# kiranbond/cilium

Hardware: AMD Instinct MI355X
Metric: policy verdicts/sec (whole node) + request GB/s, 10K-rule L7 HTTP set (higher is better)
Workload: dtype u8

## Files before the change

cilium_amd/_native.py:

```python
from __future__ import annotations

import ctypes as C
import os
from pathlib import Path

LIB_PATH = Path(os.environ.get("CILIUM_AMD_LIB") or Path(__file__).resolve().parent / "libciliumgpu.so")

CG_OK = 0
CG_POLICY_DROP = 1
CG_PARSER_ERROR = 2
CG_UNKNOWN_PARSER = 3
CG_UNKNOWN_CONNECTION = 4
CG_INVALID_ADDRESS = 5
CG_INVALID_INSTANCE = 6
CG_UNKNOWN_ERROR = 7
CG_INVALID_ARGUMENT = 16
CG_NO_DEVICE = 17
CG_DEVICE_ERROR = 18
CG_POLICY_REJECTED = 19
CG_REVISION_MISMATCH = 20
CG_MAP_FULL = 21
CG_NOT_FOUND = 22
CG_NO_MAP = 23
CG_UNSUPPORTED = 24

CG_REGEX_ECMA, CG_REGEX_GO = 0, 1

CG_L4_F_INGRESS = 0x01
CG_L4_F_FRAGMENT = 0x02
CG_L4_F_CB_POLICY = 0x04
CG_L4_CAN_ACCESS, CG_L4_INGRESS, CG_L4_EGRESS, CG_L4_IGNORE_DROP = 0, 1, 2, 0x100
CG_DROP_POLICY = -133
CG_DROP_FRAG_NOSUPPORT = -157
CG_DROP_MISSED_TAIL_CALL = -140
CG_POLICY_ARRAY_SLOTS = 65536
CG_DROP_INVALID, CG_DROP_CT_INVALID_HDR, CG_DROP_CT_UNKNOWN_PROTO, CG_DROP_UNKNOWN_L3 = -134, -135, -137, -139
CG_DROP_INVALID_EXTHDR = -156
CG_FRAME_NOT_LOCAL, CG_FRAME_TO_HOST = -1, -2
CG_ENDPOINT_F_HOST = 1

CG_PF_DYN4, CG_PF_DYN6, CG_PF_FIX4, CG_PF_FIX6 = 1, 2, 4, 8
CG_XDP_DROP, CG_XDP_PASS = 1, 2
CG_WORLD_ID = 2

CG_CTR_HTTP_PROGRAMS, CG_CTR_KAFKA, CG_CTR_PREFILTER, CG_CTR_HTTP_RULES, CG_CTR_HTTP_ALLREDUCE = 0, 1, 2, 3, 4
CG_HTTP_RULE_NO_HTTP, CG_HTTP_RULE_SCOPE_ALLOW = 0xFFFFFFFF, 0xFFFFFFFE

CG_HTTP_TILE = 64
CG_HTTP_UNITS = 9

CG_KAFKA_MAX_TOPICS = 12
CG_KAFKA_K_NIL, CG_KAFKA_K_TYPED, CG_KAFKA_K_CONSUMER_METADATA = 0, 1, 2
CG_KAFKA_UNKNOWN_STR = 0xFFFFFFFF
CG_KAFKA_TOPICS_IN_ARENA = 255
CG_KAFKA_DECODE_OK, CG_KAFKA_DECODE_ERROR = 0, 1
CG_KAFKA_V_DENY, CG_KAFKA_V_ALLOW, CG_KAFKA_V_CLOSE = 0, 1, 2

CG_SEL_MATCH_LABEL, CG_SEL_IN, CG_SEL_NOT_IN, CG_SEL_EXISTS, CG_SEL_DOES_NOT_EXIST = 0, 1, 2, 3, 4
CG_EXP_ALL = 0x1


class CiliumGPUError(RuntimeError):
    def __init__(self, code: int, msg: str):
        super().__init__(f"[{code}] {msg}")
        self.code = code
        self.msg = msg


class KV(C.Structure):
    _fields_ = [("key", C.c_char_p), ("value", C.c_char_p)]


class PolicyKeyC(C.Structure):
    _pack_ = 1
    _fields_ = [("sec_label", C.c_uint32), ("dport", C.c_uint16), ("protocol", C.c_uint8), ("egress", C.c_uint8)]


class PolicyEntryC(C.Structure):
    _fields_ = [("proxy_port", C.c_uint16), ("pad", C.c_uint16 * 3), ("packets", C.c_uint64),
                ("bytes", C.c_uint64)]


class CidrC(C.Structure):
    _fields_ = [("family", C.c_uint8), ("prefixlen", C.c_uint8), ("pad", C.c_uint8 * 2), ("addr", C.c_uint8 * 16)]


class SelectorTableC(C.Structure):
    _fields_ = [("n_selectors", C.c_size_t), ("req_off", C.c_void_p), ("ops", C.c_void_p),
                ("key_blob", C.c_void_p), ("key_off", C.c_void_p), ("val_off", C.c_void_p),
                ("val_blob", C.c_void_p), ("val_str_off", C.c_void_p)]


class SelcacheRulesC(C.Structure):
    _fields_ = [("n_rules", C.c_size_t), ("subject", C.c_void_p), ("dir_flags", C.c_void_p),
                ("req_off", C.c_void_p * 2), ("req_idx", C.c_void_p * 2),
                ("allow_off", C.c_void_p * 2), ("allow_idx", C.c_void_p * 2)]


class ExpandTableC(C.Structure):
    _fields_ = [("n_rows", C.c_size_t), ("rows", C.c_void_p), ("src_off", C.c_void_p), ("src_idx", C.c_void_p)]


_u64, _u32, _sz, _p, _i64 = C.c_uint64, C.c_uint32, C.c_size_t, C.c_void_p, C.c_int64
SIGNATURES = {
    "cg_open": (_u64, [C.POINTER(KV), _sz, C.c_uint8]),
    "cg_close": (None, [_u64]),
    "cg_last_error": (C.c_char_p, []),
    "cg_version": (C.c_char_p, []),
    "cg_sync": (C.c_int, [_u64]),
    "cg_policymap_create": (C.c_int, [_u64, _u32, C.POINTER(_u32)]),
    "cg_policymap_destroy": (C.c_int, [_u64, _u32]),
    "cg_policymap_allow": (C.c_int, [_u64, _u32, _p, _p, _sz]),
    "cg_policymap_delete": (C.c_int, [_u64, _u32, _p, _sz]),
    "cg_policymap_lookup": (C.c_int, [_u64, _u32, _p, _p]),
    "cg_policymap_dump": (C.c_int, [_u64, _u32, _p, _p, _sz, C.POINTER(_sz)]),
    "cg_policymap_flush": (C.c_int, [_u64, _u32]),
    "cg_l4_verdicts_dev": (C.c_int, [_u64, _u32, _p, _sz, _p, _p]),
    "cg_l4_verdicts_host": (C.c_int, [_u64, _u32, _p, _sz, _p]),
    "cg_l4_policy_verdicts_dev": (C.c_int, [_u64, _u32, _u32, _p, _sz, _p, _p]),
    "cg_l4_policy_verdicts_host": (C.c_int, [_u64, _u32, _u32, _p, _sz, _p]),
    "cg_prefilter_create": (C.c_int, [_u64, _u32, _u32, _u32, C.POINTER(_u32)]),
    "cg_prefilter_destroy": (C.c_int, [_u64, _u32]),
    "cg_prefilter_insert": (C.c_int, [_u64, _u32, _i64, _p, _sz, C.POINTER(_i64)]),
    "cg_prefilter_delete": (C.c_int, [_u64, _u32, _i64, _p, _sz, C.POINTER(_i64)]),
    "cg_prefilter_dump": (C.c_int, [_u64, _u32, _p, _sz, C.POINTER(_sz), C.POINTER(_i64)]),
    "cg_prefilter_set_endpoints": (C.c_int, [_u64, _u32, _p, _sz, _p, _sz]),
    "cg_prefilter_verdicts_dev": (C.c_int, [_u64, _u32, _p, _sz, _p, _p, _sz, _p, _p]),
    "cg_prefilter_verdicts_host": (C.c_int, [_u64, _u32, _p, _sz, _p, _p, _sz, _p]),
    "cg_ipcache_create": (C.c_int, [_u64, _u32, C.POINTER(_u32)]),
    "cg_ipcache_destroy": (C.c_int, [_u64, _u32]),
    "cg_ipcache_update": (C.c_int, [_u64, _u32, _p, _p, _sz]),
    "cg_ipcache_delete": (C.c_int, [_u64, _u32, _p, _sz]),
    "cg_ipcache_lookup": (C.c_int, [_u64, _u32, _p, _p]),
    "cg_ipcache_dump": (C.c_int, [_u64, _u32, _p, _p, _sz, C.POINTER(_sz)]),
    "cg_ipcache_resolve_dev": (C.c_int, [_u64, _u32, _p, _sz, _p, _p, _sz, _p, _p]),
    "cg_ipcache_resolve_host": (C.c_int, [_u64, _u32, _p, _sz, _p, _p, _sz, _p]),
    "cg_proxylib_stats": (C.c_int, [_u64, C.POINTER(C.c_uint64), C.POINTER(C.c_uint64)]),
    "cg_kafka_decode_stats": (C.c_int, [_u64, C.POINTER(C.c_uint64), C.POINTER(C.c_uint64)]),
    "cg_kafka_inflate_stats": (C.c_int, [_u64, C.POINTER(C.c_uint64)]),
    "cg_proxylib_set_batching": (C.c_int, [_u64, _u32, _u32]),
    "cg_proxylib_policy_update": (C.c_int, [_u64, C.c_char_p, _sz]),
    "cg_proxylib_policy_update_npds": (C.c_int, [_u64, C.c_char_p, _sz]),
    "cg_l4_verdicts_ipcache_dev": (C.c_int, [_u64, _u32, _u32, _p, _p, _sz, _p, _p]),
    "cg_l4_verdicts_ipcache_host": (C.c_int, [_u64, _u32, _u32, _p, _p, _sz, _p]),
    "cg_l4_verdicts_ipcache6_dev": (C.c_int, [_u64, _u32, _u32, _p, _p, _sz, _p, _p]),
    "cg_l4_verdicts_ipcache6_host": (C.c_int, [_u64, _u32, _u32, _p, _p, _sz, _p]),
    "cg_http_policy_update": (C.c_int, [_u64, C.c_char_p, _sz]),
    "cg_http_policy_update_npds": (C.c_int, [_u64, C.c_char_p, _sz]),
    "cg_http_pack_threads": (_u32, []),
    "cg_http_policy_export": (C.c_int, [_u64, C.c_void_p, _sz, C.POINTER(_sz)]),
    "cg_http_policy_import": (C.c_int, [_u64, C.c_char_p, _sz]),
    "cg_http_policy_index": (C.c_int, [_u64, C.c_char_p, C.POINTER(_u32)]),
    "cg_http_policy_stats": (C.c_int, [_u64, C.POINTER(_u64), _sz]),
    "cg_http_rule_info_get": (C.c_int, [_u64, _p, _sz, C.POINTER(_sz)]),
    "cg_http_batch_bytes": (_sz, [_u64, _sz]),
    "cg_http_batch_slots": (_sz, [_u64, _sz]),
    "cg_http_pack": (C.c_int, [_u64, _sz, _p, _p, _p, _p, _p, _p, _p, _sz, _p, C.POINTER(_sz), _p, _sz,
                               C.POINTER(_sz)]),
    "cg_http_parse_heads": (C.c_int, [_p, _p, _sz, _p, _sz, _p, C.POINTER(_sz), _p]),
    "cg_http_verdicts_dev": (C.c_int, [_u64, _p, _sz, _p, _p, _p]),
    "cg_http_verdicts_host": (C.c_int, [_u64, _p, _sz, _p, _sz, _p, _sz, _p]),
    "cg_http_verdicts_rules_host": (C.c_int, [_u64, _p, _sz, _p, _sz, _p, _sz, _p, _p]),
    "cg_http_verdicts_rules_dev": (C.c_int, [_u64, _p, _sz, _p, _p, _p, _p]),
    "cg_http_verdicts_raw_dev": (C.c_int, [_u64, _p, _p, _sz, _p, _p, _p, _p, _p, _p]),
    "cg_http_verdicts_raw_host": (C.c_int, [_u64, _p, _p, _sz, _p, _p, _p, _p, _p]),
    "cg_http_verdicts_fields_dev": (C.c_int, [_u64, _p, _p, _sz, _p, _p, _p, _p, _p, _p]),
    "cg_http_verdicts_fields_host": (C.c_int, [_u64, _p, _p, _sz, _p, _p, _p, _p, _p]),
    "cg_http_ring_open": (C.c_int, [_u64, C.c_uint32, C.c_uint32]),
    "cg_http_ring_verdicts": (C.c_int, [_u64, _p, _p, _sz, _p, _p, _p, _p, _p]),
    "cg_http_ring_stats": (C.c_int, [_u64, C.POINTER(C.c_uint64), C.POINTER(C.c_uint64)]),
    "cg_http_ring_close": (C.c_int, [_u64]),
    "cg_kafka_policy_update": (C.c_int, [_u64, C.c_char_p, _sz]),
    "cg_kafka_policy_index": (C.c_int, [_u64, C.c_char_p, C.POINTER(_u32)]),
    "cg_kafka_intern": (C.c_int, [_u64, _u32, C.c_char_p, _sz, C.POINTER(_u32)]),
    "cg_kafka_verdicts_dev": (C.c_int, [_u64, _p, _sz, _p, _p, _p]),
    "cg_kafka_verdicts_split_dev": (C.c_int, [_u64, _p, _p, _sz, _p, _p, _p]),
    "cg_kafka_verdicts_host": (C.c_int, [_u64, _p, _sz, _p, _sz, _p]),
    "cg_kafka_decode_host": (C.c_int, [_u64, _p, _p, _sz, _p, _p, _p, _p, _sz, C.POINTER(_sz), _p]),
    "cg_kafka_decode_dev": (C.c_int, [_u64, _p, _p, _sz, _p, _p, _p, _p, _sz, C.POINTER(_sz), _p, _p]),
    "cg_kafka_verdicts_raw_host": (C.c_int, [_u64, _p, _p, _sz, _p, _p, _p]),
    "cg_diag_kafka_decode_host": (C.c_int, [_u64, _p, _p, _sz, _p, _p, _p, _p, _sz, C.POINTER(_sz), _p]),
    "cg_read_counters": (C.c_int, [_u64, _u32, _u32, _p, _sz, C.POINTER(_sz)]),
    "cg_counters_device_ptr": (C.c_int, [_u64, _u32, _u32, C.POINTER(_p), C.POINTER(_sz)]),
    "cg_counters_copy_dev": (C.c_int, [_u64, _u32, _u32, _p, _sz, _p]),
    "cg_reset_counters": (C.c_int, [_u64]),
    "cg_diag_regex_match": (C.c_int, [C.c_char_p, _sz, _p, _sz, _u32, C.POINTER(C.c_uint8)]),
    "cg_regex_validate": (C.c_int, [C.c_char_p, _sz, _u32]),
    "cg_diag_http_eval_host": (C.c_int, [_u64, _p, _sz, _p, _sz, _p, _sz, _p]),
    "cg_diag_http_rules_host": (C.c_int, [_u64, _p, _sz, _p, _sz, _p, _sz, _p]),
    "cg_diag_kafka_eval_host": (C.c_int, [_u64, _p, _sz, _p, _sz, _p]),
    "cg_diag_l4_eval_host": (C.c_int, [_u64, _u32, _p, _sz, _p]),
    "cg_diag_ipcache_eval_host": (C.c_int, [_u64, _u32, _p, _sz, _p, _p, _sz, _p]),
    "cg_diag_prefilter_eval_host": (C.c_int, [_u64, _u32, _p, _sz, _p, _p, _sz, _p]),
    "cg_selcache_create": (C.c_int, [_u64, C.POINTER(_u32)]),
    "cg_selcache_destroy": (C.c_int, [_u64, _u32]),
    "cg_selcache_set_identities": (C.c_int, [_u64, _u32, _p, _sz, _p, _p, _p, _p, _p]),
    "cg_selcache_set_cidr_identities": (C.c_int, [_u64, _u32, _p, _p, _sz]),
    "cg_selcache_set_rules": (C.c_int, [_u64, _u32, C.POINTER(SelectorTableC), C.POINTER(SelcacheRulesC)]),
    "cg_selcache_info": (C.c_int, [_u64, _u32, C.POINTER(_sz), C.POINTER(_sz), C.POINTER(_sz), C.POINTER(_sz)]),
    "cg_selcache_match_dev": (C.c_int, [_u64, _u32, C.POINTER(SelectorTableC), _p, _sz, _p]),
    "cg_selcache_match_host": (C.c_int, [_u64, _u32, C.POINTER(SelectorTableC), _p, _sz]),
    "cg_selcache_reach_dev": (C.c_int, [_u64, _u32, _p, _sz, _p, _p, _p, _p]),
    "cg_selcache_reach_host": (C.c_int, [_u64, _u32, _p, _sz, _p, _p, _p]),
    "cg_diag_selcache_match_host": (C.c_int, [_u64, _u32, C.POINTER(SelectorTableC), _p, _sz, _u32]),
    "cg_diag_selcache_reach_host": (C.c_int, [_u64, _u32, _p, _sz, _p, _p, _p, _u32]),
    "cg_selcache_expand_dev": (C.c_int, [_u64, _u32, C.POINTER(ExpandTableC), _p, _sz, _p, _p, _p, _sz, _p, _p]),
    "cg_selcache_expand_host": (C.c_int, [_u64, _u32, C.POINTER(ExpandTableC), _p, _sz, _p, _p, _p, _sz, _p]),
    "cg_selcache_entries_host": (C.c_int, [_u64, _u32, C.POINTER(SelectorTableC), _p, _sz, C.POINTER(ExpandTableC),
                                           _p, _p, _p, _sz, _p, _p]),
    "cg_diag_selcache_expand_host": (C.c_int, [_u64, _u32, C.POINTER(ExpandTableC), _p, _sz, _p, _p, _p, _sz, _p,
                                               _u32]),
    "cg_diag_selcache_entries_host": (C.c_int, [_u64, _u32, C.POINTER(SelectorTableC), _p, _sz,
                                                C.POINTER(ExpandTableC), _p, _p, _p, _sz, _p, _p, _u32]),
    "cg_policymap_sync": (C.c_int, [_u64, _u32, _p, _p, _sz, C.POINTER(_sz), C.POINTER(_sz)]),
    "cg_policy_array_create": (C.c_int, [_u64, C.POINTER(_u32)]),
    "cg_policy_array_destroy": (C.c_int, [_u64, _u32]),
    "cg_policy_array_set": (C.c_int, [_u64, _u32, _p, _p, _sz]),
    "cg_policy_array_clear": (C.c_int, [_u64, _u32, _p, _sz]),
    "cg_policy_array_get": (C.c_int, [_u64, _u32, C.c_uint16, C.POINTER(_u32)]),
    "cg_l4_array_verdicts_dev": (C.c_int, [_u64, _u32, _u32, _p, _p, _sz, _p, _p]),
    "cg_l4_array_verdicts_host": (C.c_int, [_u64, _u32, _u32, _p, _p, _sz, _p]),
    "cg_l4_array_verdicts_ipcache_dev": (C.c_int, [_u64, _u32, _u32, _u32, C.c_int, _p, _p, _p, _sz, _p, _p]),
    "cg_l4_array_verdicts_ipcache_host": (C.c_int, [_u64, _u32, _u32, _u32, C.c_int, _p, _p, _p, _sz, _p]),
    "cg_diag_l4_array_eval_host": (C.c_int, [_u64, _u32, _u32, _p, _p, _sz, _p]),
    "cg_endpoint_map_create": (C.c_int, [_u64, _u32, C.POINTER(_u32)]),
    "cg_endpoint_map_destroy": (C.c_int, [_u64, _u32]),
    "cg_endpoint_map_update": (C.c_int, [_u64, _u32, _p, _p, _sz]),
    "cg_endpoint_map_delete": (C.c_int, [_u64, _u32, _p, _sz]),
    "cg_endpoint_map_lookup": (C.c_int, [_u64, _u32, _p, _p]),
    "cg_endpoint_map_dump": (C.c_int, [_u64, _u32, _p, _p, _sz, C.POINTER(_sz)]),
    "cg_l4_frames_verdicts_dev": (C.c_int, [_u64, _u32, _u32, _p, _p, _sz, _p, _u32, _p, _u32, _p, _p, _p, _p]),
    "cg_l4_frames_verdicts_host": (C.c_int, [_u64, _u32, _u32, _p, _p, _sz, _p, _u32, _p, _u32, _p, _p, _p]),
    "cg_diag_l4_frames_eval_host": (C.c_int, [_u64, _u32, _u32, _p, _p, _sz, _p, _u32, _p, _u32, _p, _p, _p, _p]),
}


def _load() -> C.CDLL:
    if not LIB_PATH.exists():
        raise ImportError(f"{LIB_PATH} is missing: build it with `python -m cilium_amd.build` "
                          "(there is no CPU fallback for the verdict paths)")
    lib = C.CDLL(str(LIB_PATH), mode=os.RTLD_NOW | getattr(os, "RTLD_GLOBAL", 0))
    for name, (res, args) in SIGNATURES.items():
        fn = getattr(lib, name)
        fn.restype = res
        fn.argtypes = args
    return lib


lib = _load()


def check(rc: int) -> None:
    if rc != CG_OK:
        raise CiliumGPUError(rc, lib.cg_last_error().decode(errors="replace"))


def regex_validate(pattern, flavour: int = CG_REGEX_GO) -> None:
    b = pattern.encode("utf-8", "surrogateescape") if isinstance(pattern, str) else bytes(pattern)
    check(lib.cg_regex_validate(b, len(b), flavour))


def ptr(a) -> int | None:
    if a is None:
        return None
    if hasattr(a, "data_ptr"):
        return a.data_ptr()
    return a.ctypes.data
```

cilium_amd/classifier.py:

```python
from __future__ import annotations

import ctypes as C
import ipaddress
import json
from typing import Iterable, Optional, Sequence

import numpy as np

from . import _native as N
from .policy import PolicyEntry, PolicyKey, PortRuleKafka, htons

L4_TUPLE_DTYPE = np.dtype([("identity", "<u4"), ("dport", "<u2"), ("proto", "u1"), ("flags", "u1"),
                           ("len", "<u4")])
POLICY_KEY_DTYPE = np.dtype([("sec_label", "<u4"), ("dport", "<u2"), ("protocol", "u1"), ("egress", "u1")])
CIDR_DTYPE = np.dtype([("family", "u1"), ("prefixlen", "u1"), ("pad", "u1", (2,)), ("addr", "u1", (16,))])
KAFKA_REQ_DTYPE = np.dtype([("api_key", "<i2"), ("api_version", "<i2"), ("kind", "u1"), ("n_topics", "u1"),
                            ("policy", "<u2"), ("remote", "<u4"), ("client_id", "<u4"),
                            ("topic_ids", "<u4", (N.CG_KAFKA_MAX_TOPICS,))])
ENDPOINT_KEY_DTYPE = np.dtype([("family", "u1"), ("pad", "u1", (3,)), ("addr", "u1", (16,))])
ENDPOINT_INFO_DTYPE = np.dtype([("lxc_id", "<u2"), ("pad", "<u2"), ("flags", "<u4")])
FRAME_INFO_DTYPE = np.dtype([("t", L4_TUPLE_DTYPE), ("lxc_id", "<u2"), ("family", "u1"), ("pad", "u1")])
assert ENDPOINT_KEY_DTYPE.itemsize == 20 and ENDPOINT_INFO_DTYPE.itemsize == 8 and FRAME_INFO_DTYPE.itemsize == 16
assert L4_TUPLE_DTYPE.itemsize == 12 and KAFKA_REQ_DTYPE.itemsize == 64 and CIDR_DTYPE.itemsize == 20


def _p(a):
    return N.ptr(a)


class HttpBatch:

    def __init__(self, batch: np.ndarray, arena: np.ndarray, order: np.ndarray, nslots: int, n: int):
        self.batch, self.arena, self.order, self.nslots, self.n = batch, arena, order, nslots, n

    def used_bytes(self) -> int:
        return int(self.batch[:64].view(np.uint64)[5])


class Classifier:

    def __init__(self, device: int = 0, debug: bool = False):
        kv = (N.KV * 1)(N.KV(b"device", str(device).encode()))
        self.h = N.lib.cg_open(kv, 1, 1 if debug else 0)
        if not self.h:
            raise N.CiliumGPUError(N.CG_NO_DEVICE, N.lib.cg_last_error().decode())
        self.device = device

    def close(self) -> None:
        if self.h:
            N.lib.cg_close(self.h)
            self.h = 0

    def __enter__(self):
        return self

    def __exit__(self, *a):
        self.close()

    def __del__(self):
        try:
            self.close()
        except Exception:
            pass

    def sync(self) -> None:
        N.check(N.lib.cg_sync(self.h))

    def policy_map(self, max_entries: int = 0) -> "PolicyMap":
        return PolicyMap(self, max_entries)

    def policy_array(self) -> "PolicyArray":
        return PolicyArray(self)

    def endpoint_map(self, max_entries: int = 0) -> "EndpointMap":
        return EndpointMap(self, max_entries)

    def prefilter(self, dyn4: bool = False, dyn6: bool = False, fix4: bool = True, fix6: bool = True,
                  max_lpm: int = 0, max_hash: int = 0) -> "PreFilter":
        return PreFilter(self, dyn4, dyn6, fix4, fix6, max_lpm, max_hash)

    def ipcache(self, max_entries: int = 0) -> "IPCache":
        return IPCache(self, max_entries)

    def selector_cache(self) -> "SelectorCache":
        from .selcache import SelectorCache
        return SelectorCache(self)

    def update_http_policy(self, policies: list[dict] | bytes | str) -> None:
        blob = policies if isinstance(policies, (bytes, str)) else json.dumps(policies, separators=(",", ":"))
        if isinstance(blob, str):
            blob = blob.encode()
        N.check(N.lib.cg_http_policy_update(self.h, blob, len(blob)))

    def update_http_policy_npds(self, discovery_response: bytes) -> None:
        N.check(N.lib.cg_http_policy_update_npds(self.h, discovery_response, len(discovery_response)))

    def export_http_policy(self) -> bytes:
        n = C.c_size_t()
        N.check(N.lib.cg_http_policy_export(self.h, None, 0, C.byref(n)))
        buf = C.create_string_buffer(n.value)
        N.check(N.lib.cg_http_policy_export(self.h, buf, n.value, C.byref(n)))
        return buf.raw[:n.value]

    def import_http_policy(self, image: bytes) -> None:
        N.check(N.lib.cg_http_policy_import(self.h, image, len(image)))

    def http_policy_index(self, name: str) -> int:
        v = C.c_uint32()
        rc = N.lib.cg_http_policy_index(self.h, name.encode(), C.byref(v))
        if rc == N.CG_NOT_FOUND:
            return 0xFFFFFFFF
        N.check(rc)
        return v.value

    def http_policy_stats(self) -> dict:
        out = (C.c_uint64 * 12)()
        N.check(N.lib.cg_http_policy_stats(self.h, out, 12))
        keys = ["programs", "parts", "states", "table_bytes", "fields", "rules", "policies", "remote_slots",
                "exceptions", "cells", "max_program_cells", "lds_programs"]
        return dict(zip(keys, list(out)))

    def pack_http(self, policy: np.ndarray, ingress: np.ndarray, port: np.ndarray, remote: np.ndarray,
                  hdr_blob: np.ndarray, hdr_off: np.ndarray):
        n = len(policy)
        policy = np.ascontiguousarray(policy, dtype=np.uint32)
        ingress = np.ascontiguousarray(ingress, dtype=np.uint8)
        port = np.ascontiguousarray(port, dtype=np.uint16)
        remote = np.ascontiguousarray(remote, dtype=np.uint32)
        hdr_blob = np.ascontiguousarray(hdr_blob, dtype=np.uint8)
        hdr_off = np.ascontiguousarray(hdr_off, dtype=np.uint64)
        if len(hdr_blob) == 0:
            hdr_blob = np.zeros(1, np.uint8)
        used = C.c_size_t()
        nslots = C.c_size_t()
        stats = (C.c_uint64 * 12)()
        N.check(N.lib.cg_http_policy_stats(self.h, stats, 12))
        cap = (int(hdr_off[n]) - int(hdr_off[0]) if n else 0) + n * (int(stats[4]) + 24) + 16
        arena = np.empty(cap, np.uint8)
        batch = np.empty(N.lib.cg_http_batch_bytes(self.h, n), np.uint8)
        order = np.empty(max(N.lib.cg_http_batch_slots(self.h, n), 1), np.uint32)
        N.check(N.lib.cg_http_pack(self.h, n, _p(policy), _p(ingress), _p(port), _p(remote), _p(hdr_blob),
                                   _p(hdr_off), _p(batch), batch.nbytes, _p(order), C.byref(nslots), _p(arena),
                                   arena.nbytes, C.byref(used)))
        arena = arena[:max(used.value, 16)].copy()
        return HttpBatch(batch, arena, order[:nslots.value], nslots.value, n)

    @staticmethod
    def parse_http_heads(raw_blob: np.ndarray, raw_off: np.ndarray):
        raw_blob = np.ascontiguousarray(raw_blob, np.uint8)
        raw_off = np.ascontiguousarray(raw_off, np.uint64)
        n = len(raw_off) - 1
        if len(raw_blob) == 0:
            raw_blob = np.zeros(1, np.uint8)
        used = C.c_size_t()
        N.check(N.lib.cg_http_parse_heads(_p(raw_blob), _p(raw_off), n, None, 0, None, C.byref(used), None))
        blob = np.zeros(max(used.value, 1), np.uint8)
        off = np.zeros(n + 1, np.uint64)
        ok = np.zeros(max(n, 1), np.uint8)
        N.check(N.lib.cg_http_parse_heads(_p(raw_blob), _p(raw_off), n, _p(blob), blob.nbytes, _p(off),
                                          C.byref(used), _p(ok)))
        return blob, off, ok[:n]

    def pack_http_raw(self, policy, ingress, port, remote, raw_blob: np.ndarray, raw_off: np.ndarray):
        blob, off, ok = self.parse_http_heads(raw_blob, raw_off)
        pol = np.where(ok.astype(bool), np.asarray(policy, np.uint32), np.uint32(0xFFFFFFFF)).astype(np.uint32)
        return self.pack_http(pol, ingress, port, remote, blob, off)

    def http_verdicts_raw(self, policy, ingress, port, remote, raw_blob: np.ndarray, raw_off: np.ndarray) -> np.ndarray:
        return self._verdicts_from_host(N.lib.cg_http_verdicts_raw_host, policy, ingress, port, remote, raw_blob,
                                        raw_off)

    def http_verdicts_fields(self, policy, ingress, port, remote, hdr_blob: np.ndarray,
                             hdr_off: np.ndarray) -> np.ndarray:
        return self._verdicts_from_host(N.lib.cg_http_verdicts_fields_host, policy, ingress, port, remote, hdr_blob,
                                        hdr_off)

    def http_ring_open(self, workgroups: int = 16, slots: int = 32) -> None:
        N.check(N.lib.cg_http_ring_open(self.h, workgroups, slots))

    def http_ring_verdicts(self, policy, ingress, port, remote, hdr_blob: np.ndarray,
                           hdr_off: np.ndarray) -> np.ndarray:
        return self._verdicts_from_host(N.lib.cg_http_ring_verdicts, policy, ingress, port, remote, hdr_blob,
                                        hdr_off)

    def http_ring_stats(self) -> dict:
        served, launches = C.c_uint64(), C.c_uint64()
        N.check(N.lib.cg_http_ring_stats(self.h, C.byref(served), C.byref(launches)))
        return {"served": served.value, "launches": launches.value}

    def http_ring_close(self) -> None:
        N.check(N.lib.cg_http_ring_close(self.h))

    def _verdicts_from_host(self, fn, policy, ingress, port, remote, raw_blob, raw_off) -> np.ndarray:
        raw_blob = np.ascontiguousarray(raw_blob, np.uint8)
        raw_off = np.ascontiguousarray(raw_off, np.uint64)
        n = len(raw_off) - 1
        if len(raw_blob) == 0:
            raw_blob = np.zeros(1, np.uint8)
        pol = np.ascontiguousarray(policy, np.uint32)
        ing = np.ascontiguousarray(ingress, np.uint8)
        prt = np.ascontiguousarray(port, np.uint16)
        rem = np.ascontiguousarray(remote, np.uint32)
        out = np.zeros(max(n, 1), np.uint8)
        N.check(fn(self.h, _p(raw_blob), _p(raw_off), n, _p(pol), _p(ing), _p(prt), _p(rem), _p(out)))
        return out[:n]

    def http_verdicts_raw_dev(self, d_raw, d_off, n: int, d_policy, d_ingress, d_port, d_remote, d_out,
                              stream=None) -> None:
        N.check(N.lib.cg_http_verdicts_raw_dev(self.h, _p(d_raw), _p(d_off), n, _p(d_policy), _p(d_ingress),
                                               _p(d_port), _p(d_remote), _p(d_out), stream))

    def http_verdicts_fields_dev(self, d_blob, d_off, n: int, d_policy, d_ingress, d_port, d_remote, d_out,
                                 stream=None) -> None:
        N.check(N.lib.cg_http_verdicts_fields_dev(self.h, _p(d_blob), _p(d_off), n, _p(d_policy), _p(d_ingress),
                                                  _p(d_port), _p(d_remote), _p(d_out), stream))

    def http_verdicts(self, b: "HttpBatch") -> np.ndarray:
        out = np.zeros(max(b.n, 1), np.uint8)
        N.check(N.lib.cg_http_verdicts_host(self.h, _p(b.batch), b.nslots, _p(b.order), b.n, _p(b.arena),
                                            b.arena.nbytes, _p(out)))
        return out[:b.n]

    def http_verdicts_dev(self, d_batch, nslots: int, d_arena, d_out, stream=None) -> None:
        N.check(N.lib.cg_http_verdicts_dev(self.h, _p(d_batch), nslots, _p(d_arena), _p(d_out), stream))

    def http_verdicts_rules(self, b: "HttpBatch") -> tuple[np.ndarray, np.ndarray]:
        out = np.zeros(max(b.n, 1), np.uint8)
        rule = np.zeros(max(b.n, 1), np.uint32)
        N.check(N.lib.cg_http_verdicts_rules_host(self.h, _p(b.batch), b.nslots, _p(b.order), b.n, _p(b.arena),
                                                  b.arena.nbytes, _p(out), _p(rule)))
        return out[:b.n], rule[:b.n]

    def http_verdicts_rules_dev(self, d_batch, nslots: int, d_arena, d_out, d_rule, stream=None) -> None:
        N.check(N.lib.cg_http_verdicts_rules_dev(self.h, _p(d_batch), nslots, _p(d_arena), _p(d_out), _p(d_rule),
                                                 stream))

    HTTP_RULE_INFO_DTYPE = np.dtype([("policy", "<u4"), ("ingress", "<u4"), ("port", "<u4"), ("scope", "<u4"),
                                     ("rule", "<u4"), ("http_rule", "<u4")])

    def http_rule_info(self) -> np.ndarray:
        n = C.c_size_t()
        N.check(N.lib.cg_http_rule_info_get(self.h, None, 0, C.byref(n)))
        out = np.zeros(max(n.value, 1), self.HTTP_RULE_INFO_DTYPE)
        N.check(N.lib.cg_http_rule_info_get(self.h, _p(out), n.value, C.byref(n)))
        return out[:n.value]

    def http_rule_hits(self) -> np.ndarray:
        return self.read_counters(N.CG_CTR_HTTP_RULES)

    def allreduce_counter_count(self) -> int:
        return self.counters_device_ptr(N.CG_CTR_HTTP_ALLREDUCE)[1]

    def counters_copy_dev(self, d_dst, n: int, stream=None, what: int = N.CG_CTR_HTTP_ALLREDUCE) -> None:
        N.check(N.lib.cg_counters_copy_dev(self.h, what, 0, _p(d_dst), n, stream))

    def http_rules_host_diag(self, b: "HttpBatch") -> np.ndarray:
        out = np.zeros(max(b.n, 1), np.uint32)
        N.check(N.lib.cg_diag_http_rules_host(self.h, _p(b.batch), b.nslots, _p(b.order), b.n, _p(b.arena),
                                              b.arena.nbytes, _p(out)))
        return out[:b.n]

    def http_eval_host_diag_slots(self, b: "HttpBatch") -> np.ndarray:
        v = self.http_eval_host_diag(b)
        out = np.zeros(b.nslots, np.uint8)
        order = b.order[:b.nslots]
        real = order < b.n
        out[real] = v[order[real]]
        return out

    def http_eval_host_diag(self, b: "HttpBatch") -> np.ndarray:
        out = np.zeros(max(b.n, 1), np.uint8)
        N.check(N.lib.cg_diag_http_eval_host(self.h, _p(b.batch), b.nslots, _p(b.order), b.n, _p(b.arena),
                                             b.arena.nbytes, _p(out)))
        return out[:b.n]

    def update_kafka_policy(self, redirects: list[dict]) -> None:
        def conv(r):
            return r.to_json() if isinstance(r, PortRuleKafka) else r
        doc = [{"name": rd["name"], "selectors": [
            {"identities": s.get("identities"), "rules": [conv(r) for r in s.get("rules", [])]}
            for s in rd.get("selectors", [])]} for rd in redirects]
        blob = json.dumps(doc).encode()
        N.check(N.lib.cg_kafka_policy_update(self.h, blob, len(blob)))

    def kafka_redirect_index(self, name: str) -> int:
        v = C.c_uint32()
        rc = N.lib.cg_kafka_policy_index(self.h, name.encode(), C.byref(v))
        if rc == N.CG_NOT_FOUND:
            return 0xFFFF
        N.check(rc)
        return v.value

    def kafka_intern(self, what: str, s: bytes) -> int:
        v = C.c_uint32()
        N.check(N.lib.cg_kafka_intern(self.h, 0 if what == "topic" else 1, s, len(s), C.byref(v)))
        return v.value

    def pack_kafka(self, redirect: Sequence[int], remote: Sequence[int], api_key: Sequence[int],
                   api_version: Sequence[int], kind: Sequence[int], client_id: Sequence[bytes],
                   topics: Sequence[Sequence[bytes]]):
        n = len(redirect)
        reqs = np.zeros(n, KAFKA_REQ_DTYPE)
        reqs["policy"] = np.asarray(redirect, np.uint16)
        reqs["remote"] = np.asarray(remote, np.uint32)
        reqs["api_key"] = np.asarray(api_key, np.int16)
        reqs["api_version"] = np.asarray(api_version, np.int16)
        reqs["kind"] = np.asarray(kind, np.uint8)
        cache_t: dict = {}
        cache_c: dict = {}
        arena: list[int] = []
        for i in range(n):
            c = client_id[i]
            if c not in cache_c:
                cache_c[c] = self.kafka_intern("client", c)
            reqs["client_id"][i] = cache_c[c]
            ts = topics[i]
            ids = []
            for t in ts:
                if t not in cache_t:
                    cache_t[t] = self.kafka_intern("topic", t)
                ids.append(cache_t[t])
            reqs["n_topics"][i] = min(len(ids), N.CG_KAFKA_TOPICS_IN_ARENA)
            if len(ids) <= N.CG_KAFKA_MAX_TOPICS:
                reqs["topic_ids"][i, :len(ids)] = ids
            else:
                reqs["topic_ids"][i, 0] = len(arena)
                if len(ids) >= N.CG_KAFKA_TOPICS_IN_ARENA:
                    reqs["topic_ids"][i, 1] = len(ids)
                arena.extend(ids)
        return reqs, np.asarray(arena if arena else [0], np.uint32)

    def kafka_decode(self, raw, raw_off, redirect, remote, diag_cpu: bool = False):
        raw = np.ascontiguousarray(raw, np.uint8)
        off = np.ascontiguousarray(raw_off, np.uint64)
        n = len(off) - 1
        red = np.ascontiguousarray(redirect, np.uint16)
        rem = np.ascontiguousarray(remote, np.uint32)
        if len(red) != n or len(rem) != n:
            raise ValueError("redirect/remote must have one entry per request")
        reqs = np.zeros(max(n, 1), KAFKA_REQ_DTYPE)
        status = np.zeros(max(n, 1), np.uint8)
        fn = N.lib.cg_diag_kafka_decode_host if diag_cpu else N.lib.cg_kafka_decode_host
        cap = 64
        while True:
            arena = np.zeros(cap, np.uint32)
            used = C.c_size_t()
            rc = fn(self.h, _p(raw), _p(off), n, _p(red), _p(rem), _p(reqs), _p(arena), cap, C.byref(used),
                    _p(status))
            if rc == N.CG_MAP_FULL and used.value > cap:
                cap = used.value
                continue
            N.check(rc)
            return reqs[:n], arena[:max(used.value, 1)], status[:n]

    def kafka_decode_dev(self, d_raw, d_off, n: int, d_redirect, d_remote, d_reqs, d_arena, arena_cap: int,
                         d_status, stream=None) -> int:
        used = C.c_size_t()
        N.check(N.lib.cg_kafka_decode_dev(self.h, _p(d_raw), _p(d_off), n, _p(d_redirect), _p(d_remote),
                                          _p(d_reqs), _p(d_arena), arena_cap, C.byref(used), _p(d_status), stream))
        return used.value

    def kafka_verdicts_raw(self, raw, raw_off, redirect, remote) -> np.ndarray:
        raw = np.ascontiguousarray(raw, np.uint8)
        off = np.ascontiguousarray(raw_off, np.uint64)
        n = len(off) - 1
        red = np.ascontiguousarray(redirect, np.uint16)
        rem = np.ascontiguousarray(remote, np.uint32)
        if len(red) != n or len(rem) != n:
            raise ValueError("redirect/remote must have one entry per request")
        out = np.zeros(max(n, 1), np.uint8)
        N.check(N.lib.cg_kafka_verdicts_raw_host(self.h, _p(raw), _p(off), n, _p(red), _p(rem), _p(out)))
        return out[:n]

    def kafka_verdicts(self, reqs: np.ndarray, arena: Optional[np.ndarray] = None) -> np.ndarray:
        n = len(reqs)
        out = np.zeros(max(n, 1), np.uint8)
        N.check(N.lib.cg_kafka_verdicts_host(self.h, _p(reqs), n, _p(arena), 0 if arena is None else len(arena),
                                             _p(out)))
        return out[:n]

    def kafka_verdicts_dev(self, d_reqs, n: int, d_arena, d_out, stream=None) -> None:
        N.check(N.lib.cg_kafka_verdicts_dev(self.h, _p(d_reqs), n, _p(d_arena), _p(d_out), stream))

    def kafka_verdicts_split_dev(self, d_heads, d_topics, n: int, d_arena, d_out, stream=None) -> None:
        N.check(N.lib.cg_kafka_verdicts_split_dev(self.h, _p(d_heads), _p(d_topics), n, _p(d_arena), _p(d_out),
                                                  stream))

    def kafka_eval_host_diag(self, reqs: np.ndarray, arena: Optional[np.ndarray] = None) -> np.ndarray:
        n = len(reqs)
        out = np.zeros(max(n, 1), np.uint8)
        N.check(N.lib.cg_diag_kafka_eval_host(self.h, _p(reqs), n, _p(arena), 0 if arena is None else len(arena),
                                              _p(out)))
        return out[:n]

    def read_counters(self, what: int, ident: int = 0) -> np.ndarray:
        n = C.c_size_t()
        N.check(N.lib.cg_read_counters(self.h, what, ident, None, 0, C.byref(n)))
        out = np.zeros(max(n.value, 1), np.uint64)
        N.check(N.lib.cg_read_counters(self.h, what, ident, _p(out), n.value, C.byref(n)))
        return out[:n.value]

    def counters_device_ptr(self, what: int, ident: int = 0) -> tuple[int, int]:
        p = C.c_void_p()
        n = C.c_size_t()
        N.check(N.lib.cg_counters_device_ptr(self.h, what, ident, C.byref(p), C.byref(n)))
        return p.value or 0, n.value

    def reset_counters(self) -> None:
        N.check(N.lib.cg_reset_counters(self.h))


class PolicyEntriesDump(list):

    def less(self, i: int, j: int) -> bool:
        a, b = self[i][0], self[j][0]
        if a.TrafficDirection < b.TrafficDirection:
            return True
        return a.TrafficDirection <= b.TrafficDirection and a.Identity < b.Identity

    def sorted(self) -> "PolicyEntriesDump":
        return PolicyEntriesDump(sorted(self, key=lambda ke: (ke[0].TrafficDirection, ke[0].Identity)))


class PolicyMap:

    def __init__(self, cl: Classifier, max_entries: int = 0):
        self.cl = cl
        v = C.c_uint32()
        N.check(N.lib.cg_policymap_create(cl.h, max_entries, C.byref(v)))
        self.id = v.value

    @classmethod
    def attach(cls, cl: Classifier, map_id: int) -> "PolicyMap":
        pm = cls.__new__(cls)
        pm.cl, pm.id = cl, int(map_id)
        return pm

    @staticmethod
    def _keys(keys: Iterable[PolicyKey]) -> np.ndarray:
        ks = list(keys)
        a = np.zeros(len(ks), POLICY_KEY_DTYPE)
        for i, k in enumerate(ks):
            a[i] = (k.Identity, k.DestPort, k.Nexthdr, k.TrafficDirection)
        return a

    def allow_key(self, k: PolicyKey, proxy_port: int) -> None:
        self.allow(k.Identity, k.DestPort, k.Nexthdr, k.TrafficDirection, proxy_port)

    def allow(self, identity: int, dport: int, proto: int, direction: int, proxy_port: int) -> None:
        self.allow_keys(self._keys([PolicyKey(identity, htons(dport), proto, int(direction))]),
                        np.asarray([htons(proxy_port)], np.uint16))

    def allow_keys(self, keys: np.ndarray, ports_be: np.ndarray) -> None:
        keys = np.ascontiguousarray(keys, POLICY_KEY_DTYPE)
        ports_be = np.ascontiguousarray(ports_be, np.uint16)
        N.check(N.lib.cg_policymap_allow(self.cl.h, self.id, _p(keys), _p(ports_be), len(keys)))

    def sync(self, keys: np.ndarray, ports_be: np.ndarray) -> tuple[int, int]:
        keys = np.ascontiguousarray(keys, POLICY_KEY_DTYPE)
        ports_be = np.ascontiguousarray(ports_be, np.uint16)
        if len(keys) != len(ports_be):
            raise ValueError("keys and ports_be differ in length")
        added, deleted = C.c_size_t(), C.c_size_t()
        N.check(N.lib.cg_policymap_sync(self.cl.h, self.id, _p(keys) if len(keys) else None,
                                        _p(ports_be) if len(keys) else None, len(keys),
                                        C.byref(added), C.byref(deleted)))
        return added.value, deleted.value

    def exists(self, identity: int, dport: int, proto: int, direction: int) -> bool:
        return self.lookup(PolicyKey(identity, htons(dport), proto, int(direction))) is not None

    def lookup(self, k: PolicyKey) -> Optional[PolicyEntry]:
        key = self._keys([k])
        e = N.PolicyEntryC()
        rc = N.lib.cg_policymap_lookup(self.cl.h, self.id, _p(key), C.byref(e))
        if rc == N.CG_NOT_FOUND:
            return None
        N.check(rc)
        return PolicyEntry(e.proxy_port, e.packets, e.bytes)

    def delete_key(self, k: PolicyKey) -> None:
        self.delete(k.Identity, k.DestPort, k.Nexthdr, k.TrafficDirection)

    def delete(self, identity: int, dport: int, proto: int, direction: int) -> None:
        key = self._keys([PolicyKey(identity, htons(dport), proto, int(direction))])
        N.check(N.lib.cg_policymap_delete(self.cl.h, self.id, _p(key), 1))

    def dump_to_slice(self) -> PolicyEntriesDump:
        n = C.c_size_t()
        N.check(N.lib.cg_policymap_dump(self.cl.h, self.id, None, None, 0, C.byref(n)))
        keys = np.zeros(max(n.value, 1), POLICY_KEY_DTYPE)
        ents = (N.PolicyEntryC * max(n.value, 1))()
        N.check(N.lib.cg_policymap_dump(self.cl.h, self.id, _p(keys), C.addressof(ents), n.value, C.byref(n)))
        return PolicyEntriesDump(
            (PolicyKey(int(k["sec_label"]), int(k["dport"]), int(k["protocol"]), int(k["egress"])),
             PolicyEntry(e.proxy_port, e.packets, e.bytes)) for k, e in zip(keys[:n.value], ents[:n.value]))

    def destroy(self) -> None:
        N.check(N.lib.cg_policymap_destroy(self.cl.h, self.id))

    def flush(self) -> None:
        N.check(N.lib.cg_policymap_flush(self.cl.h, self.id))

    def verdicts(self, tuples: np.ndarray, mode: int = N.CG_L4_CAN_ACCESS) -> np.ndarray:
        tuples = np.ascontiguousarray(tuples, L4_TUPLE_DTYPE)
        out = np.zeros(max(len(tuples), 1), np.int32)
        if mode == N.CG_L4_CAN_ACCESS:
            N.check(N.lib.cg_l4_verdicts_host(self.cl.h, self.id, _p(tuples), len(tuples), _p(out)))
        else:
            N.check(N.lib.cg_l4_policy_verdicts_host(self.cl.h, self.id, mode, _p(tuples), len(tuples), _p(out)))
        return out[:len(tuples)]

    def policy_can_access_ingress(self, tuples: np.ndarray) -> np.ndarray:
        return self.verdicts(tuples, N.CG_L4_INGRESS)

    def policy_can_egress(self, tuples: np.ndarray) -> np.ndarray:
        return self.verdicts(tuples, N.CG_L4_EGRESS)

    def verdicts_via_ipcache(self, ipc: "IPCache", remote: np.ndarray, tuples: np.ndarray) -> np.ndarray:
        tuples = np.ascontiguousarray(tuples, L4_TUPLE_DTYPE)
        out = np.zeros(max(len(tuples), 1), np.int32)
        if remote.dtype == np.uint8:
            remote = np.ascontiguousarray(remote, np.uint8).reshape(-1, 16)
            N.check(N.lib.cg_l4_verdicts_ipcache6_host(self.cl.h, self.id, ipc.id, _p(remote), _p(tuples),
                                                       len(tuples), _p(out)))
        else:
            remote = np.ascontiguousarray(remote, np.uint32)
            N.check(N.lib.cg_l4_verdicts_ipcache_host(self.cl.h, self.id, ipc.id, _p(remote), _p(tuples),
                                                      len(tuples), _p(out)))
        return out[:len(tuples)]

    def verdicts_dev(self, d_tuples, n: int, d_out, stream=None, mode: int = N.CG_L4_CAN_ACCESS) -> None:
        if mode == N.CG_L4_CAN_ACCESS:
            N.check(N.lib.cg_l4_verdicts_dev(self.cl.h, self.id, _p(d_tuples), n, _p(d_out), stream))
        else:
            N.check(N.lib.cg_l4_policy_verdicts_dev(self.cl.h, self.id, mode, _p(d_tuples), n, _p(d_out), stream))

    def eval_host_diag(self, tuples: np.ndarray) -> np.ndarray:
        tuples = np.ascontiguousarray(tuples, L4_TUPLE_DTYPE)
        out = np.zeros(max(len(tuples), 1), np.int32)
        N.check(N.lib.cg_diag_l4_eval_host(self.cl.h, self.id, _p(tuples), len(tuples), _p(out)))
        return out[:len(tuples)]


class PolicyArray:

    def __init__(self, cl: Classifier):
        self.cl = cl
        v = C.c_uint32()
        N.check(N.lib.cg_policy_array_create(cl.h, C.byref(v)))
        self.id = v.value

    @staticmethod
    def _lxc(lxc_ids) -> np.ndarray:
        a = np.asarray(lxc_ids)
        if a.size and (a.min() < 0 or a.max() >= N.CG_POLICY_ARRAY_SLOTS):
            raise N.CiliumGPUError(N.CG_INVALID_ARGUMENT, "lxc_id outside the policy array")
        return np.ascontiguousarray(a, np.uint16).reshape(-1)

    def set(self, lxc_id: int, policy_map: "PolicyMap") -> None:
        self.set_many([lxc_id], [policy_map])

    def set_many(self, lxc_ids, maps: Sequence) -> None:
# ... 332 lines not shown
```

cilium_amd/csrc/capi.cc:

```cpp
#include <hip/hip_runtime_api.h>

#include <algorithm>
#include <exception>
#include <chrono>
#include <cstring>
#include <map>
#include <memory>
#include <mutex>
#include <thread>
#include <string>
#include <vector>

#include "endpoint_map.h"
#include "engine.h"
#include "frame_walk.h"
#include "http.h"
#include "kafka.h"
#include "kafka_wire.h"
#include "kernels.h"
#include "l4.h"
#include "l4_array.h"
#include "l4_walk.h"
#include "ipcache.h"
#include "lpm.h"
// ... 1396 lines not shown

int cg_diag_selcache_match_host(uint64_t h, uint32_t sc_id, const cg_selector_table* sels, uint64_t* bits,
                                size_t cap_words, uint32_t threads) {
  return guarded([&] {
    auto e = get(h);
    const auto p = sc_pub(*e, sc_id);
    ScSelTab own;
    const ScSelTab& t = sc_table_of(*p, sels, &own);
    sc_check_cap(*p, t, bits, cap_words);
    sc_match_host(p->host_idents(), t.view(), bits, threads);
  });
}

static void sc_ensure_host_m(Engine& e, ScPublished& p, uint32_t threads) {
  std::lock_guard<std::mutex> lk(e.mu);
  const size_t need = p.seltab.sels.size() * (size_t)p.words;
  if (p.host_m.size() != need || !need) {
    p.host_m.assign(std::max<size_t>(need, 1), 0);
    sc_match_host(p.host_idents(), p.seltab.view(), p.host_m.data(), threads);
    if (!need) p.host_m.resize(1);
  }
}

int cg_diag_selcache_reach_host(uint64_t h, uint32_t sc_id, const uint32_t* endpoints, size_t n, uint64_t* ing,
                                uint64_t* eg, uint8_t* flags, uint32_t threads) {
  return guarded([&] {
    auto e = get(h);
    const auto p = sc_pub(*e, sc_id);
    sc_check_endpoints(*p, endpoints, n, ing, eg, flags);
    sc_ensure_host_m(*e, *p, threads);
    sc_reach_host(p->host_rules(), p->n, p->words, endpoints, n, ing, eg, flags, threads);
  });
}

static void sc_check_expand_out(const cg_expand_table* table, const void* row_off, const void* keys,
                                const void* proxy, size_t cap) {
  if (!table) fail(CG_INVALID_ARGUMENT, "selcache expand: NULL table");
  if (!row_off) fail(CG_INVALID_ARGUMENT, "selcache expand: NULL row_off");
  if (cap && (!keys || !proxy)) fail(CG_INVALID_ARGUMENT, "selcache expand: NULL keys/proxy");
  if (cap > (1ull << 40)) fail(CG_INVALID_ARGUMENT, "selcache expand: cap_entries out of range");
}

static ScExpDev sc_exp_view(const ScPublished& p, const ScExpRow* rows, const uint32_t* src_idx, size_t n_rows,
                            const uint32_t* ids, const uint64_t* src) {
  ScExpDev X{};
  X.rows = rows;
  X.src_idx = src_idx;
  X.ids = ids;
  X.src = reinterpret_cast<const unsigned long long*>(src);
  X.n_rows = (uint32_t)n_rows;
  X.n_ids = p.n;
  X.words = p.words;
  return X;
}

int cg_selcache_expand_dev(uint64_t h, uint32_t sc_id, const cg_expand_table* table, const uint64_t* d_src,
                           size_t src_rows, uint64_t* d_row_off, cg_policy_key* d_keys, uint16_t* d_proxy,
                           size_t cap_entries, uint64_t* d_total, void* stream) {
  return guarded([&] {
    auto e = get(h);
    e->require_gpu();
    sc_check_expand_out(table, d_row_off, d_keys, d_proxy, cap_entries);
    if ((uintptr_t)d_keys & 7u) fail(CG_INVALID_ARGUMENT, "selcache expand: d_keys is not 8-byte aligned");
    const auto p = sc_pub(*e, sc_id);
    const ScExpTab t = sc_compile_expand(*table, src_rows);
    if (!t.src_idx.empty() && p->words && !d_src) fail(CG_INVALID_ARGUMENT, "selcache expand: NULL source matrix");
    e->set_device();
    void* st = stream_of(*e, stream);
    auto tmp = std::make_shared<DevTables>();
    const ScExpDev X = sc_exp_view(*p, tmp->add(t.rows), tmp->add(t.src_idx), t.rows.size(), p->d_ids, d_src);
    check_launch(launch_selcache_expand(X, (unsigned long long*)d_row_off, d_keys, d_proxy, cap_entries,
                                        (unsigned long long*)d_total, st, e->cus),
                 "selcache expand kernel launch");
    fence(p->tab, st);
    fence(tmp, st);
  });
}

static void sc_expand_copy_back(Engine& e, size_t n_rows, const DevMem& d_off, const DevMem& d_keys,
                                const DevMem& d_proxy, uint64_t* row_off, cg_policy_key* keys, uint16_t* proxy,
                                size_t cap, uint64_t* total) {
  hipStream_t st = (hipStream_t)e.stream;
  hip_check(hipMemcpyAsync(row_off, d_off.get(), (n_rows + 1) * sizeof(uint64_t), hipMemcpyDeviceToHost, st),
            "hipMemcpy D2H");
  dev_sync(e, nullptr);
  const uint64_t n = row_off[n_rows];
  if (total) *total = n;
  if (n && n <= cap) {
    hip_check(hipMemcpyAsync(keys, d_keys.get(), n * sizeof(cg_policy_key), hipMemcpyDeviceToHost, st), "hipMemcpy D2H");
    hip_check(hipMemcpyAsync(proxy, d_proxy.get(), n * sizeof(uint16_t), hipMemcpyDeviceToHost, st), "hipMemcpy D2H");
    dev_sync(e, nullptr);
  }
}

int cg_selcache_expand_host(uint64_t h, uint32_t sc_id, const cg_expand_table* table, const uint64_t* src,
                            size_t src_rows, uint64_t* row_off, cg_policy_key* keys, uint16_t* proxy,
                            size_t cap_entries, uint64_t* total) {
  return guarded([&] {
    auto e = get(h);
    e->require_gpu();
    sc_check_expand_out(table, row_off, keys, proxy, cap_entries);
    const auto p = sc_pub(*e, sc_id);
    const ScExpTab t = sc_compile_expand(*table, src_rows);
    const size_t src_bytes = src_rows * (size_t)p->words * sizeof(uint64_t);
    if (src_bytes && !src) fail(CG_INVALID_ARGUMENT, "selcache expand: NULL source matrix");
    e->set_device();
    DevTables tmp;
    DevMem d_src, d_off, d_keys, d_proxy;
    d_src.upload(src, src_bytes);
    d_off.alloc((t.rows.size() + 1) * sizeof(uint64_t));
    d_keys.alloc(cap_entries * sizeof(cg_policy_key));
    d_proxy.alloc(cap_entries * sizeof(uint16_t));
    const ScExpDev X = sc_exp_view(*p, tmp.add(t.rows), tmp.add(t.src_idx), t.rows.size(), p->d_ids, d_src.as<uint64_t>());
    check_launch(launch_selcache_expand(X, d_off.as<unsigned long long>(), d_keys.get(), d_proxy.as<uint16_t>(),
                                        cap_entries, nullptr, e->stream, e->cus),
                 "selcache expand kernel launch");
    fence(p->tab, e->stream);
    sc_expand_copy_back(*e, t.rows.size(), d_off, d_keys, d_proxy, row_off, keys, proxy, cap_entries, total);
  });
}

static void sc_check_entries_args(const ScPublished& p, const uint32_t* eps, size_t n, const void* flags) {
  if (n && (!eps || !flags)) fail(CG_INVALID_ARGUMENT, "selcache entries: NULL endpoints/flags");
  if (n > 0x3FFFFFFFu) fail(CG_MAP_FULL, "selcache entries: too many endpoints");
  for (size_t i = 0; i < n; ++i)
    if (eps[i] >= p.n) fail(CG_INVALID_ARGUMENT, "selcache entries: endpoint index outside the identity table");
}

int cg_selcache_entries_host(uint64_t h, uint32_t sc_id, const cg_selector_table* sels, const uint32_t* endpoints,
                             size_t n_endpoints, const cg_expand_table* table, uint64_t* row_off,
                             cg_policy_key* keys, uint16_t* proxy, size_t cap_entries, uint64_t* total,
                             uint8_t* flags) {
  return guarded([&] {
    auto e = get(h);
    e->require_gpu();
    sc_check_expand_out(table, row_off, keys, proxy, cap_entries);
    const auto p = sc_pub(*e, sc_id);
    sc_check_entries_args(*p, endpoints, n_endpoints, flags);
    ScSelTab own;
    if (sels) own = sc_compile_selectors(*p->idents, sc_parse_selectors(*sels));
    const size_t S = own.sels.size(), E = n_endpoints, W = p->words;
    const ScExpTab t = sc_compile_expand(*table, S + 2 * E);
    e->set_device();
    DevTables tmp;
    DevMem d_src, d_ep, d_fl, d_off, d_keys, d_proxy;
    d_src.alloc((S + 2 * E) * W * sizeof(uint64_t));
    d_off.alloc((t.rows.size() + 1) * sizeof(uint64_t));
    d_keys.alloc(cap_entries * sizeof(cg_policy_key));
    d_proxy.alloc(cap_entries * sizeof(uint16_t));
    unsigned long long* src = d_src.as<unsigned long long>();
    if (S)
      check_launch(launch_selcache_match(p->dI, sc_upload_table(own, tmp), src, e->stream, e->cus),
                   "selcache match kernel launch");
    if (E) {
      d_ep.upload(endpoints, E * sizeof(uint32_t));
      d_fl.alloc(E);
      check_launch(launch_selcache_reach(p->dR, p->n, p->words, d_ep.as<uint32_t>(), E, src + S * W,
                                         src + (S + E) * W, d_fl.as<uint8_t>(), e->stream),
                   "selcache reach kernel launch");
      hip_check(hipMemcpyAsync(flags, d_fl.get(), E, hipMemcpyDeviceToHost, (hipStream_t)e->stream), "hipMemcpy D2H");
    }
    const ScExpDev X = sc_exp_view(*p, tmp.add(t.rows), tmp.add(t.src_idx), t.rows.size(), p->d_ids, d_src.as<uint64_t>());
    check_launch(launch_selcache_expand(X, d_off.as<unsigned long long>(), d_keys.get(), d_proxy.as<uint16_t>(),
                                        cap_entries, nullptr, e->stream, e->cus),
                 "selcache expand kernel launch");
    fence(p->tab, e->stream);
    sc_expand_copy_back(*e, t.rows.size(), d_off, d_keys, d_proxy, row_off, keys, proxy, cap_entries, total);
  });
}

int cg_diag_selcache_expand_host(uint64_t h, uint32_t sc_id, const cg_expand_table* table, const uint64_t* src,
                                 size_t src_rows, uint64_t* row_off, cg_policy_key* keys, uint16_t* proxy,
                                 size_t cap_entries, uint64_t* total, uint32_t threads) {
  return guarded([&] {
    auto e = get(h);
    sc_check_expand_out(table, row_off, keys, proxy, cap_entries);
    const auto p = sc_pub(*e, sc_id);
    const ScExpTab t = sc_compile_expand(*table, src_rows);
    if (src_rows * (size_t)p->words && !src) fail(CG_INVALID_ARGUMENT, "selcache expand: NULL source matrix");
    uint64_t n = 0;
    sc_expand_host(sc_exp_view(*p, t.rows.data(), t.src_idx.data(), t.rows.size(), p->ids.data(), src),
                   row_off, keys, proxy, cap_entries, &n, threads);
    if (total) *total = n;
  });
}

int cg_diag_selcache_entries_host(uint64_t h, uint32_t sc_id, const cg_selector_table* sels,
                                  const uint32_t* endpoints, size_t n_endpoints, const cg_expand_table* table,
                                  uint64_t* row_off, cg_policy_key* keys, uint16_t* proxy, size_t cap_entries,
                                  uint64_t* total, uint8_t* flags, uint32_t threads) {
  return guarded([&] {
    auto e = get(h);
    sc_check_expand_out(table, row_off, keys, proxy, cap_entries);
    const auto p = sc_pub(*e, sc_id);
    sc_check_entries_args(*p, endpoints, n_endpoints, flags);
    ScSelTab own;
    if (sels) own = sc_compile_selectors(*p->idents, sc_parse_selectors(*sels));
    const size_t S = own.sels.size(), E = n_endpoints, W = p->words;
    const ScExpTab t = sc_compile_expand(*table, S + 2 * E);
    std::vector<uint64_t> src(std::max<size_t>((S + 2 * E) * W, 1), 0);
    if (S) sc_match_host(p->host_idents(), own.view(), src.data(), threads);
    if (E) {
      sc_ensure_host_m(*e, *p, threads);
      sc_reach_host(p->host_rules(), p->n, p->words, endpoints, E, src.data() + S * W,
                    src.data() + (S + E) * W, flags, threads);
    }
    uint64_t n = 0;
    sc_expand_host(sc_exp_view(*p, t.rows.data(), t.src_idx.data(), t.rows.size(), p->ids.data(), src.data()),
                   row_off, keys, proxy, cap_entries, &n, threads);
    if (total) *total = n;
  });
}

int cg_http_policy_update(uint64_t h, const char* json, size_t len) {
  return guarded([&] {
    auto e = get(h);
    if (!json) fail(CG_INVALID_ARGUMENT, "NULL policy");
    std::shared_ptr<HttpSnapshot> snap = http_compile(json, len);
    if (e->has_gpu()) {
      e->set_device();
      snap->upload(*e);
    }
    {
      std::lock_guard<std::mutex> lk(e->mu);
      e->http = snap;
    }
    bump_epoch();
  });
}

int cg_http_policy_update_npds(uint64_t h, const uint8_t* resp, size_t len) {
  std::string json;
  const int rc = guarded([&] {
    if (!resp && len) fail(CG_INVALID_ARGUMENT, "NULL DiscoveryResponse");
    json = npds_pb_to_json(resp, len, true);
  });
  if (rc != CG_OK) return rc;
  return cg_http_policy_update(h, json.data(), json.size());
}

static std::shared_ptr<HttpSnapshot> http_snap(Engine& e);

int cg_http_policy_export(uint64_t h, void* buf, size_t cap, size_t* len) {
  return guarded([&] {
    auto e = get(h);
    const std::vector<uint8_t> img = http_image_export(*http_snap(*e));
    if (len) *len = img.size();
    if (buf && cap >= img.size()) memcpy(buf, img.data(), img.size());
    else if (buf) fail(CG_INVALID_ARGUMENT, "policy image buffer too small");
  });
}

int cg_http_policy_import(uint64_t h, const void* buf, size_t len) {
  return guarded([&] {
    auto e = get(h);
    std::shared_ptr<HttpSnapshot> snap = http_image_import(static_cast<const uint8_t*>(buf), len);
    if (e->has_gpu()) {
      e->set_device();
      snap->upload(*e);
    }
    {
      std::lock_guard<std::mutex> lk(e->mu);
      e->http = snap;
    }
    bump_epoch();
  });
}

static std::shared_ptr<HttpSnapshot> http_snap(Engine& e) {
  std::lock_guard<std::mutex> lk(e.mu);
  if (!e.http) fail(CG_NOT_FOUND, "no HTTP policy installed");
  return e.http;
}

int cg_http_policy_index(uint64_t h, const char* name, uint32_t* index) {
  return guarded([&] {
    auto e = get(h);
    auto s = http_snap(*e);
    auto it = s->policy_index.find(name ? name : "");
    if (it == s->policy_index.end()) fail(CG_NOT_FOUND, "no policy named " + std::string(name ? name : ""));
    *index = it->second;
  });
}

int cg_http_rule_info_get(uint64_t h, cg_http_rule_info* out, size_t cap, size_t* n) {
  return guarded([&] {
    auto e = get(h);
    auto s = http_snap(*e);
    if (n) *n = s->rule_info.size();
    if (out) memcpy(out, s->rule_info.data(), std::min(cap, s->rule_info.size()) * sizeof(cg_http_rule_info));
  });
}

int cg_http_policy_stats(uint64_t h, uint64_t* out, size_t n) {
  return guarded([&] {
    auto e = get(h);
    auto s = http_snap(*e);
    uint64_t max_prog_cells = 0, lds_progs = 0;
    for (const auto& pg : s->progs) {
      if (pg.flags & kProgAllowAll) continue;
      max_prog_cells = std::max<uint64_t>(max_prog_cells, pg.cell_count);
      lds_progs += (pg.flags & kProgRebased) && pg.cell_count <= kMaxLdsCells;
    }
    uint64_t v[12] = {s->progs.size(),
                     s->parts.size(),
                     s->total_states,
                     s->cells.size() * 4,
                     s->fields.size(),
                     s->total_rules,
                     s->npolicies,
                     s->total_remote_slots,
                     s->total_exceptions,
                     s->cells.size(),
                     max_prog_cells,
                     lds_progs};
    for (size_t i = 0; i < n && i < 12; ++i) out[i] = v[i];
  });
}

size_t cg_http_batch_bytes(uint64_t h, size_t n) {
  size_t v = 0;
  guarded([&] {
    auto e = get(h);
    v = http_batch_bytes(*http_snap(*e), n);
  });
  return v;
}

size_t cg_http_batch_slots(uint64_t h, size_t n) {
  size_t v = 0;
  guarded([&] {
    auto e = get(h);
    v = http_batch_slots(*http_snap(*e), n);
  });
  return v;
}

int cg_http_pack(uint64_t h, size_t n, const uint32_t* policy, const uint8_t* ingress, const uint16_t* port,
                 const uint32_t* remote, const uint8_t* hdr_blob, const uint64_t* hdr_off, void* batch,
                 size_t batch_cap, uint32_t* order, size_t* nslots, uint8_t* arena, size_t arena_cap,
                 size_t* arena_used) {
  return guarded([&] {
    auto e = get(h);
    auto s = http_snap(*e);
    http_pack(*s, n, policy, ingress, port, remote, hdr_blob, hdr_off, batch, batch_cap, order, nslots, arena,
              arena_cap, arena_used);
  });
}

static size_t batch_used_bytes(const void* batch) {
  HttpBatchHeader hdr;
  memcpy(&hdr, batch, sizeof(hdr));
  if (hdr.magic != kBatchMagic) fail(CG_INVALID_ARGUMENT, "not a packed HTTP batch");
  return hdr.total_bytes;
}

int cg_http_verdicts_dev(uint64_t h, const void* d_batch, size_t nslots, const uint8_t* d_arena, uint8_t* d_out,
                         void* stream) {
  return guarded([&] {
    auto e = get(h);
    e->require_gpu();
    auto s = http_snap(*e);
    e->set_device();
    check_launch(launch_http(s->dev, d_batch, nslots, d_arena, d_out, stream_of(*e, stream), e->cus),
                 "http kernel launch");
    s->fence.record(stream_of(*e, stream));
  });
}

int cg_http_verdicts_rules_dev(uint64_t h, const void* d_batch, size_t nslots, const uint8_t* d_arena, uint8_t* d_out,
                               uint32_t* d_rule, void* stream) {
  return guarded([&] {
    auto e = get(h);
    e->require_gpu();
    auto s = http_snap(*e);
    if (nslots && !d_rule) fail(CG_INVALID_ARGUMENT, "NULL rule array");
    e->set_device();
    check_launch(launch_http(s->dev, d_batch, nslots, d_arena, d_out, stream_of(*e, stream), e->cus, nullptr, d_rule),
                 "http kernel launch");
    s->fence.record(stream_of(*e, stream));
  });
}

int cg_http_verdicts_raw_dev(uint64_t h, const uint8_t* d_raw, const uint64_t* d_raw_off, size_t n,
                             const uint32_t* d_policy, const uint8_t* d_ingress, const uint16_t* d_port,
                             const uint32_t* d_remote, uint8_t* d_out, void* stream) {
  return guarded([&] {
    auto e = get(h);
    e->require_gpu();
    auto s = http_snap(*e);
    if (n && (!d_raw_off || !d_policy || !d_ingress || !d_port || !d_remote || !d_out))
      fail(CG_INVALID_ARGUMENT, "NULL device array");
    e->set_device();
    auto lease = e->staging.acquire(e->device);
    http_verdicts_raw_on(*s, *lease, e->cus, RawInput::Heads, d_raw, d_raw_off, n, d_policy, d_ingress, d_port,
                         d_remote, d_out, stream_of(*e, stream));
    s->fence.record(stream_of(*e, stream));
    if (!stream) hip_check(hipStreamSynchronize((hipStream_t)stream_of(*e, stream)), "hipStreamSynchronize");
  });
}

int cg_http_verdicts_fields_dev(uint64_t h, const uint8_t* d_hdr_blob, const uint64_t* d_hdr_off, size_t n,
                                const uint32_t* d_policy, const uint8_t* d_ingress, const uint16_t* d_port,
                                const uint32_t* d_remote, uint8_t* d_out, void* stream) {
  return guarded([&] {
    auto e = get(h);
    e->require_gpu();
    auto s = http_snap(*e);
    if (n && (!d_hdr_off || !d_policy || !d_ingress || !d_port || !d_remote || !d_out))
      fail(CG_INVALID_ARGUMENT, "NULL device array");
    e->set_device();
    auto lease = e->staging.acquire(e->device);
    http_verdicts_raw_on(*s, *lease, e->cus, RawInput::Lists, d_hdr_blob, d_hdr_off, n, d_policy, d_ingress, d_port,
                         d_remote, d_out, stream_of(*e, stream));
    s->fence.record(stream_of(*e, stream));
    if (!stream) hip_check(hipStreamSynchronize((hipStream_t)stream_of(*e, stream)), "hipStreamSynchronize");
  });
}

static void* stage_in(StagingSlot& sl, int i, const void* src, size_t bytes) {
  void* d = sl.dev_buf(i, bytes);
  if (!bytes) return d;
  void* hb = sl.host_buf(i, bytes);
  memcpy(hb, src, bytes);
  hip_check(hipMemcpyAsync(d, hb, bytes, hipMemcpyHostToDevice, (hipStream_t)sl.stream), "H2D");
  return d;
}

static void http_verdicts_host_impl(uint64_t h, const void* batch, size_t nslots, const uint32_t* order,
                                    size_t n, const uint8_t* arena, size_t arena_len, uint8_t* out, uint32_t* rule);

int cg_http_verdicts_host(uint64_t h, const void* batch, size_t nslots, const uint32_t* order, size_t n,
                          const uint8_t* arena, size_t arena_len, uint8_t* out) {
  return guarded([&] { http_verdicts_host_impl(h, batch, nslots, order, n, arena, arena_len, out, nullptr); });
}

int cg_http_verdicts_rules_host(uint64_t h, const void* batch, size_t nslots, const uint32_t* order, size_t n,
                                const uint8_t* arena, size_t arena_len, uint8_t* out, uint32_t* rule) {
  return guarded([&] {
    if (n && !rule) fail(CG_INVALID_ARGUMENT, "NULL rule array");
    http_verdicts_host_impl(h, batch, nslots, order, n, arena, arena_len, out, rule);
  });
}

static void http_verdicts_host_impl(uint64_t h, const void* batch, size_t nslots, const uint32_t* order,
                                    size_t n, const uint8_t* arena, size_t arena_len, uint8_t* out, uint32_t* rule) {
  {
    auto e = get(h);
    e->require_gpu();
    auto s = http_snap(*e);
    if (!batch || (n && (!order || !out))) fail(CG_INVALID_ARGUMENT, "NULL batch/order/out");
    HttpBatchHeader hdr;
    memcpy(&hdr, batch, sizeof(hdr));
    if (hdr.magic != kBatchMagic || hdr.epoch != s->epoch)
      fail(CG_INVALID_ARGUMENT, "batch was packed against another policy snapshot");
    if (hdr.nslots != nslots) fail(CG_INVALID_ARGUMENT, "nslots differs from the packed batch");
    if (hdr.arena_bytes && (!arena || arena_len < hdr.arena_bytes))
      fail(CG_INVALID_ARGUMENT, "overflow arena shorter than the packed batch needs");
    e->set_device();
    auto lease = e->staging.acquire(e->device);
    void* dr = stage_in(*lease, 0, batch, batch_used_bytes(batch));
    void* da = stage_in(*lease, 1, arena, hdr.arena_bytes);
    void* dout = lease->dev_buf(2, nslots + 1);
    uint32_t* drule = rule ? (uint32_t*)lease->dev_buf(3, (nslots + 1) * 4) : nullptr;
    check_launch(launch_http(s->dev, dr, nslots, (const uint8_t*)da, (uint8_t*)dout, lease->stream, e->cus, nullptr,
                             drule),
                 "http kernel launch");
    uint8_t* slots = (uint8_t*)lease->host_buf(2, nslots + 1);
    uint32_t* rslots = rule ? (uint32_t*)lease->host_buf(3, (nslots + 1) * 4) : nullptr;
    if (nslots)
      hip_check(hipMemcpyAsync(slots, dout, nslots, hipMemcpyDeviceToHost, (hipStream_t)lease->stream), "D2H");
    if (nslots && rule)
      hip_check(hipMemcpyAsync(rslots, drule, nslots * 4, hipMemcpyDeviceToHost, (hipStream_t)lease->stream), "D2H");
    hip_check(hipStreamSynchronize((hipStream_t)lease->stream), "hipStreamSynchronize");
    for (size_t i = 0; i < nslots; ++i)
      if (order[i] < n) {
        out[order[i]] = slots[i];
        if (rule) rule[order[i]] = rslots[i];
      }
  }
}

int cg_kafka_policy_update(uint64_t h, const char* json, size_t len) {
  return guarded([&] {
    auto e = get(h);
    if (!json) fail(CG_INVALID_ARGUMENT, "NULL policy");
    auto snap = kafka_compile(json, len);
    if (e->has_gpu()) {
      e->set_device();
      snap->upload(*e);
    }
    std::lock_guard<std::mutex> lk(e->mu);
    e->kafka = snap;
  });
}

static std::shared_ptr<KafkaSnapshot> kafka_snap(Engine& e) {
  std::lock_guard<std::mutex> lk(e.mu);
  if (!e.kafka) fail(CG_NOT_FOUND, "no Kafka policy installed");
  return e.kafka;
}

int cg_kafka_policy_index(uint64_t h, const char* name, uint32_t* index) {
  return guarded([&] {
    auto e = get(h);
    auto s = kafka_snap(*e);
    auto it = s->redirect_index.find(name ? name : "");
    if (it == s->redirect_index.end()) fail(CG_NOT_FOUND, "no Kafka redirect named " + std::string(name ? name : ""));
    *index = it->second;
  });
}

int cg_kafka_intern(uint64_t h, uint32_t what, const char* str, size_t len, uint32_t* id) {
  return guarded([&] {
    auto e = get(h);
    auto s = kafka_snap(*e);
    const auto& m = what == 0 ? s->topic_ids : s->client_ids;
    auto it = m.find(std::string(str ? str : "", len));
    *id = it == m.end() ? CG_KAFKA_UNKNOWN_STR : it->second;
  });
}

int cg_kafka_verdicts_dev(uint64_t h, const cg_kafka_request* d_reqs, size_t n, const uint32_t* d_arena,
                          uint8_t* d_out, void* stream) {
  return guarded([&] {
    auto e = get(h);
    e->require_gpu();
    auto s = kafka_snap(*e);
    e->set_device();
    check_launch(launch_kafka(s->dev, d_reqs, n, d_arena, d_out, stream_of(*e, stream), e->cus),
                 "kafka kernel launch");
    s->fence.record(stream_of(*e, stream));
  });
}

int cg_kafka_verdicts_split_dev(uint64_t h, const cg_kafka_request_head* d_heads, const uint32_t* d_topics,
                                size_t n, const uint32_t* d_arena, uint8_t* d_out, void* stream) {
  return guarded([&] {
    auto e = get(h);
    e->require_gpu();
    auto s = kafka_snap(*e);
    if (n && (!d_heads || !d_topics || !d_out)) fail(CG_INVALID_ARGUMENT, "NULL heads/topics/out");
    e->set_device();
    check_launch(launch_kafka(s->dev, d_heads, n, d_arena, d_out, stream_of(*e, stream), e->cus, d_topics),
                 "kafka kernel launch");
    s->fence.record(stream_of(*e, stream));
  });
}

int cg_kafka_verdicts_host(uint64_t h, const cg_kafka_request* reqs, size_t n, const uint32_t* arena,
                           size_t arena_len, uint8_t* out) {
  return guarded([&] {
    auto e = get(h);
    e->require_gpu();
    auto s = kafka_snap(*e);
    if (n && (!reqs || !out)) fail(CG_INVALID_ARGUMENT, "NULL requests/out");
    e->set_device();
    auto lease = e->staging.acquire(e->device);
    const uint32_t* da = (const uint32_t*)stage_in(*lease, 0, arena, arena ? arena_len * 4 : 0);
    hip_check(hipStreamSynchronize((hipStream_t)lease->stream), "hipStreamSynchronize");
    host_pipeline(*e, n, {{reqs, sizeof(cg_kafka_request)}}, {{out, 1}},
                  [&](void* const* din, void* const* dout, size_t cnt, void* st) {
                    check_launch(launch_kafka(s->dev, din[0], cnt, da, (uint8_t*)dout[0], st, e->cus),
                                 "kafka kernel launch");
                  });
  });
}

static size_t kafka_decode_on(Engine& e, const KafkaSnapshot& s, StagingSlot& sl, const uint8_t* d_raw,
                              const uint64_t* d_off, size_t n, const uint16_t* d_red, const uint32_t* d_rem,
                              cg_kafka_request* d_reqs, uint32_t* d_arena, size_t arena_cap, uint8_t* d_status,
                              hipStream_t st) {
  auto* ctr = (unsigned long long*)sl.dev_buf(7, 48);
  hip_check(hipMemsetAsync(ctr, 0, 48, st), "hipMemsetAsync");
  auto* dlist = (uint32_t*)sl.dev_buf(28, n * 4);
  uint8_t* zarena = (uint8_t*)sl.dev_buf(27, kKafkaInflateArena);
  check_launch(launch_kafka_decode(s.ddict[0], s.ddict[1], d_raw, d_off, n, d_red, d_rem, d_reqs, d_arena,
                                   arena_cap, ctr, d_status, st, e.cus, dlist, zarena, kKafkaInflateArena),
               "kafka decode kernel launch");
  auto* hc = (unsigned long long*)sl.host_buf(7, 48);
  hip_check(hipMemcpyAsync(hc, ctr, 48, hipMemcpyDeviceToHost, st), "D2H");
  hip_check(hipStreamSynchronize(st), "hipStreamSynchronize");
  size_t used = (size_t)hc[0];
  e.kafka_inflated.fetch_add(hc[3]);
  e.kafka_deferred.fetch_add(hc[4]);
  e.kafka_arena_full.fetch_add(hc[5]);
  if (hc[4] == 0) return used;
  std::vector<uint8_t> status(n);
  std::vector<uint64_t> off(n + 1);
  hip_check(hipMemcpy(status.data(), d_status, n, hipMemcpyDeviceToHost), "D2H");
  hip_check(hipMemcpy(off.data(), d_off, (n + 1) * 8, hipMemcpyDeviceToHost), "D2H");
  std::vector<uint8_t> bytes;
  std::vector<uint32_t> spill;
  for (size_t i = 0; i < n; ++i) {
    if (status[i] != 2) continue;
    const uint64_t len = off[i + 1] > off[i] ? off[i + 1] - off[i] : 0;
    bytes.resize(len);
    if (len) hip_check(hipMemcpy(bytes.data(), d_raw + off[i], len, hipMemcpyDeviceToHost), "D2H");
    cg_kafka_request q;
    hip_check(hipMemcpy(&q, d_reqs + i, sizeof(q), hipMemcpyDeviceToHost), "D2H");
    const size_t base = spill.size();
    const uint8_t rc = kafka_decode_host_one(s, bytes.data(), len, q.policy, q.remote, &q, &spill);
    if (rc == CG_KAFKA_DECODE_OK && q.n_topics > CG_KAFKA_MAX_TOPICS) q.topic_ids[0] = (uint32_t)(used + base);
    hip_check(hipMemcpy(d_reqs + i, &q, sizeof(q), hipMemcpyHostToDevice), "H2D");
    hip_check(hipMemcpy(d_status + i, &rc, 1, hipMemcpyHostToDevice), "H2D");
  }
  if (!spill.empty() && used + spill.size() <= arena_cap)
    hip_check(hipMemcpy(d_arena + used, spill.data(), spill.size() * 4, hipMemcpyHostToDevice), "H2D");
  return used + spill.size();
}

static void check_offsets(const uint64_t* off, size_t n) {
  if (!off) fail(CG_INVALID_ARGUMENT, "NULL raw_off");
  for (size_t i = 0; i < n; ++i)
    if (off[i + 1] < off[i]) fail(CG_INVALID_ARGUMENT, "raw_off must be non-decreasing");
}

int cg_kafka_decode_stats(uint64_t h, uint64_t* device_inflated, uint64_t* host_deferred) {
  return guarded([&] {
// ... 695 lines not shown
```

cilium_amd/csrc/clsdfa.cc:

```cpp
#include "clsdfa.h"

#include <algorithm>
#include <deque>
#include <map>
#include <numeric>
#include <unordered_map>

#include "common.h"

namespace cg {

namespace {

struct Partition {
  std::vector<int> elems, loc, blk, first, end, mid;
  std::vector<int> touched;

  explicit Partition(int n) : elems(n), loc(n), blk(n, 0) {
    std::iota(elems.begin(), elems.end(), 0);
    std::iota(loc.begin(), loc.end(), 0);
  }
  int nblocks() const { return (int)first.size(); }
  void mark(int e) {
    int b = blk[e];
    int i = loc[e], j = mid[b];
    if (i < j) return;
    std::swap(elems[i], elems[j]);
    loc[elems[i]] = i;
    loc[elems[j]] = j;
    if (mid[b]++ == first[b]) touched.push_back(b);
  }
};

}

ClsDfa minimize_cls(const ClsDfa& d) {
  const int n = d.size();
  const int k = d.ncls;
  Partition P(n);
  {
    std::vector<std::pair<uint32_t, int>> v(n);
    for (int s = 0; s < n; ++s) v[s] = {d.label[s], s};
    std::stable_sort(v.begin(), v.end());
    for (int i = 0; i < n; ++i) {
      int s = v[i].second;
      P.elems[i] = s;
      P.loc[s] = i;
      if (i == 0 || v[i].first != v[i - 1].first) {
        P.first.push_back(i);
        if (i > 0) P.end.push_back(i);
      }
      P.blk[s] = (int)P.first.size() - 1;
    }
    P.end.push_back(n);
    P.mid = P.first;
  }
  std::vector<int> inv_off((size_t)k * n + 1, 0);
  std::vector<int> inv((size_t)n * k);
  for (int s = 0; s < n; ++s)
    for (int c = 0; c < k; ++c) inv_off[(size_t)c * n + d.trans[(size_t)s * k + c] + 1]++;
  for (size_t i = 1; i < inv_off.size(); ++i) inv_off[i] += inv_off[i - 1];
  {
    std::vector<int> fill(inv_off.begin(), inv_off.end() - 1);
    for (int s = 0; s < n; ++s)
      for (int c = 0; c < k; ++c) inv[fill[(size_t)c * n + d.trans[(size_t)s * k + c]]++] = s;
  }
  std::vector<uint8_t> in_w(P.nblocks(), 1);
  std::vector<int> W;
  for (int b = 0; b < P.nblocks(); ++b) W.push_back(b);
  std::vector<int> splitter;
  while (!W.empty()) {
    int A = W.back();
    W.pop_back();
    in_w[A] = 0;
    splitter.assign(P.elems.begin() + P.first[A], P.elems.begin() + P.end[A]);
    for (int c = 0; c < k; ++c) {
      for (int t : splitter) {
        size_t o = (size_t)c * n + t;
        for (int i = inv_off[o]; i < inv_off[o + 1]; ++i) P.mark(inv[i]);
      }
      for (int b : P.touched) {
        if (P.mid[b] == P.end[b]) {
          P.mid[b] = P.first[b];
          continue;
        }
        int nb = P.nblocks();
        P.first.push_back(P.first[b]);
        P.end.push_back(P.mid[b]);
        P.mid.push_back(P.first[b]);
        P.first[b] = P.mid[b];
        P.mid[b] = P.first[b];
        for (int i = P.first[nb]; i < P.end[nb]; ++i) P.blk[P.elems[i]] = nb;
        in_w.push_back(0);
        int sz_nb = P.end[nb] - P.first[nb], sz_b = P.end[b] - P.first[b];
        if (in_w[b]) {
          W.push_back(nb);
          in_w[nb] = 1;
        } else if (sz_nb <= sz_b) {
          W.push_back(nb);
          in_w[nb] = 1;
        } else {
          W.push_back(b);
          in_w[b] = 1;
        }
      }
      P.touched.clear();
    }
  }
  const int nb = P.nblocks();
  std::vector<int> rep(nb);
  for (int b = 0; b < nb; ++b) rep[b] = P.elems[P.first[b]];
  std::vector<int> newid(nb, -1);
  std::vector<int> order;
  int dead_b = P.blk[0];
  newid[dead_b] = 0;
  order.push_back(dead_b);
  ClsDfa out;
  int start_b = P.blk[1];
  if (start_b != dead_b) {
    newid[start_b] = 1;
    order.push_back(start_b);
    for (size_t qi = 1; qi < order.size(); ++qi) {
      int s = rep[order[qi]];
      for (int c = 0; c < k; ++c) {
        int t = P.blk[d.trans[(size_t)s * k + c]];
        if (newid[t] < 0) {
          newid[t] = (int)order.size();
          order.push_back(t);
        }
      }
    }
  } else {
    order.push_back(dead_b);
  }
  const int m = (int)order.size();
  std::vector<int> col_id(k);
  std::vector<int> col_rep;
  {
    std::map<std::vector<int>, int> cols;
    std::vector<int> col(m);
    for (int c = 0; c < k; ++c) {
      for (int i = 0; i < m; ++i) {
        int t = (i == 1 && start_b == dead_b) ? 0 : newid[P.blk[d.trans[(size_t)rep[order[i]] * k + c]]];
        col[i] = (i == 0) ? 0 : t;
      }
      auto it = cols.emplace(col, (int)cols.size());
      col_id[c] = it.first->second;
      if (it.second) col_rep.push_back(c);
    }
  }
  out.ncls = (int)col_rep.size();
  for (int b = 0; b < 256; ++b) out.clsmap[b] = (uint8_t)col_id[d.clsmap[b]];
  out.trans.assign((size_t)m * out.ncls, 0);
  out.label.assign(m, 0);
  for (int i = 1; i < m; ++i) {
    if (start_b == dead_b) break;
    int s = rep[order[i]];
    out.label[i] = d.label[s];
    for (int c = 0; c < out.ncls; ++c)
      out.trans[(size_t)i * out.ncls + c] = newid[P.blk[d.trans[(size_t)s * k + col_rep[c]]]];
  }
  return out;
}

}
```

cilium_amd/csrc/clsdfa.h:

```cpp
#pragma once

#include <cstddef>
#include <cstdint>
#include <vector>

namespace cg {

struct ClsDfa {
  int ncls = 1;
  uint8_t clsmap[256] = {0};
  std::vector<int32_t> trans;
  std::vector<uint32_t> label;
  int size() const { return (int)label.size(); }
  int next(int s, uint8_t b) const { return trans[(size_t)s * ncls + clsmap[b]]; }
};

ClsDfa minimize_cls(const ClsDfa& d);

}
```

cilium_amd/csrc/dev_types.h:

```cpp
#pragma once

#include <hip/hip_vector_types.h>

#include <cstddef>
#include <cstdint>
#include <cstring>

#include "../../include/cilium_gpu.h"

#if defined(__HIP__) || defined(__HIPCC__)
#define CG_HD __host__ __device__
#else
#define CG_HD
#endif
#define CG_HDI CG_HD inline __attribute__((always_inline))

namespace cg {

CG_HD inline uint4 load16(const void* p) {
#if defined(__HIP_DEVICE_COMPILE__)
  return *reinterpret_cast<const uint4*>(p);
#else
  uint4 v;
  memcpy(&v, p, sizeof(v));
  return v;
#endif
}

constexpr uint64_t kL4EmptyKey = ~0ULL;
struct L4Slot {
  uint64_t key;
  uint32_t val;
  uint32_t pad;
};
struct L4Dev {
  const L4Slot* slots;
  const uint32_t* fp;
  uint32_t bucket_mask;
  uint32_t max_entries;
  unsigned long long* counters;
};

CG_HD inline uint64_t l4_hash1(uint64_t k) {
  k ^= k >> 33;
  k *= 0xff51afd7ed558ccdULL;
  k ^= k >> 33;
  k *= 0xc4ceb9fe1a85ec53ULL;
  k ^= k >> 33;
  return k;
}
CG_HD inline uint32_t l4_fin(uint32_t x) {
  x ^= x >> 15;
  x *= 0x2C1B3C6Du;
  x ^= x >> 13;
  return x;
}
constexpr uint32_t kL4MulLo = 0x9E3779B1u, kL4MulHi = 0x85EBCA77u;
CG_HD inline uint32_t l4_h(uint64_t key) {
  return l4_fin((uint32_t)key * kL4MulLo + (uint32_t)(key >> 32) * kL4MulHi);
}
CG_HD inline uint32_t l4_alt(uint32_t fp) { return (fp * 0x9E3779u) | 1u; }

CG_HD inline uint64_t l4_hash2(uint64_t k) {
  k += 0x9e3779b97f4a7c15ULL;
  k ^= k >> 30;
  k *= 0xbf58476d1ce4e5b9ULL;
  k ^= k >> 27;
  k *= 0x94d049bb133111ebULL;
  k ^= k >> 31;
  return k;
}

CG_HD inline void l4_place_h(uint32_t h, uint32_t mask, uint32_t* b1, uint32_t* b2, uint32_t* fp) {
  uint32_t f = h >> 24;
  f = f ? f : 1u;
  *fp = f;
  *b1 = h & mask;
  *b2 = *b1 ^ (l4_alt(f) & mask);
}
CG_HD inline void l4_place(uint64_t key, uint32_t mask, uint32_t* b1, uint32_t* b2, uint32_t* fp) {
  l4_place_h(l4_h(key), mask, b1, b2, fp);
}

struct L4ArrDev {
  const uint32_t* slot;
  const L4Dev* recs;
};
static_assert(sizeof(L4Dev) == 32, "the array kernel reads a record as two 16-byte loads");

constexpr uint32_t kLpmPartial = 2;
struct LpmDev {
  const uint32_t* top;
  const uint32_t* top_rank;
  const uint32_t* mid;
  const uint32_t* leaf_base;
  const uint64_t* leaves;
  const uint64_t* v6_code;
  const uint32_t* v6_mix;
  const uint64_t* v6_iv;
  uint32_t v6_bits;
  const uint32_t* ep4_keys;
  uint32_t ep4_mask;
  uint32_t ep4_zero;
  const uint64_t* ep6_keys;
  uint32_t ep6_mask;
  uint32_t ep6_zero;
  unsigned long long* counters;
};

CG_HD inline uint32_t ep_hash32(uint32_t a) { return l4_fin(a * kL4MulLo); }
CG_HD inline uint32_t ep_hash128(uint64_t hi, uint64_t lo) {
  return l4_fin((uint32_t)hi * kL4MulLo + (uint32_t)(hi >> 32) * kL4MulHi + (uint32_t)lo * 0xC2B2AE3Du +
                (uint32_t)(lo >> 32) * 0x27D4EB2Fu);
}
CG_HD inline uint32_t lpm_partials(uint32_t w) { return w & ~(w << 1) & 0xAAAAAAAAu; }
CG_HD inline uint32_t v6_code_of(uint64_t cw, uint32_t tb, uint32_t* m) {
  const uint32_t w = (uint32_t)cw, sh = 2 * (tb & 15);
  *m = (uint32_t)(cw >> 32) + (uint32_t)__builtin_popcount(lpm_partials(w) & ((1u << sh) - 1));
  return (w >> sh) & 3;
}

constexpr uint32_t kProgAllowAll = 1;
constexpr uint32_t kProgHasAlways = 2;
constexpr uint32_t kNoAcc = 0xFFFFFFFFu;
struct HttpProg {
  uint32_t part_begin;
  uint32_t part_count;
  uint32_t flags;
  uint32_t mask_words;
  uint32_t always_off;
  uint32_t default_remote;
  uint32_t cell_begin;
  uint32_t cell_count;
  uint32_t rtab_off;
  uint32_t rtab_nb;
  uint32_t rule_base;
  uint32_t nrules;
  uint32_t rdir_base, rdir_len, rdir_off, pad;
};
constexpr uint32_t kProgRemoteDirect = 16;
constexpr uint32_t kRdirMaxSpan = 8192;
constexpr uint32_t kLdsRuleHits = 512;
constexpr uint32_t kMaxLdsCells = (160 * 1024 - 64 - 4 * kLdsRuleHits - 4 * 64) / 4;
constexpr uint32_t kNoRow = 0xFFFFFFFFu;
constexpr uint32_t kProgRebased = 4;
constexpr uint32_t kProgClass = 8;
struct HttpPart {
  uint32_t cell_off;
  uint32_t ncells;
  uint32_t acc_off;
  uint32_t start;
  uint32_t nstates;
  uint32_t dead;
  uint32_t walk_off;
  uint32_t mode;
};
constexpr uint32_t kPartClass = 1;
constexpr uint32_t kProgAllow = 0xFFFFFFFEu;
constexpr uint32_t kProgDeny = 0xFFFFFFFFu;

constexpr uint32_t kBatchMagic = 0x34484743u;
constexpr uint32_t kChunkTiles = 64;
struct HttpBatchHeader {
  uint32_t magic;
  uint32_t epoch;
  uint32_t nchunks;
  uint32_t ntiles;
  uint64_t tiles_off;
  uint64_t nslots;
  uint64_t ttab_off;
  uint64_t total_bytes;
  uint64_t arena_bytes;
  uint32_t pad[2];
};
struct HttpTile {
  uint32_t at;
  uint32_t units;
};
constexpr uint32_t kTileHalfLast = 0x8000u;
CG_HD inline uint32_t tile_units(const HttpTile& t) { return t.units & 0x7FFFu; }
CG_HD inline uint32_t tile_tail(const HttpTile& t) { return t.units >> 16; }
CG_HD inline bool tile_half(const HttpTile& t) { return (t.units & kTileHalfLast) != 0; }
CG_HD inline uint32_t tile_granules(const HttpTile& t) { return 1 + 2 * tile_units(t) - (tile_half(t) ? 1u : 0u); }
struct HttpChunk {
  uint32_t prog;
  uint32_t first_tile;
  uint32_t ntiles;
  uint32_t pad;
};
struct HttpDev {
  const HttpProg* progs;
  const HttpPart* parts;
  const uint32_t* cells;
  const uint32_t* dflt;
  uint32_t npolicies;
  uint32_t nprogs;
  uint32_t nparts;
  uint32_t epoch;
  uint32_t lds_cells;
  uint32_t n_global_progs;
  unsigned long long* counters;
  unsigned long long* rule_hits;
};

constexpr uint32_t kRawMaxFields = 32;
constexpr uint32_t kRawMaxHead = 61440;
constexpr uint32_t kRawKeys = 10;
constexpr uint32_t kFieldsMaxList = 65535;
struct HttpRawDev {
  const uint32_t* phash_keys;
  const uint32_t* phash_vals;
  uint32_t phash_mask;
  uint32_t npolicies;
  const uint32_t* dflt;
  const HttpProg* progs;
  uint32_t nprogs;
  uint32_t nfields;
  int32_t f_method, f_path, f_authority;
  uint32_t fmask;
  const uint32_t* fslots;
  const uint8_t* fnames;
  const uint8_t* codes;
  const uint32_t* nkeys;
  uint32_t nkmask;
  uint32_t fnames_bytes;
  const uint32_t* walk_bits;
  uint32_t raw_values;
  int32_t f_empty;
};
CG_HD inline uint32_t raw_name_hash(uint32_t nl, uint32_t lo0, uint32_t lo1, uint32_t hi0, uint32_t hi1) {
  uint32_t x = lo0 ^ (lo1 << 7 | lo1 >> 25) ^ (hi0 << 13 | hi0 >> 19) ^ (hi1 << 21 | hi1 >> 11) ^ nl;
  x ^= x >> 16;
  return ((x & 0xFFFFFFu) * 0x9E3779u) ^ (x >> 11);
}
CG_HD inline uint32_t raw_fnv(uint32_t h, uint8_t c) { return (h ^ c) * 16777619u; }
constexpr uint32_t kRawFnvInit = 2166136261u;
struct RawReqs {
  const uint8_t* raw;
  const uint64_t* off;
  const uint32_t* policy;
  const uint8_t* ingress;
  const uint16_t* port;
  const uint32_t* remote;
  size_t n;
  RawReqs at(size_t a, size_t m) const { return {raw, off + a, policy + a, ingress + a, port + a, remote + a, m}; }
};
constexpr uint32_t kRingReqs = 256;
constexpr uint32_t kRingBlob = 32 * 1024;
constexpr size_t kRingOut = 64, kRingData = kRingOut + kRingReqs;
struct RingLayout {
  uint32_t rem, port, ing, off, blob;
};
CG_HD inline RingLayout ring_layout(uint32_t n) {
  RingLayout L;
  L.rem = 4 * n;
  L.port = 8 * n;
  L.ing = L.port + ((2 * n + 3) & ~3u);
  L.off = L.ing + ((n + 3) & ~3u);
  L.blob = (L.off + 4 * (n + 1) + 15) & ~15u;
  return L;
}
constexpr size_t kRingDataMax = ((15 * kRingReqs + 4 + 16) & ~(size_t)15) + kRingBlob;
constexpr size_t kRingSlotBytes = (kRingData + kRingDataMax + 255) & ~(size_t)255;
static_assert(kRingData % 16 == 0, "the data is copied in 16-byte units");
constexpr uint32_t kRingStop = 0, kRingCtlBytes = 256;
constexpr size_t kRingReplyBytes = 512;
static_assert(kRingOut + kRingReqs <= kRingReplyBytes, "reply slot");
struct HttpRingDev {
  uint8_t* slots;
  uint8_t* reply;
  uint32_t reply_stride;
  uint32_t* ctl;
  uint32_t nslots, nwg;
  uint64_t idle_ticks;
  uint64_t life_ticks;
  uint32_t lds_cells;
  uint32_t trace;
  uint32_t echo;
  uint32_t lds_tabs;
};
constexpr uint32_t kRingStampAt = 8, kRingStamps = 7;

struct HttpRawRun {
  uint32_t t0, units, base, prog;
  uint32_t send;
};

constexpr uint32_t kRawUnits = 9;
constexpr uint32_t kRawTileGran = 1 + 2 * 8;
constexpr uint32_t kRawScanThreads = 256;
constexpr uint32_t kRawCntStride = 64;
enum : uint32_t {
  kRawCtlChunks = 0,
  kRawCtlWalk = 1,
  kRawCtlDefer = 2,
  kRawCtlError = 3,
  kRawCtlLate = 4,
  kRawCtlWords = 16
};
struct RawLayoutDev {
  uint32_t* kcnt;
  unsigned long long* dir;
  HttpChunk* chunks;
  HttpTile* ttab;
  uint8_t* tiles;
  uint32_t* order;
  uint32_t* ctl;
  uint32_t* walk;
  uint32_t* dlist;
  unsigned long long* late;
  uint32_t dpk, ext, cshift;
  uint32_t seq, maxchunks, nkeys;
  uint32_t spin;
  uint32_t stripes;
};
CG_HD inline uint32_t raw_vkey(const RawLayoutDev& L, uint32_t k, uint32_t b) { return k * L.stripes + (b & (L.stripes - 1u)); }

CG_HD inline uint32_t hash32(uint32_t x) {
  x ^= x >> 16;
  x *= 0x7feb352dU;
  x ^= x >> 15;
  x *= 0x846ca68bU;
  x ^= x >> 16;
  return x;
}
template <class P>
CG_HDI uint32_t lookup_prog(P phk, P phv, P dflt, uint32_t phash_mask, uint32_t npolicies, uint32_t policy,
                            bool ingress, uint32_t port) {
  if (policy >= npolicies) return kProgDeny;
  const uint32_t key = (policy << 17) | ((uint32_t)ingress << 16) | (port & 0xFFFF);
  uint32_t h = hash32(key) & phash_mask;
  for (uint32_t probe = 0; probe <= phash_mask; ++probe) {
    const uint32_t kk = phk[h];
    if (kk == key) return phv[h];
    if (kk == 0xFFFFFFFFu) break;
    h = (h + 1) & phash_mask;
  }
  return dflt[policy * 2 + (ingress ? 1 : 0)];
}
constexpr uint32_t kRtabBucketCells = 8;
CG_HD inline uint32_t mul24(uint32_t a, uint32_t b) {
#if defined(__HIP_DEVICE_COMPILE__)
  return __umul24(a, b);
#else
  return (a & 0xFFFFFFu) * (b & 0xFFFFFFu);
#endif
}
CG_HD inline uint32_t mulhi24(uint32_t a, uint32_t b) {
  return (uint32_t)(((uint64_t)(a & 0xFFFFFFu) * (b & 0xFFFFFFu)) >> 32);
}
CG_HD inline uint32_t rtab_hash(uint32_t id) {
  const uint32_t a = id ^ (id >> 15);
  return mul24(a, 0x9E3779u) ^ (a >> 17);
}
CG_HD inline uint32_t rtab_b1h(uint32_t h, uint32_t nb) { return mulhi24(h, nb << 8); }
CG_HD inline uint32_t rtab_b2h(uint32_t h, uint32_t nb) {
  return mulhi24(mul24(h ^ (h >> 11), 0x85EBCBu) >> 8, nb << 8);
}
CG_HD inline uint32_t rtab_b1(uint32_t id, uint32_t nb) { return rtab_b1h(rtab_hash(id), nb); }
CG_HD inline uint32_t rtab_b2(uint32_t id, uint32_t nb) { return rtab_b2h(rtab_hash(id), nb); }

CG_HD inline uint32_t hash64to32(uint64_t k) {
  k = l4_hash1(k);
  return (uint32_t)k;
}

struct KafkaRuleDev {
  unsigned long long keys;
  uint32_t flags;
  int32_t version;
  uint32_t client_id;
  uint32_t pad;
};
constexpr uint32_t kKfKeyWild = 1, kKfVerWild = 2, kKfHasClient = 4, kKfHasTopic = 8;
CG_HD inline uint32_t kf_hash(uint64_t k) {
  return l4_fin((uint32_t)k * kL4MulLo + (uint32_t)(k >> 32) * kL4MulHi);
}
constexpr uint32_t kKfBuckets = 65;
constexpr uint32_t kKfSumsPerGroup = 2 * kKfBuckets;
struct KafkaSumDev {
  unsigned long long vm[3];
  uint32_t any;
  uint32_t x_off, x_cnt;
  uint32_t pad;
};
constexpr uint32_t kKfSumHasClients = 8;
struct KafkaClientDev {
  unsigned long long key;
  unsigned long long vm;
  uint32_t any, pad[3];
};
struct KafkaGroupSlot {
  unsigned long long key;
  uint32_t group, pad;
};
struct KafkaTopicDev {
  unsigned long long key;
  uint32_t off, cnt;
};
struct KafkaDev {
  const KafkaSumDev* sums;
  const KafkaRuleDev* rules;
  const KafkaTopicDev* thash;
  uint32_t thash_mask;
  const KafkaClientDev* chash;
  uint32_t chash_mask;
  const KafkaGroupSlot* ghash;
  uint32_t ghash_mask;
  const uint32_t* dflt_group;
  uint32_t nredirects;
  unsigned long long* counters;
};

constexpr uint32_t kKfDictSlotWords = 8;
struct KafkaDictDev {
  const uint32_t* slots;
  const uint8_t* blob;
  uint32_t mask, pad;
};
constexpr uint32_t kKfDictEmpty = 0xFFFFFFFFu;
CG_HD inline uint32_t kf_fnv1a(const uint8_t* p, uint32_t n) {
  uint32_t h = 2166136261u;
  for (uint32_t i = 0; i < n; ++i) h = (h ^ p[i]) * 16777619u;
  return h;
}

constexpr uint32_t kWorldId = 2;
constexpr uint64_t kIpcMiss = kWorldId;
struct alignas(8) IpcVal {
  uint32_t identity;
  uint32_t tunnel;
};
struct IpcacheDev {
  const uint32_t* l16x;
  const uint64_t* chunks;
  const uint64_t* code6;
  const uint32_t* ent6;
  const uint8_t* crowd6;
  const uint64_t* runs6;
  uint32_t v6_bits;
  uint32_t nruns6;
  const uint32_t* ex4;
  const uint64_t* ex6;
  uint32_t ex4_mask, ex6_mask, ex4_probes, ex6_probes;
};
constexpr uint32_t kIpcExact = 1u << 17;
// ... 370 lines not shown
```

cilium_amd/csrc/http.cc:

```cpp
#include "http.h"

#include <algorithm>
#include <array>
#include <cstdio>
#include <cstdlib>
#include <atomic>
#include <cstring>
#include <functional>
#include <map>
#include <random>
#include <set>
#include <unordered_map>

#include "clsdfa.h"
#include "comb.h"
#include "http_walk.h"
#include "json.h"
#include "regex.h"

namespace cg {

namespace {

constexpr uint8_t kSep = 0x00;
// ... 286 lines not shown
    }
  }
  int ncls = 0;
  for (int b = 0; b < 256; ++b) ncls = std::max(ncls, cls[b] + 1);
  std::vector<int> rep(ncls, -1);
  for (int b = 0; b < 256; ++b)
    if (rep[cls[b]] < 0) rep[cls[b]] = b;

  ClsDfa d;
  d.ncls = ncls;
  for (int b = 0; b < 256; ++b) d.clsmap[b] = (uint8_t)cls[b];
  std::unordered_map<std::vector<uint64_t>, int, VecHash64> ids;
  std::vector<std::vector<uint64_t>> states;
  std::map<std::vector<uint64_t>, uint32_t> mask_ids;
  label_masks.clear();

  auto label_of = [&](const std::vector<uint64_t>& st) -> uint32_t {
    if ((int)st[0] != F) return 0;
    std::vector<uint64_t> m(W, 0);
    for (size_t i = 1; i < st.size(); ++i)
      for (uint32_t t : all_rules[(size_t)(st[i] >> 32)].tags) m[t >> 6] |= 1ULL << (t & 63);
    uint32_t kept_group = 0xFFFFFFFFu;
    for (uint32_t b = 0; b < 64 * W; ++b) {
      if (!((m[b >> 6] >> (b & 63)) & 1)) continue;
      if (group[b] == kept_group) m[b >> 6] &= ~(1ULL << (b & 63));
      else kept_group = group[b];
    }
    auto it = mask_ids.emplace(m, (uint32_t)mask_ids.size() + 1);
    if (it.second) label_masks.push_back(m);
    return it.first->second;
  };
  auto intern = [&](std::vector<uint64_t>&& st) -> int {
    if (st.size() == 1) return 0;
    auto it = ids.find(st);
    if (it != ids.end()) return it->second;
    int id = (int)states.size();
    if (id >= kMaxUnionStates) throw TooBig{};
    ids.emplace(st, id);
    d.label.push_back(label_of(st));
    states.push_back(std::move(st));
    d.trans.resize((size_t)(id + 1) * ncls, 0);
    return id;
  };
  states.push_back({(uint64_t)-1});
  d.label.push_back(0);
  d.trans.assign(ncls, 0);
  {
    std::vector<uint64_t> st{0};
    for (int r : rules) {
      if (F == 0) {
        st.push_back((uint64_t)r << 32 | 1);
      } else {
        st.push_back((uint64_t)r << 32 | (uint32_t)fc.dfas[all_rules[r].fd[0]].start);
      }
    }
    if (F == 0) st[0] = 0;
    if (st.size() == 1) {
      states.push_back({(uint64_t)-2});
      d.label.push_back(0);
      d.trans.resize(2 * ncls, 0);
    } else {
      int id = (int)states.size();
      ids.emplace(st, id);
      d.label.push_back(label_of(st));
      states.push_back(st);
      d.trans.resize((size_t)(id + 1) * ncls, 0);
    }
  }
  std::vector<uint64_t> nx;
  for (size_t si = 1; si < states.size(); ++si) {
    if (states[si][0] == (uint64_t)-2) break;
    const int f = (int)states[si][0];
    for (int c = 0; c < ncls; ++c) {
      int b = rep[c];
      int target = 0;
      if (f < F) {
        const std::vector<uint64_t>& cur = states[si];
        nx.clear();
        if (b == kRestAbsent) {
          nx.push_back((uint64_t)F);
          for (size_t i = 1; i < cur.size(); ++i) {
            uint32_t r = (uint32_t)(cur[i] >> 32), q = (uint32_t)cur[i];
            bool ok = true;
            for (int g = f; g < F && ok; ++g) {
              const ByteDfa& fd = fc.dfas[all_rules[r].fd[g]];
              const int s1 = fd.next(g == f ? (int)q : fd.start, kAbsent);
              ok = s1 != 0 && fd.accept[s1];
            }
            if (ok) nx.push_back((uint64_t)r << 32 | 1u);
          }
        } else if (b == kSep) {
          nx.push_back((uint64_t)(f + 1));
          for (size_t i = 1; i < cur.size(); ++i) {
            uint32_t r = (uint32_t)(cur[i] >> 32), q = (uint32_t)cur[i];
            const ByteDfa& fd = fc.dfas[all_rules[r].fd[f]];
            if (!fd.accept[q]) continue;
            uint32_t nq = (f + 1 < F) ? (uint32_t)fc.dfas[all_rules[r].fd[f + 1]].start : 1u;
            nx.push_back((uint64_t)r << 32 | nq);
          }
        } else {
          nx.push_back((uint64_t)f);
          for (size_t i = 1; i < cur.size(); ++i) {
            uint32_t r = (uint32_t)(cur[i] >> 32), q = (uint32_t)cur[i];
            int nq = fc.dfas[all_rules[r].fd[f]].next((int)q, b);
            if (nq) nx.push_back((uint64_t)r << 32 | (uint32_t)nq);
          }
        }
        target = intern(std::vector<uint64_t>(nx));
      }
      d.trans[si * ncls + c] = target;
    }
  }
  return d;
}

struct PartOut {
  ClsDfa dfa;
  CombTable comb;
  std::vector<std::vector<uint64_t>> label_masks;
};

void build_parts(const FieldDfaCache& fc, const std::vector<URule>& all_rules, std::vector<int> rules,
                 int F, uint32_t W, const std::vector<uint32_t>& group, std::vector<PartOut>& out) {
  if (rules.empty()) return;
  PartOut p;
  bool ok = true;
  try {
    ClsDfa raw = build_union(fc, all_rules, rules, F, W, group, p.label_masks);
    p.dfa = minimize_cls(raw);
    std::vector<uint32_t> labels(p.dfa.size(), kCombNoLabel);
    for (int s = 0; s < p.dfa.size(); ++s)
      if (p.dfa.label[s]) labels[s] = p.dfa.label[s] - 1;
    if (p.dfa.size() > kMaxPartStates || p.label_masks.size() >= kCombNoLabel ||
        !build_comb(p.dfa, labels, &p.comb))
      ok = false;
  } catch (const TooBig&) {
    ok = false;
  }
  if (ok) {
    if (getenv("CILIUM_GPU_DEBUG"))
      fprintf(stderr, "[cilium-gpu] http part: %zu rules, %d states, %d byte classes, %zu comb cells\n", rules.size(),
              p.dfa.size(), p.dfa.ncls, p.comb.cells.size());
    out.push_back(std::move(p));
    return;
  }
  if (rules.size() == 1) fail(CG_UNSUPPORTED, "a single HTTP rule exceeds the DFA state budget");
  std::vector<int> a(rules.begin(), rules.begin() + rules.size() / 2);
  std::vector<int> b(rules.begin() + rules.size() / 2, rules.end());
  build_parts(fc, all_rules, a, F, W, group, out);
  build_parts(fc, all_rules, b, F, W, group, out);
}

}

uint32_t http_next_epoch() {
  static std::atomic<uint32_t> g_epoch{0};
  return ++g_epoch;
}

std::shared_ptr<HttpSnapshot> http_compile(const char* json, size_t len) {
  std::vector<PolicySpec> pols = parse_npds(json, len);
  auto snap = std::make_shared<HttpSnapshot>();
  HttpSnapshot& S = *snap;
  S.epoch = http_next_epoch();
  if (pols.size() >= 0x7FFF) fail(CG_POLICY_REJECTED, "too many policies");

  std::set<std::string> names;
  for (const auto& p : pols)
    for (int d = 0; d < 2; ++d)
      for (const auto& [port, sc] : p.dir[d])
        for (const auto& pr : sc.rules)
          for (const auto& hr : pr.http)
            for (const auto& m : hr) names.insert(m.name);
  for (const char* pseudo : {":method", ":path", ":authority"})
    if (names.count(pseudo)) {
      S.fields.push_back(pseudo);
      names.erase(pseudo);
    }
  for (const auto& n : names) S.fields.push_back(n);
  const int F = (int)S.fields.size();
  std::map<std::string, int> field_idx;
  for (int i = 0; i < F; ++i) field_idx[S.fields[i]] = i;

  FieldDfaCache fc;
  {
    size_t nraw = 0;
    for (const auto& p : pols) nraw += p.deny_unlisted;
    if (nraw && nraw != pols.size())
      fail(CG_POLICY_REJECTED, "proxylib and Envoy HTTP policies cannot share one snapshot");
    S.raw_values = fc.raw = nraw != 0;
  }
  S.npolicies = (uint32_t)pols.size();
  S.dflt.assign((size_t)S.npolicies * 2, kProgAllow);
  std::vector<std::pair<uint32_t, uint32_t>> phash;


  auto build_prog = [&](const std::vector<const ScopeSpec*>& scopes, uint32_t key, uint32_t pol_idx,
                        uint32_t ingress, uint32_t port) -> uint32_t {
    HttpProg pg{};
    uint32_t pid = (uint32_t)S.progs.size();
    struct Bit {
      const PnprSpec* pnpr;
      uint32_t scope, pnpr_idx, http_idx;
    };
    std::vector<Bit> bits;
    std::vector<uint32_t> pnpr_first;
    std::vector<const PnprSpec*> pnprs;
    for (uint32_t si = 0; si < scopes.size(); ++si) {
      const ScopeSpec* sc = scopes[si];
      bool have_http = false;
      for (const auto& r : sc->rules) have_http |= r.has_http;
      if (!have_http || sc->rules.empty()) {
        if (si == 0) {
          pg.flags = kProgAllowAll;
          S.progs.push_back(pg);
          S.prog_key.push_back(key);
          return pid;
        }
        bits.push_back({nullptr, si, 0, CG_HTTP_RULE_SCOPE_ALLOW});
        break;
      }
      for (uint32_t ri = 0; ri < sc->rules.size(); ++ri) {
        const PnprSpec& r = sc->rules[ri];
        pnprs.push_back(&r);
        pnpr_first.push_back((uint32_t)bits.size());
        if (r.http.empty()) bits.push_back({&r, si, ri, CG_HTTP_RULE_NO_HTTP});
        for (uint32_t hi = 0; hi < r.http.size(); ++hi) bits.push_back({&r, si, ri, hi});
      }
    }
    const uint32_t R = (uint32_t)bits.size();
    const uint32_t W = (R + 63) / 64;
    pg.mask_words = W;
    pg.rule_base = (uint32_t)S.rule_info.size();
    pg.nrules = R;
    for (const Bit& b : bits) S.rule_info.push_back({pol_idx, ingress, port, b.scope, b.pnpr_idx, b.http_idx});
    std::vector<uint64_t> always(W, 0), open(W, 0);
    std::map<uint32_t, std::vector<uint64_t>> by_remote;
    for (uint32_t j = 0; j < R; ++j) {
      const Bit& b = bits[j];
      if (!b.pnpr || b.pnpr->http.empty()) always[j >> 6] |= 1ULL << (j & 63);
      if (!b.pnpr || !b.pnpr->has_remotes) open[j >> 6] |= 1ULL << (j & 63);
    }
    for (uint32_t j = 0; j < R; ++j) {
      const Bit& b = bits[j];
      if (!b.pnpr || !b.pnpr->has_remotes) continue;
      for (uint64_t rid : b.pnpr->remotes) {
        if (rid > 0xFFFFFFFFULL) continue;
        auto it = by_remote.find((uint32_t)rid);
        if (it == by_remote.end()) it = by_remote.emplace((uint32_t)rid, open).first;
        it->second[j >> 6] |= 1ULL << (j & 63);
      }
    }
    for (uint64_t w : always)
      if (w) pg.flags |= kProgHasAlways;
    std::vector<URule> urules;
    std::map<std::vector<int>, size_t> dedupe;
    for (uint32_t j = 0; j < (uint32_t)pnprs.size(); ++j) {
      uint32_t bit = pnpr_first[j];
      for (const auto& hr : pnprs[j]->http) {
        const uint32_t tag = bit++;
        std::vector<std::vector<const MatcherSpec*>> per_field(F);
        for (const auto& m : hr) per_field[field_idx[m.name]].push_back(&m);
        std::vector<int> fd(F);
        bool empty = false;
        for (int f = 0; f < F; ++f) {
          fd[f] = fc.conj(per_field[f]);
          if (fc.empty_lang(fd[f])) empty = true;
        }
        if (empty) continue;
        auto it = dedupe.find(fd);
        if (it == dedupe.end()) {
          dedupe[fd] = urules.size();
          urules.push_back({fd, {tag}});
        } else {
          urules[it->second].tags.push_back(tag);
        }
      }
    }
    S.total_rules += urules.size();
    std::vector<int> idx(urules.size());
    for (size_t i = 0; i < idx.size(); ++i) idx[i] = (int)i;
    std::vector<PartOut> parts;
    std::vector<uint32_t> group(64 * (size_t)W, 0xFFFFFFFEu);
    for (uint32_t j = 0; j < R; ++j) group[j] = (j && bits[j].pnpr == bits[j - 1].pnpr) ? group[j - 1] : j;
    build_parts(fc, urules, idx, F, W, group, parts);
    std::array<uint8_t, 256> code{};
    if (parts.size() == 1 && parts[0].dfa.ncls <= 64) {
      ClsDfa z = zero_class_first(parts[0].dfa);
      std::vector<uint32_t> labels(z.size(), kCombNoLabel);
      for (int st = 0; st < z.size(); ++st)
        if (z.label[st]) labels[st] = z.label[st] - 1;
      CombTable cc;
      if (build_comb(z, labels, &cc, kCombMaxBase, true) && scale_comb(&cc)) {
        parts[0].dfa = std::move(z);
        parts[0].comb = std::move(cc);
        pg.flags |= kProgClass;
        for (int b = 0; b < 256; ++b) code[b] = (uint8_t)(4 * parts[0].dfa.clsmap[b]);
      }
    }
    if (pg.flags & kProgClass) {
      S.prog_code.resize(pid + 1);
      S.prog_code[pid] = code;
    }
    pg.part_begin = (uint32_t)S.parts.size();
    pg.part_count = (uint32_t)parts.size();
    while (S.cells.size() & 3) S.cells.push_back(kCombEmpty);
    pg.cell_begin = (uint32_t)S.cells.size();
    size_t block = 0;
    for (const auto& po : parts) block += po.comb.cells.size();
    const bool rebase = block <= kCombMaxBase;
    if (rebase) pg.flags |= kProgRebased;
    for (auto& po : parts) {
      HttpPart hp{};
      const ClsDfa& d = po.dfa;
      CombTable& cb = po.comb;
      hp.cell_off = (uint32_t)S.cells.size();
      if (rebase) rebase_comb(&cb, hp.cell_off - pg.cell_begin);
      hp.walk_off = rebase ? pg.cell_begin : hp.cell_off;
      hp.nstates = (uint32_t)d.size();
      hp.start = cb.start;
      hp.dead = cb.dead;
      hp.ncells = (uint32_t)cb.cells.size();
      hp.mode = cb.scaled ? kPartClass : 0;
      S.cells.insert(S.cells.end(), cb.cells.begin(), cb.cells.end());
      S.total_states += d.size();
      S.total_exceptions += cb.exceptions;
      S.parts.push_back(hp);
    }
    auto put_mask = [&](const std::vector<uint64_t>& m) -> uint32_t {
      if (S.cells.size() & 1) S.cells.push_back(0);
      const uint32_t off = (uint32_t)S.cells.size() - pg.cell_begin;
      for (uint64_t w : m) {
        S.cells.push_back((uint32_t)w);
        S.cells.push_back((uint32_t)(w >> 32));
      }
      return off;
    };
    for (size_t i = 0; i < parts.size(); ++i) {
      HttpPart& hp = S.parts[pg.part_begin + i];
      if (S.cells.size() & 1) S.cells.push_back(0);
      hp.acc_off = (uint32_t)S.cells.size() - pg.cell_begin;
      for (size_t l = 0; l < parts[i].label_masks.size(); ++l) put_mask(parts[i].label_masks[l]);
    }
    pg.always_off = put_mask(always);
    {
      std::map<std::vector<uint64_t>, uint32_t> rows;
      auto row_of = [&](const std::vector<uint64_t>& m) {
        auto it = rows.find(m);
        if (it == rows.end()) it = rows.emplace(m, put_mask(m)).first;
        return it->second;
      };
      pg.default_remote = row_of(open);
      std::vector<std::pair<uint32_t, uint32_t>> ent;
      for (auto& [rid, m] : by_remote) ent.push_back({rid, row_of(m)});
      uint32_t nb = (uint32_t)std::max<size_t>((ent.size() * 10 / 9 + 3) / 4, 1);
      std::vector<std::pair<uint32_t, uint32_t>> slots;
      for (;; nb += nb / 8 + 1) {
        if (nb >= 65536) fail(CG_POLICY_REJECTED, "too many remote identities in one HTTP policy scope");
        slots.assign((size_t)nb * 4, {0u, kNoRow});
        std::mt19937 rng(0xC111A);
        auto put = [&](uint32_t bk, const std::pair<uint32_t, uint32_t>& e) {
          for (int sl = 0; sl < 4; ++sl)
            if (slots[(size_t)bk * 4 + sl].second == kNoRow) {
              slots[(size_t)bk * 4 + sl] = e;
              return true;
            }
          return false;
        };
        bool ok = true;
        for (const auto& e : ent) {
          auto cur = e;
          uint32_t from = 0xFFFFFFFFu;
          bool placed = false;
          for (int kick = 0; kick < 500 && !placed; ++kick) {
            const uint32_t c1 = rtab_b1(cur.first, nb), c2 = rtab_b2(cur.first, nb);
            if (put(c1, cur) || put(c2, cur)) {
              placed = true;
              break;
            }
            const uint32_t vb = c1 == from ? c2 : c2 == from ? c1 : (rng() & 1) ? c1 : c2;
            std::swap(cur, slots[(size_t)vb * 4 + (rng() & 3)]);
            from = vb;
          }
          if (!placed) {
            ok = false;
            break;
          }
        }
        if (ok) break;
      }
      while ((S.cells.size() - pg.cell_begin) & 3) S.cells.push_back(0);

      pg.rtab_off = (uint32_t)S.cells.size() - pg.cell_begin;
      pg.rtab_nb = nb;
      uint32_t empty_id = 0;
      while (by_remote.count(empty_id)) ++empty_id;
      const size_t at = S.cells.size();
      S.cells.resize(at + kRtabBucketCells * (size_t)nb, 0);
      for (uint32_t k = 0; k < nb; ++k)
        for (int sl = 0; sl < 4; ++sl) {
          const auto& e = slots[(size_t)k * 4 + sl];
          const bool empty = e.second == kNoRow;
          S.cells[at + kRtabBucketCells * k + sl] = empty ? empty_id : e.first;
          S.cells[at + kRtabBucketCells * k + 4 + sl] = empty ? pg.default_remote : e.second;
        }
      const uint32_t cap = 4 * nb;
      S.total_remote_slots += cap;
      if (!ent.empty()) {
        uint32_t lo = ent[0].first, hi = ent[0].first;
        bool rows16 = pg.default_remote < 0x10000;
        for (const auto& e : ent) {
          lo = std::min(lo, e.first);
          hi = std::max(hi, e.first);
          rows16 &= e.second < 0x10000;
        }
        if (rows16 && hi - lo < kRdirMaxSpan) {
          const uint32_t len = hi - lo + 1;
          std::vector<uint16_t> t(len + 1, (uint16_t)pg.default_remote);
          for (const auto& e : ent) t[e.first - lo] = (uint16_t)e.second;
          pg.rdir_base = lo;
          pg.rdir_len = len;
          pg.rdir_off = (uint32_t)S.cells.size() - pg.cell_begin;
          for (uint32_t k = 0; k < len; k += 2) S.cells.push_back((uint32_t)t[k] | (uint32_t)t[k + 1] << 16);
          pg.flags |= kProgRemoteDirect;
        }
      }
    }
    S.cells.push_back(0);
    S.cells.push_back(0);
    pg.cell_count = (uint32_t)S.cells.size() - pg.cell_begin;
    if (getenv("CILIUM_GPU_DEBUG")) {
      size_t comb = 0, labels = 0;
      for (uint32_t i = 0; i < pg.part_count; ++i) {
        comb += S.parts[pg.part_begin + i].ncells;
        labels += parts[i].label_masks.size();
      }
      fprintf(stderr, "[cilium-gpu] http program %u: block %u cells (comb %zu, %zu labels x %u words, remote table %u "
              "buckets, direct %u)\n", pid, pg.cell_count, comb, labels, 2 * pg.mask_words, pg.rtab_nb, pg.rdir_len);
    }
    S.progs.push_back(pg);
    S.prog_key.push_back(key);
    return pid;
  };

  for (uint32_t pi = 0; pi < pols.size(); ++pi) {
    const PolicySpec& p = pols[pi];
    S.policy_index[p.name] = pi;
    for (int d = 0; d < 2; ++d) {
      const auto& ports = p.dir[d];
      const ScopeSpec* wild = nullptr;
      auto w = ports.find(0);
      if (w != ports.end()) wild = &w->second;
      if (p.deny_unlisted) S.dflt[pi * 2 + d] = kProgDeny;
      if (wild) S.dflt[pi * 2 + d] = build_prog({wild}, (pi << 17) | ((uint32_t)d << 16), pi, d, 0);
      for (const auto& [port, sc] : ports) {
        if (port == 0) continue;
        if (port > 0xFFFF) continue;
        std::vector<const ScopeSpec*> scs{&sc};
        if (wild) scs.push_back(wild);
        uint32_t key = (pi << 17) | ((uint32_t)d << 16) | port;
        phash.push_back({key, build_prog(scs, key, pi, d, port)});
      }
    }
  }

  {
    uint32_t cap = next_pow2(std::max<size_t>(2 * phash.size(), 16));
    S.phash_keys.assign(cap, 0xFFFFFFFFu);
    S.phash_vals.assign(cap, 0);
    S.phash_mask = cap - 1;
    for (auto [k, v] : phash) {
      uint32_t h = hash32(k) & S.phash_mask;
      while (S.phash_keys[h] != 0xFFFFFFFFu) h = (h + 1) & S.phash_mask;
      S.phash_keys[h] = k;
      S.phash_vals[h] = v;
    }
  }
  if (S.cells.empty()) S.cells.push_back(kCombEmpty);
  if (S.progs.empty()) S.progs.push_back(HttpProg{});
  S.prog_code.resize(S.progs.size());
  if (S.parts.empty()) S.parts.push_back(HttpPart{});
  if (S.dflt.empty()) S.dflt.push_back(kProgDeny);
  return snap;
}

HttpDev HttpSnapshot::view(bool device) const {
  HttpDev d{};
  d.progs = device ? d_progs.as<HttpProg>() : progs.data();
  d.parts = device ? d_parts.as<HttpPart>() : parts.data();
  d.cells = device ? d_cells.as<uint32_t>() : cells.data();
  d.dflt = device ? d_dflt.as<uint32_t>() : dflt.data();
  d.npolicies = npolicies;
  d.nprogs = (uint32_t)progs.size();
  d.nparts = (uint32_t)parts.size();
  d.epoch = epoch;
  uint32_t max_cells = 0;
  d.lds_cells = kMaxLdsCells;
  for (const auto& pg : progs)
    if (walk::prog_in_lds(d, pg, walk::prog_walked(true, pg))) max_cells = std::max(max_cells, pg.cell_count);
  d.lds_cells = std::min((max_cells + 255) & ~255u, kMaxLdsCells);
  for (const auto& pg : progs)
    if (walk::prog_walked(true, pg) && !walk::prog_in_lds(d, pg, true)) d.n_global_progs++;
  d.counters = device ? d_counters.as<unsigned long long>() : nullptr;
  d.rule_hits = device ? d.counters + 2 * (size_t)d.nprogs + 1 : nullptr;
  return d;
}

void HttpSnapshot::upload(Engine& e) {
  if (!e.has_gpu()) return;
  d_progs.upload_vec(progs);
  d_parts.upload_vec(parts);
  d_cells.upload_vec(cells);
  d_dflt.upload_vec(dflt);
  d_counters.alloc((std::max<size_t>(progs.size(), 1) * 2 + 1 + rule_info.size()) * sizeof(uint64_t));
  d_counters.zero();
  dev = view(true);
  http_raw_upload(*this);
}

}
```

cilium_amd/csrc/http.h:

```cpp
#pragma once

#include <array>
#include <map>
#include <memory>
#include <string>
#include <vector>

#include "dev_types.h"
#include "engine.h"

namespace cg {

struct HttpSnapshot {
  std::vector<std::string> fields;
  bool raw_values = false;
  std::map<std::string, uint32_t> policy_index;
  uint32_t npolicies = 0;

  std::vector<HttpProg> progs;
  std::vector<HttpPart> parts;
  std::vector<uint32_t> cells;
  std::vector<uint32_t> phash_keys, phash_vals;
  uint32_t phash_mask = 0;
  std::vector<uint32_t> dflt;
  std::vector<uint32_t> prog_key;
  std::vector<std::array<uint8_t, 256>> prog_code;
  std::vector<cg_http_rule_info> rule_info;

  uint32_t epoch = 0;
  uint64_t total_states = 0;
  uint64_t total_exceptions = 0;
  uint64_t total_rules = 0;
  uint64_t total_remote_slots = 0;

  DevMem d_progs, d_parts, d_cells, d_dflt, d_counters;
  HttpDev dev{};
  DevMem d_phk, d_phv, d_fslots, d_fnames, d_codes, d_nkeys, d_walk;
  HttpRawDev raw{};
  bool raw_ok = false, lists_ok = false;
  LaunchFence fence;

  HttpDev view(bool device) const;
  HttpDev host_view() const { return view(false); }
  void upload(Engine& e);
  uint32_t lookup_prog(uint32_t policy, bool ingress, uint32_t port) const {
    return cg::lookup_prog(phash_keys.data(), phash_vals.data(), dflt.data(), phash_mask, npolicies, policy, ingress,
                           port);
  }
};

std::shared_ptr<HttpSnapshot> http_compile(const char* json, size_t len);
uint32_t http_next_epoch();
std::vector<uint8_t> http_image_export(const HttpSnapshot& s);
std::shared_ptr<HttpSnapshot> http_image_import(const uint8_t* p, size_t n);

std::string npds_pb_to_json(const uint8_t* p, size_t n, bool strict_utf8);

enum class RawInput { Heads, Lists };
void http_raw_upload(HttpSnapshot& S);
void http_verdicts_raw_on(const HttpSnapshot& s, StagingSlot& sl, int cus, RawInput in, const uint8_t* d_raw,
                          const uint64_t* d_off, size_t n, const uint32_t* d_policy, const uint8_t* d_ingress,
                          const uint16_t* d_port, const uint32_t* d_remote, uint8_t* d_out, void* stream);

size_t http_batch_slots(const HttpSnapshot& s, size_t n);
size_t http_batch_bytes(const HttpSnapshot& s, size_t n);

void http_pack(const HttpSnapshot& s, size_t n, const uint32_t* policy, const uint8_t* ingress,
               const uint16_t* port, const uint32_t* remote, const uint8_t* hdr_blob,
               const uint64_t* hdr_off, void* batch, size_t batch_cap, uint32_t* order, size_t* nslots,
               uint8_t* arena, size_t arena_cap, size_t* arena_used);

void http_eval_host(const HttpSnapshot& s, const uint8_t* batch, size_t nslots, const uint8_t* arena,
                    size_t arena_len, uint8_t* out, uint32_t* rule = nullptr);

}
```

cilium_amd/csrc/http_image.cc:

```cpp
#include <cstring>
#include <string>
#include <vector>

#include "comb.h"
#include "http.h"

namespace cg {

namespace {

constexpr uint32_t kImageMagic = 0x49484743u;
constexpr uint32_t kImageVersion = 1u | (uint32_t)sizeof(HttpProg) << 8 | (uint32_t)sizeof(HttpPart) << 16 |
                                   (uint32_t)sizeof(cg_http_rule_info) << 24;

uint64_t fnv64(const uint8_t* p, size_t n) {
  uint64_t h = 1469598103934665603ull;
  for (size_t i = 0; i < n; ++i) h = (h ^ p[i]) * 1099511628211ull;
  return h;
}

struct Writer {
  std::vector<uint8_t> b;
  void raw(const void* p, size_t n) {
    const uint8_t* q = static_cast<const uint8_t*>(p);
    b.insert(b.end(), q, q + n);
  }
  void u32(uint32_t v) { raw(&v, 4); }
  void u64(uint64_t v) { raw(&v, 8); }
  void str(const std::string& s) {
    u32((uint32_t)s.size());
    raw(s.data(), s.size());
  }
  template <class T>
  void vec(const std::vector<T>& v) {
    u64(v.size());
    raw(v.data(), v.size() * sizeof(T));
  }
};

struct Reader {
  const uint8_t* p;
  const uint8_t* e;
  void raw(void* dst, size_t n) {
    if ((size_t)(e - p) < n) fail(CG_POLICY_REJECTED, "policy image: truncated");
    memcpy(dst, p, n);
    p += n;
  }
  uint32_t u32() {
    uint32_t v;
    raw(&v, 4);
    return v;
  }
  uint64_t u64() {
    uint64_t v;
    raw(&v, 8);
    return v;
  }
  std::string str() {
    const uint32_t n = u32();
    if ((size_t)(e - p) < n) fail(CG_POLICY_REJECTED, "policy image: truncated");
    std::string s((const char*)p, n);
    p += n;
    return s;
  }
  template <class T>
  void vec(std::vector<T>* v) {
    const uint64_t n = u64();
    if (n > (uint64_t)(e - p) / sizeof(T)) fail(CG_POLICY_REJECTED, "policy image: truncated");
    v->resize((size_t)n);
    raw(v->data(), (size_t)n * sizeof(T));
  }
};

}

std::vector<uint8_t> http_image_export(const HttpSnapshot& s) {
  Writer w;
  w.u32(kImageMagic);
  w.u32(kImageVersion);
  w.u32(s.raw_values ? 1u : 0u);
  w.u32((uint32_t)s.fields.size());
  for (const auto& f : s.fields) w.str(f);
  w.u32((uint32_t)s.policy_index.size());
  for (const auto& [name, idx] : s.policy_index) {
    w.str(name);
    w.u32(idx);
  }
  w.u32(s.npolicies);
  w.vec(s.progs);
  w.vec(s.parts);
  w.vec(s.cells);
  w.vec(s.phash_keys);
  w.vec(s.phash_vals);
  w.u32(s.phash_mask);
  w.vec(s.dflt);
  w.vec(s.prog_key);
  w.vec(s.prog_code);
  w.vec(s.rule_info);
  w.u64(s.total_states);
  w.u64(s.total_exceptions);
  w.u64(s.total_rules);
  w.u64(s.total_remote_slots);
  w.u64(fnv64(w.b.data(), w.b.size()));
  return std::move(w.b);
}

void validate_image(const HttpSnapshot& s) {
  auto bad = [](const char* what) { fail(CG_POLICY_REJECTED, std::string("policy image: ") + what); };
  const size_t np = s.progs.size(), nc = s.cells.size();
  auto prog_ref_ok = [&](uint32_t v) { return v < np || v == kProgAllow || v == kProgDeny; };
  if (s.phash_keys.size() != (size_t)s.phash_mask + 1 || s.phash_vals.size() != s.phash_keys.size())
    bad("bad program hash");
  bool empty_slot = false;
  for (size_t i = 0; i < s.phash_keys.size(); ++i) {
    empty_slot |= s.phash_keys[i] == 0xFFFFFFFFu;
    if (s.phash_keys[i] != 0xFFFFFFFFu && !prog_ref_ok(s.phash_vals[i])) bad("program hash value out of range");
  }
  if (!empty_slot) bad("program hash has no empty slot");
  if (s.dflt.size() < (size_t)s.npolicies * 2 || s.prog_code.size() != np || s.prog_key.size() > np)
    bad("inconsistent tables");
  for (uint32_t v : s.dflt)
    if (!prog_ref_ok(v)) bad("default program out of range");
  for (const auto& [name, idx] : s.policy_index)
    if (idx >= s.npolicies) bad("policy index out of range");
  for (size_t pi = 0; pi < np; ++pi) {
    const HttpProg& pg = s.progs[pi];
    if ((size_t)pg.part_begin + pg.part_count > s.parts.size() || (size_t)pg.cell_begin + pg.cell_count > nc)
      bad("program out of range");
    if (pg.flags & kProgAllowAll) continue;
    const uint64_t W = pg.mask_words, blk = pg.cell_count;
    if (W == 0 || W > (1u << 16)) bad("bad mask width");
    if ((uint64_t)pg.rule_base + pg.nrules > s.rule_info.size() || pg.nrules > 64 * W) bad("rule range out of range");
    const uint32_t* b = s.cells.data() + pg.cell_begin;
    auto mask_ok = [&](uint64_t o, bool check_bits) {
      if (o + 2 * W > blk) return false;
      if (check_bits)
        for (uint64_t w = 0; w < W; ++w) {
          const uint64_t m = (uint64_t)b[o + 2 * w] | (uint64_t)b[o + 2 * w + 1] << 32;
          for (uint32_t bit = 0; bit < 64; ++bit)
            if (((m >> bit) & 1) && w * 64 + bit >= pg.nrules) return false;
        }
      return true;
    };
    if (!mask_ok(pg.always_off, true) || !mask_ok(pg.default_remote, false)) bad("program mask out of range");
    if (pg.flags & kProgRemoteDirect) {
      if (pg.rdir_len > kRdirMaxSpan || (uint64_t)pg.rdir_off + (pg.rdir_len + 1) / 2 > blk)
        bad("remote direct array out of range");
      const uint16_t* d = (const uint16_t*)(b + pg.rdir_off);
      for (uint32_t i = 0; i < pg.rdir_len; ++i)
        if (!mask_ok(d[i], false)) bad("remote row out of range");
    } else {
      if (pg.rtab_nb == 0 || (uint64_t)pg.rtab_off + (uint64_t)kRtabBucketCells * pg.rtab_nb > blk)
        bad("remote table out of range");
      for (uint32_t k = 0; k < pg.rtab_nb; ++k)
        for (uint32_t sl = 0; sl < 4; ++sl) {
          const uint32_t* bk = b + pg.rtab_off + kRtabBucketCells * k;
          if (bk[sl] != kNoRow && !mask_ok(bk[4 + sl], false)) bad("remote row out of range");
        }
    }
    uint32_t max_code = 255;
    if (pg.flags & kProgClass) {
      max_code = 0;
      for (uint8_t c : s.prog_code[pi]) {
        if (c & 3) bad("class code not a cell offset");
        max_code = std::max<uint32_t>(max_code, c);
      }
    }
    const bool rebased = pg.flags & kProgRebased;
    const uint64_t limit = rebased ? (uint64_t)pg.cell_begin + pg.cell_count : nc;
    for (uint32_t k = 0; k < pg.part_count; ++k) {
      const HttpPart& pt = s.parts[pg.part_begin + k];
      if (pt.mode != 0 && pt.mode != kPartClass) bad("bad part mode");
      const bool scaled = pt.mode == kPartClass;
      if (scaled != ((pg.flags & kProgClass) != 0)) bad("class mode mismatch");
      if ((rebased && pt.walk_off != pg.cell_begin) || pt.cell_off < pt.walk_off ||
          (uint64_t)pt.cell_off + pt.ncells > limit)
        bad("part out of range");
      auto state_ok = [&](uint64_t st) {
        if (scaled && (st & 3)) return false;
        const uint64_t lo = scaled ? st >> 2 : st, hi = scaled ? (st + max_code) >> 2 : st + 255;
        return lo >= 1 && pt.walk_off + hi < limit;
      };
      if (!state_ok(pt.start) || !state_ok(pt.dead)) bad("part state out of range");
      for (uint64_t i = pt.cell_off; i < (uint64_t)pt.cell_off + pt.ncells; ++i) {
        const uint32_t c = s.cells[i];
        if (c == kCombEmpty) continue;
        if ((c & 0xFFFF) == 0xFFFF) {
          const uint32_t lab = c >> 16;
          if (lab != kCombNoLabel && !mask_ok((uint64_t)pt.acc_off + (uint64_t)lab * 2 * W, true))
            bad("accept label out of range");
        } else if (!state_ok(c >> 16)) {
          bad("transition out of range");
        }
      }
    }
  }
}

std::shared_ptr<HttpSnapshot> http_image_import(const uint8_t* p, size_t n) {
  if (!p || n < 16) fail(CG_POLICY_REJECTED, "policy image: too short");
  uint64_t sum;
  memcpy(&sum, p + n - 8, 8);
  if (sum != fnv64(p, n - 8)) fail(CG_POLICY_REJECTED, "policy image: checksum mismatch");
  Reader r{p, p + n - 8};
  if (r.u32() != kImageMagic) fail(CG_POLICY_REJECTED, "policy image: bad magic");
  if (r.u32() != kImageVersion) fail(CG_POLICY_REJECTED, "policy image: built by another library version");
  auto snap = std::make_shared<HttpSnapshot>();
  HttpSnapshot& s = *snap;
  s.raw_values = r.u32() != 0;
  const uint32_t nf = r.u32();
  if (nf > (1u << 20)) fail(CG_POLICY_REJECTED, "policy image: bad field count");
  for (uint32_t i = 0; i < nf; ++i) s.fields.push_back(r.str());
  const uint32_t np = r.u32();
  for (uint32_t i = 0; i < np; ++i) {
    std::string name = r.str();
    s.policy_index[name] = r.u32();
  }
  s.npolicies = r.u32();
  r.vec(&s.progs);
  r.vec(&s.parts);
  r.vec(&s.cells);
  r.vec(&s.phash_keys);
  r.vec(&s.phash_vals);
  s.phash_mask = r.u32();
  r.vec(&s.dflt);
  r.vec(&s.prog_key);
  r.vec(&s.prog_code);
  r.vec(&s.rule_info);
  s.total_states = r.u64();
  s.total_exceptions = r.u64();
  s.total_rules = r.u64();
  s.total_remote_slots = r.u64();
  if (r.p != r.e) fail(CG_POLICY_REJECTED, "policy image: trailing bytes");
  validate_image(s);
  s.epoch = http_next_epoch();
  return snap;
}

}
```

cilium_amd/csrc/http_pack.cc:

```cpp
#include <algorithm>
#include <chrono>
#include <cstdio>
#include <vector>
#include <exception>
#include <cstdlib>
#include <mutex>
#include <thread>
#include <type_traits>
#include <atomic>
#include <cstddef>
#include <array>
#include <cstring>
#include <map>
#include <string>

#include "comb.h"
#include "http.h"
#include "http_walk.h"

namespace cg {

namespace {

constexpr uint8_t kSep = 0x00;
constexpr uint8_t kAbsent = 0x01;
constexpr uint8_t kRestAbsent = 0x02;

inline bool codec_rejects(uint8_t c) { return (c < 0x20 && c != 0x09) || c == 0x7F; }
constexpr size_t kUnitBytes = (size_t)CG_HTTP_TILE * 16;
constexpr size_t kMetaBytes = (size_t)CG_HTTP_TILE * CG_HTTP_META_BYTES;
constexpr size_t kGranule = 512;
constexpr size_t kMaxTileBytes = kMetaBytes + (size_t)(CG_HTTP_UNITS - 1) * kUnitBytes;

inline size_t tile_unit_at(const HttpTile& t, uint32_t u, size_t lane) {
  const bool half = u && u == tile_units(t) && tile_half(t);
  return (size_t)t.at * kGranule +
         (u ? kMetaBytes + (size_t)(u - 1) * kUnitBytes + lane * (half ? 8 : 16) : lane * CG_HTTP_META_BYTES);
}

bool name_eq_ci(const uint8_t* a, size_t an, const std::string& lower_b) {
  if (an != lower_b.size()) return false;
  for (size_t i = 0; i < an; ++i) {
    uint8_t c = a[i];
    if (c >= 'A' && c <= 'Z') c = c - 'A' + 'a';
    if (c != (uint8_t)lower_b[i]) return false;
  }
  return true;
}

size_t max_groups(const HttpSnapshot& s, size_t n) { return std::min(n, s.progs.size() + 2); }

size_t ttab_off(size_t max_tiles) { return sizeof(HttpBatchHeader) + sizeof(HttpChunk) * max_tiles; }
size_t header_bytes(size_t max_tiles) {
  size_t b = ttab_off(max_tiles) + sizeof(HttpTile) * max_tiles;
  return (b + 1023) & ~(size_t)1023;
}

}

size_t http_batch_slots(const HttpSnapshot& s, size_t n) {
  return ((n + CG_HTTP_TILE - 1) / CG_HTTP_TILE + max_groups(s, n)) * CG_HTTP_TILE;
}

size_t http_batch_bytes(const HttpSnapshot& s, size_t n) {
  size_t tiles = http_batch_slots(s, n) / CG_HTTP_TILE;
  return header_bytes(tiles) + tiles * kMaxTileBytes;
}

namespace {

unsigned pack_threads(size_t n) {
  if (n < 16384) return 1;
  static const unsigned t = [] {
    if (const char* e = getenv("CILIUM_GPU_PACK_THREADS")) {
      const long v = strtol(e, nullptr, 10);
      if (v >= 1 && v <= 256) return (unsigned)v;
    }
    return std::max(1u, std::min(16u, std::thread::hardware_concurrency()));
  }();
  return t;
}

template <class F>
void parallel_ranges(size_t n, unsigned nt, F&& fn) {
  if (nt <= 1 || n == 0) {
    fn((size_t)0, n, 0u);
    return;
  }
  std::vector<std::thread> th;
  std::exception_ptr err;
  std::mutex mu;
  for (unsigned t = 0; t < nt; ++t) {
    const size_t a = n * t / nt, b = n * (t + 1) / nt;
    th.emplace_back([&, a, b, t] {
      try {
        fn(a, b, t);
      } catch (...) {
        std::lock_guard<std::mutex> lk(mu);
        if (!err) err = std::current_exception();
      }
    });
  }
  for (auto& x : th) x.join();
  if (err) std::rethrow_exception(err);
}

template <class F>
void parallel_items(size_t n, unsigned nt, F&& fn) {
  std::atomic<size_t> next{0};
  parallel_ranges(nt, nt, [&](size_t, size_t, unsigned) {
    for (size_t i; (i = next.fetch_add(1)) < n;) fn(i);
  });
}

}

void http_pack(const HttpSnapshot& s, size_t n, const uint32_t* policy, const uint8_t* ingress,
               const uint16_t* port, const uint32_t* remote, const uint8_t* hdr_blob,
               const uint64_t* hdr_off, void* batch, size_t batch_cap, uint32_t* order, size_t* nslots_out,
               uint8_t* arena, size_t arena_cap, size_t* arena_used) {
  const unsigned nt = pack_threads(n);
  const bool build = batch || arena_used;
  const bool dbg = getenv("CILIUM_GPU_PACK_DEBUG") != nullptr;
  auto t0 = std::chrono::steady_clock::now();
  auto lap = [&](const char* what) {
    if (!dbg) return;
    auto t1 = std::chrono::steady_clock::now();
    fprintf(stderr, "[pack] %-10s %8.1f ms\n", what, std::chrono::duration<double, std::milli>(t1 - t0).count());
    t0 = t1;
  };
  const size_t np = s.progs.size();
  auto group_of = [&](uint32_t p) -> size_t { return p < np ? p : np + (p == kProgAllow ? 0 : 1); };
  auto prog_of_group = [&](size_t g) -> uint32_t { return g < np ? (uint32_t)g : g == np ? kProgAllow : kProgDeny; };
  const size_t F = s.fields.size();
  std::vector<std::vector<uint8_t>> sbuf(nt);
  std::vector<uint32_t> prog(n), soff(n), slen(n);
  std::vector<uint8_t> malformed(n, 0);
  std::vector<std::vector<size_t>> gcount(nt, std::vector<size_t>(np + 2, 0));
  std::vector<std::vector<uint32_t>> by_len;
  for (size_t f = 0; f < F; ++f) {
    const size_t L = s.fields[f].size();
    if (by_len.size() <= L) by_len.resize(L + 1);
    by_len[L].push_back((uint32_t)f);
  }
  auto worker_of = [&](size_t i) -> unsigned {
    unsigned t = (unsigned)((i * nt) / n);
    while (t + 1 < nt && i >= n * (t + 1) / nt) ++t;
    while (t > 0 && i < n * t / nt) --t;
    return t;
  };
  parallel_ranges(n, nt, [&](size_t a, size_t b, unsigned t) {
    std::vector<uint8_t>& strs = sbuf[t];
    if (build) strs.reserve((b - a) * 64);
    std::vector<const uint8_t*> vp(F);
    std::vector<size_t> vl(F);
    for (size_t i = a; i < b; ++i) {
      prog[i] = policy[i] >= s.npolicies ? kProgDeny : s.lookup_prog(policy[i], ingress[i] != 0, port[i]);
      gcount[t][group_of(prog[i])]++;
      if (!build) continue;
      std::fill(vp.begin(), vp.end(), nullptr);
      const uint8_t* p = hdr_blob + hdr_off[i];
      const uint8_t* e = hdr_blob + hdr_off[i + 1];
      while (p < e) {
        const uint8_t* nm = p;
        while (p < e && *p) ++p;
        size_t nl = p - nm;
        if (p < e) ++p;
        const uint8_t* v = p;
        while (p < e && *p) ++p;
        size_t vlen = p - v;
        if (p < e) ++p;
        if (s.raw_values) {
          for (size_t k = 0; k < vlen; ++k) {
            if (v[k] <= 0x02) malformed[i] = 1;
            if (v[k] == 0x03) {
              if (k + 1 >= vlen || v[k + 1] < 0x10 || v[k + 1] > 0x14) malformed[i] = 1;
              ++k;
            }
          }
        } else {
          for (size_t k = 0; k < vlen; ++k)
            if (codec_rejects(v[k])) malformed[i] = 1;
        }
        if (nl < by_len.size())
          for (uint32_t f : by_len[nl])
            if (!vp[f] && name_eq_ci(nm, nl, s.fields[f])) {
              vp[f] = v;
              vl[f] = vlen;
            }
      }
      const size_t o = strs.size();
      size_t last = 0;
      for (size_t f = 0; f < F; ++f)
        if (vp[f]) last = f + 1;
      for (size_t f = 0; f < last; ++f) {
        if (!vp[f]) strs.push_back(kAbsent);
        else strs.insert(strs.end(), vp[f], vp[f] + vl[f]);
        strs.push_back(kSep);
      }
      if (last < F) strs.push_back(kRestAbsent);
      if (strs.size() - o > 0xFFFFFFFFull) fail(CG_INVALID_ARGUMENT, "request string beyond 4 GiB");
      soff[i] = (uint32_t)o;
      slen[i] = (uint32_t)(strs.size() - o);
      if (strs.size() > 0xFFFFFFFFull) fail(CG_INVALID_ARGUMENT, "packer buffer beyond 4 GiB per worker");
      if (prog[i] < np && (s.progs[prog[i]].flags & kProgClass)) {
        const auto& code = s.prog_code[prog[i]];
        for (size_t k = o; k < strs.size(); ++k) strs[k] = code[strs[k]];
      }
    }
  });
  std::vector<const uint8_t*> sp(build ? n : 0);
  if (build)
    parallel_ranges(n, nt, [&](size_t a, size_t b, unsigned t) {
      for (size_t i = a; i < b; ++i) sp[i] = sbuf[t].data() + soff[i];
    });
  lap("strings");
  auto str_ptr = [&](size_t i) -> const uint8_t* { return sp[i]; };
  auto str_len = [&](size_t i) -> size_t { return build ? slen[i] : 0; };
  auto walked_units = [&](size_t i) -> uint32_t {
    const size_t len = str_len(i);
    if (malformed[i] || len > CG_HTTP_SLOT_BYTES) return 0;
    return (uint32_t)((len + 15) / 16);
  };
  std::vector<size_t> count(np + 2, 0);
  for (unsigned t = 0; t < nt; ++t)
    for (size_t g = 0; g < np + 2; ++g) count[g] += gcount[t][g];
  std::vector<size_t> first_slot(np + 2, 0);
  std::vector<HttpChunk> chunks;
  size_t tiles = 0;
  for (size_t g = 0; g < np + 2; ++g) {
    if (!count[g]) continue;
    first_slot[g] = tiles * CG_HTTP_TILE;
    size_t t = (count[g] + CG_HTTP_TILE - 1) / CG_HTTP_TILE;
    for (size_t k = 0; k < t; k += kChunkTiles)
      chunks.push_back({prog_of_group(g), (uint32_t)(tiles + k), (uint32_t)std::min<size_t>(kChunkTiles, t - k), 0});
    tiles += t;
  }
  const size_t nslots = tiles * CG_HTTP_TILE;
  if (nslots_out) *nslots_out = nslots;
  constexpr size_t kKeys = CG_HTTP_UNITS + 2;
  auto key_of = [&](size_t i) -> size_t {
    const size_t len = str_len(i);
    return len > CG_HTTP_SLOT_BYTES ? CG_HTTP_UNITS + 1 : (len + 15) / 16;
  };
  std::vector<size_t> bstart((np + 2) * kKeys + 1, 0);
  for (size_t i = 0; i < n; ++i) bstart[group_of(prog[i]) * kKeys + key_of(i) + 1]++;
  for (size_t k = 1; k < bstart.size(); ++k) bstart[k] += bstart[k - 1];
  lap("buckets");
  std::vector<uint32_t> idx(n);
  {
    std::vector<size_t> fill(bstart.begin(), bstart.end() - 1);
    for (size_t i = 0; i < n; ++i) idx[fill[group_of(prog[i]) * kKeys + key_of(i)]++] = (uint32_t)i;
  }
  lap("idx");
  if (build) {
    struct Rec {
      uint32_t len, i;
      uint64_t pre[4];
      uint64_t rest;
    };
    std::vector<size_t> buckets;
    for (size_t k = 0; k + 1 < bstart.size(); ++k)
      if (bstart[k + 1] - bstart[k] > 1) buckets.push_back(k);
    std::sort(buckets.begin(), buckets.end(),
              [&](size_t a, size_t b) { return bstart[a + 1] - bstart[a] > bstart[b + 1] - bstart[b]; });
    parallel_items(buckets.size(), nt, [&](size_t bi) {
      const size_t k = buckets[bi];
      std::vector<Rec> r(bstart[k + 1] - bstart[k]);
      for (size_t j = 0; j < r.size(); ++j) {
        const uint32_t i = idx[bstart[k] + j];
        const uint8_t* q = sp[i];
        const size_t L = slen[i];
        Rec& e = r[j];
        for (int w = 0; w < 4; ++w) {
          uint64_t x = 0;
          for (size_t c = 8 * w; c < 8 * w + 8; ++c) x = x << 8 | (c < L ? q[c] : 0);
          e.pre[w] = x;
        }
        uint64_t h = 1469598103934665603ull;
        for (size_t c = 32; c < L; ++c) h = (h ^ q[c]) * 1099511628211ull;
        e.rest = h;
        e.i = i;
        e.len = (uint32_t)L;
      }
      std::sort(r.begin(), r.end(), [](const Rec& a, const Rec& b) {
        if (a.len != b.len) return a.len < b.len;
        for (int w = 0; w < 4; ++w)
          if (a.pre[w] != b.pre[w]) return a.pre[w] < b.pre[w];
        if (a.rest != b.rest) return a.rest < b.rest;
        return a.i < b.i;
      });
      for (size_t j = 0; j < r.size(); ++j) idx[bstart[k] + j] = r[j].i;
    });
  }
  lap("sort");
  std::vector<uint32_t> slot_of(n);
  std::vector<uint32_t> req_of_slot(nslots, 0xFFFFFFFFu);
  for (size_t g = 0; g < np + 2; ++g) {
    size_t pos = first_slot[g];
    for (size_t r = bstart[g * kKeys]; r < bstart[(g + 1) * kKeys]; ++r) {
      slot_of[idx[r]] = (uint32_t)pos;
      req_of_slot[pos] = idx[r];
      ++pos;
    }
  }
  std::vector<HttpTile> ttab(tiles);
  std::vector<uint8_t> half_ok(tiles, 0);
  for (const HttpChunk& c : chunks) {
    const bool ok = c.prog < np && !(s.progs[c.prog].flags & kProgAllowAll) && s.progs[c.prog].part_count == 1 &&
                    (s.progs[c.prog].flags & kProgRebased) && s.progs[c.prog].cell_count <= kMaxLdsCells;
    std::fill(half_ok.begin() + c.first_tile, half_ok.begin() + c.first_tile + c.ntiles, (uint8_t)ok);
  }
  parallel_ranges(tiles, nt, [&](size_t a, size_t b, unsigned) {
    for (size_t k = a; k < b; ++k) {
      uint32_t units = 0, tail = 0;
      for (size_t l = 0; l < CG_HTTP_TILE; ++l) {
        const uint32_t i = req_of_slot[k * CG_HTTP_TILE + l];
        if (i != 0xFFFFFFFFu) units = std::max(units, walked_units(i));
      }
      for (size_t l = 0; l < CG_HTTP_TILE && units; ++l) {
        const uint32_t i = req_of_slot[k * CG_HTTP_TILE + l];
        if (i != 0xFFFFFFFFu && walked_units(i) == units)
          tail = std::max<uint32_t>(tail, (uint32_t)(str_len(i) - 16 * (units - 1)));
      }
      if (units && !tail) tail = 16;
      ttab[k].units = units | (units && tail <= 8 && half_ok[k] ? kTileHalfLast : 0u) | tail << 16;
    }
  });
  lap("ttab");
  uint64_t gran = 0;
  for (auto& t : ttab) {
    if (gran > 0xFFFFFFFFull) fail(CG_INVALID_ARGUMENT, "batch beyond 2 TiB");
    t.at = (uint32_t)gran;
    gran += tile_granules(t);
  }
  const size_t max_tiles = http_batch_slots(s, n) / CG_HTTP_TILE;
  const size_t hdr = header_bytes(max_tiles);
  const size_t need = hdr + gran * kGranule;
  if (batch && need > batch_cap) fail(CG_INVALID_ARGUMENT, "batch buffer too small");
  uint8_t* data = batch ? (uint8_t*)batch + hdr : nullptr;
  auto unit_ptr = [&](size_t slot, uint32_t u) {
    return data + tile_unit_at(ttab[slot / CG_HTTP_TILE], u, slot % CG_HTTP_TILE);
  };
  std::vector<uint64_t> aoff(n, ~0ull);
  size_t used = 0;
  for (size_t i = 0; i < n && build; ++i) {
    const size_t len = str_len(i);
    if (len <= CG_HTTP_SLOT_BYTES) continue;
    if (used / 16 >= (1u << 24)) fail(CG_INVALID_ARGUMENT, "overflow arena beyond 256 MiB");
    aoff[i] = used;
    used += (4 + len + 15) & ~(size_t)15;
  }
  if (batch) {
    HttpBatchHeader h{};
    h.magic = kBatchMagic;
    h.epoch = s.epoch;
    h.nchunks = (uint32_t)chunks.size();
    h.ntiles = (uint32_t)tiles;
    h.tiles_off = hdr;
    h.nslots = nslots;
    h.ttab_off = ttab_off(max_tiles);
    h.total_bytes = need;
    h.arena_bytes = used;
    memcpy(batch, &h, sizeof(h));
    memcpy((uint8_t*)batch + sizeof(h), chunks.data(), chunks.size() * sizeof(HttpChunk));
    memcpy((uint8_t*)batch + h.ttab_off, ttab.data(), ttab.size() * sizeof(HttpTile));
  }
  if (order)
    for (size_t sl = 0; sl < nslots; ++sl) order[sl] = req_of_slot[sl];
  if (batch || (arena && build)) {
    parallel_ranges(tiles, nt, [&](size_t a, size_t b, unsigned) {
      for (size_t k = a; k < b; ++k) {
        if (batch) memset(data + (size_t)ttab[k].at * kGranule, 0, (size_t)tile_granules(ttab[k]) * kGranule);
        for (size_t l = 0; l < CG_HTTP_TILE; ++l) {
          const size_t sl = k * CG_HTTP_TILE + l;
          const uint32_t i = req_of_slot[sl];
          if (i == 0xFFFFFFFFu) {
            if (batch) unit_ptr(sl, 0)[7] = CG_HTTP_F_PAD;
            continue;
          }
          const uint8_t* str = str_ptr(i);
          const uint32_t len = (uint32_t)str_len(i);
          uint8_t meta[CG_HTTP_META_BYTES] = {0};
          memcpy(meta, &remote[i], 4);
          uint8_t flags = ingress[i] ? CG_HTTP_F_INGRESS : 0;
          if (malformed[i]) flags |= CG_HTTP_F_MALFORMED;
          if (len > CG_HTTP_SLOT_BYTES) {
            flags |= CG_HTTP_F_OVERFLOW;
            const uint64_t o = aoff[i];
            if (arena && o + 4 + len <= arena_cap) {
              memcpy(arena + o, &len, 4);
              memcpy(arena + o + 4, str, len);
            }
            const uint32_t off16 = (uint32_t)(o / 16);
            meta[4] = off16 & 0xFF;
            meta[5] = (off16 >> 8) & 0xFF;
            meta[6] = (off16 >> 16) & 0xFF;
          }
          meta[7] = flags;
          if (batch) {
            memcpy(unit_ptr(sl, 0), meta, CG_HTTP_META_BYTES);
            const uint32_t wu = walked_units(i);
            const HttpTile& tt = ttab[k];
            for (uint32_t u = 0; u < wu; ++u) {
              const size_t cap = u + 1 == tile_units(tt) && tile_half(tt) ? 8 : 16;
              memcpy(unit_ptr(sl, u + 1), str + u * 16, std::min<size_t>(cap, len - u * 16));
            }
          }
        }
      }
    });
  }
  lap("write");
  if (arena_used) *arena_used = used;
  if (arena && used > arena_cap) fail(CG_INVALID_ARGUMENT, "overflow arena too small");
}

void http_eval_host(const HttpSnapshot& s, const uint8_t* batch, size_t nslots, const uint8_t* arena,
                    size_t arena_len, uint8_t* out, uint32_t* rule) {
  using namespace walk;
  const HttpDev T = s.host_view();
  HttpBatchHeader h;
  memcpy(&h, batch, sizeof(h));
  if (h.magic != kBatchMagic || h.epoch != T.epoch) fail(CG_INVALID_ARGUMENT, "batch packed for another snapshot");
  if ((size_t)h.ntiles * CG_HTTP_TILE > nslots) fail(CG_INVALID_ARGUMENT, "batch of more slots than given");
  const HttpChunk* chunks = (const HttpChunk*)(batch + sizeof(h));
  const HttpTile* ttab = (const HttpTile*)(batch + h.ttab_off);
  bool inside = sizeof(h) + (uint64_t)h.nchunks * sizeof(HttpChunk) <= h.total_bytes &&
                h.ttab_off <= h.total_bytes && h.tiles_off <= h.total_bytes &&
                (uint64_t)h.ntiles * sizeof(HttpTile) <= h.total_bytes - h.ttab_off;
  for (uint32_t t = 0; inside && t < h.ntiles; ++t)
    inside = ((uint64_t)ttab[t].at + tile_granules(ttab[t])) * kGranule <= h.total_bytes - h.tiles_off;
  if (!inside) fail(CG_INVALID_ARGUMENT, "batch tables or tiles past its end");
  const uint64_t arena_bytes = std::min<uint64_t>(h.arena_bytes, arena_len);

  std::fill(out, out + nslots, (uint8_t)0);
  if (rule) std::fill(rule, rule + nslots, kNoHit);
  for (uint32_t c = 0; c < h.nchunks; ++c) {
    const HttpChunk ch = chunks[c];
    if (!chunk_ok(ch, h.ntiles)) continue;
    const uint32_t prog = ch.prog;
    const bool real = prog < T.nprogs;
    HttpProg pg{};
    if (real) pg = T.progs[prog];
    const bool walkp = prog_walked(real, pg);
    const bool generic = !(prog_in_lds(T, pg, walkp) && pg.part_count == 1);
    const uint32_t* blk = T.cells + pg.cell_begin;
    const bool rebased = pg.flags & kProgRebased;
    const uint32_t W = pg.mask_words;
    for (uint32_t t = ch.first_tile; t < ch.first_tile + ch.ntiles; ++t) {
      const HttpTile tt = ttab[t];
      const uint8_t* tile = batch + h.tiles_off + (size_t)tt.at * kGranule;
      const bool half = tile_half(tt);
      const uint32_t units = generic ? tile_units(tt) : std::min<uint32_t>(tile_units(tt), CG_HTTP_UNITS - 1);
      for (uint32_t lane = 0; lane < CG_HTTP_TILE; ++lane) {
        const size_t sl = (size_t)t * CG_HTTP_TILE + lane;
        uint2 meta;
        memcpy(&meta, tile + lane * CG_HTTP_META_BYTES, sizeof(meta));
        const bool counted = slot_counted(meta.y);
        if (!walkp) out[sl] = counted && trivial_allows(prog, real);
        if (!walkp || !counted || (generic && half)) continue;
        const uint32_t row = remote_row(blk, pg, meta.x);
        auto part_hit = [&](auto cls, const HttpPart& pt, const uint32_t* cells) {
          constexpr bool kCls = decltype(cls)::value;
          uint32_t st = pt.start;
          for (uint32_t u = 0; u < units && st != pt.dead; ++u) {
            const uint8_t* up = tile + kMetaBytes + (size_t)u * kUnitBytes;
            uint4 unit = make_uint4(0, 0, 0, 0);
            if (half && u + 1 == units) memcpy(&unit, up + lane * 8, 8);
            else unit = load16(up + lane * 16);
            for (int k = 0; k < 16; ++k) st = step<kCls>(cells, pt.dead, st, get_byte(unit, k));
          }
          if (slot_overflow(meta.y)) st = walk_overflow<kCls>(cells, pt.dead, pt.start, arena, arena_bytes, meta, true);
          const uint32_t lab = state_label<kCls>(cells, st);
          return lab != 0xFFFFu ? first_meet(blk, pt.acc_off + lab * 2 * W, row, W) : kNoHit;
        };
        uint32_t hit = kNoHit;
        for (uint32_t pi = 0; pi < pg.part_count; ++pi) {
          const HttpPart pt = T.parts[pg.part_begin + pi];
          const uint32_t* cells = rebased ? blk : T.cells + pt.walk_off;
          hit = std::min(hit, pt.mode == kPartClass ? part_hit(std::true_type{}, pt, cells)
                                                    : part_hit(std::false_type{}, pt, cells));
        }
        if (pg.flags & kProgHasAlways) hit = std::min(hit, first_meet(blk, pg.always_off, row, W));
        out[sl] = hit != kNoHit;
        if (rule && hit != kNoHit) rule[sl] = pg.rule_base + hit;
      }
    }
  }
}

}

extern "C" uint32_t cg_http_pack_threads(void) { return cg::pack_threads((size_t)1 << 20); }
```

include/cilium_gpu.h:

```cpp
#ifndef CILIUM_GPU_H
#define CILIUM_GPU_H

#include <stddef.h>
#include <stdint.h>

#ifdef __cplusplus
extern "C" {
#endif

typedef enum {
  CG_OK = 0,
  CG_POLICY_DROP = 1,
  CG_PARSER_ERROR = 2,
  CG_UNKNOWN_PARSER = 3,
  CG_UNKNOWN_CONNECTION = 4,
  CG_INVALID_ADDRESS = 5,
  CG_INVALID_INSTANCE = 6,
  CG_UNKNOWN_ERROR = 7,
  CG_INVALID_ARGUMENT = 16,
  CG_NO_DEVICE = 17,
  CG_DEVICE_ERROR = 18,
  CG_POLICY_REJECTED = 19,
  CG_REVISION_MISMATCH = 20,
  CG_MAP_FULL = 21,
// ... 138 lines not shown

#define CG_PF_DYN4 0x1u
#define CG_PF_DYN6 0x2u
#define CG_PF_FIX4 0x4u
#define CG_PF_FIX6 0x8u

#define CG_XDP_DROP 1
#define CG_XDP_PASS 2

int cg_prefilter_create(uint64_t h, uint32_t config, uint32_t max_lpm, uint32_t max_hash,
                        uint32_t* pf_id);
int cg_prefilter_destroy(uint64_t h, uint32_t pf_id);
int cg_prefilter_insert(uint64_t h, uint32_t pf_id, int64_t revision, const cg_cidr* cidrs,
                        size_t n, int64_t* revision_out);
int cg_prefilter_delete(uint64_t h, uint32_t pf_id, int64_t revision, const cg_cidr* cidrs,
                        size_t n, int64_t* revision_out);
int cg_prefilter_dump(uint64_t h, uint32_t pf_id, cg_cidr* out, size_t cap, size_t* n,
                      int64_t* revision);
int cg_prefilter_set_endpoints(uint64_t h, uint32_t pf_id, const uint32_t* v4_be, size_t n4,
                               const uint8_t* v6, size_t n6);
int cg_prefilter_verdicts_dev(uint64_t h, uint32_t pf_id, const uint32_t* d_v4, size_t n4,
                              uint8_t* d_out4, const uint8_t* d_v6, size_t n6, uint8_t* d_out6,
                              void* stream);
int cg_prefilter_verdicts_host(uint64_t h, uint32_t pf_id, const uint32_t* v4, size_t n4,
                               uint8_t* out4, const uint8_t* v6, size_t n6, uint8_t* out6);


typedef struct {
  uint32_t sec_label;
  uint32_t tunnel_endpoint;
} cg_remote_endpoint_info;

#define CG_WORLD_ID 2

int cg_ipcache_create(uint64_t h, uint32_t max_entries, uint32_t* ipc_id);
int cg_ipcache_destroy(uint64_t h, uint32_t ipc_id);
int cg_ipcache_update(uint64_t h, uint32_t ipc_id, const cg_cidr* keys,
                      const cg_remote_endpoint_info* values, size_t n);
int cg_ipcache_delete(uint64_t h, uint32_t ipc_id, const cg_cidr* keys, size_t n);
int cg_ipcache_lookup(uint64_t h, uint32_t ipc_id, const cg_cidr* key, cg_remote_endpoint_info* value);
int cg_ipcache_dump(uint64_t h, uint32_t ipc_id, cg_cidr* keys, cg_remote_endpoint_info* values,
                    size_t cap, size_t* n);
int cg_ipcache_resolve_dev(uint64_t h, uint32_t ipc_id, const uint32_t* d_v4, size_t n4,
                           cg_remote_endpoint_info* d_out4, const uint8_t* d_v6, size_t n6,
                           cg_remote_endpoint_info* d_out6, void* stream);
int cg_ipcache_resolve_host(uint64_t h, uint32_t ipc_id, const uint32_t* v4, size_t n4,
                            cg_remote_endpoint_info* out4, const uint8_t* v6, size_t n6,
                            cg_remote_endpoint_info* out6);

int cg_l4_verdicts_ipcache_dev(uint64_t h, uint32_t map_id, uint32_t ipc_id, const uint32_t* d_remote_v4,
                               const cg_l4_tuple* d_tuples, size_t n, int32_t* d_verdicts, void* stream);
int cg_l4_verdicts_ipcache_host(uint64_t h, uint32_t map_id, uint32_t ipc_id, const uint32_t* remote_v4,
                                const cg_l4_tuple* tuples, size_t n, int32_t* verdicts);
int cg_l4_verdicts_ipcache6_dev(uint64_t h, uint32_t map_id, uint32_t ipc_id, const uint8_t* d_remote_v6,
                                const cg_l4_tuple* d_tuples, size_t n, int32_t* d_verdicts, void* stream);
int cg_l4_verdicts_ipcache6_host(uint64_t h, uint32_t map_id, uint32_t ipc_id, const uint8_t* remote_v6,
                                 const cg_l4_tuple* tuples, size_t n, int32_t* verdicts);


int cg_proxylib_policy_update(uint64_t instance, const char* json, size_t len);

int cg_proxylib_policy_update_npds(uint64_t instance, const uint8_t* discovery_response, size_t len);

int cg_proxylib_stats(uint64_t instance, uint64_t* batches, uint64_t* calls);

int cg_proxylib_set_batching(uint64_t instance, uint32_t min_calls, uint32_t max_wait_us);


int cg_http_policy_update(uint64_t h, const char* npds_json, size_t len);
int cg_http_policy_export(uint64_t h, void* buf, size_t cap, size_t* len);
int cg_http_policy_import(uint64_t h, const void* buf, size_t len);

int cg_http_policy_update_npds(uint64_t h, const uint8_t* discovery_response, size_t len);
int cg_http_policy_index(uint64_t h, const char* name, uint32_t* index);
int cg_http_policy_stats(uint64_t h, uint64_t* out, size_t n);

typedef struct {
  uint32_t policy;
  uint32_t ingress;
  uint32_t port;
  uint32_t scope;
  uint32_t rule;
  uint32_t http_rule;
} cg_http_rule_info;
#define CG_HTTP_RULE_NO_HTTP 0xFFFFFFFFu
#define CG_HTTP_RULE_SCOPE_ALLOW 0xFFFFFFFEu
int cg_http_rule_info_get(uint64_t h, cg_http_rule_info* out, size_t cap, size_t* n);

#define CG_HTTP_TILE 64
#define CG_HTTP_UNITS 9
#define CG_HTTP_SLOT_BYTES 128
#define CG_HTTP_META_BYTES 8
size_t cg_http_batch_bytes(uint64_t h, size_t n);
size_t cg_http_batch_slots(uint64_t h, size_t n);

#define CG_HTTP_F_INGRESS 0x01u
#define CG_HTTP_F_OVERFLOW 0x02u
#define CG_HTTP_F_MALFORMED 0x04u
#define CG_HTTP_F_PAD 0x08u

uint32_t cg_http_pack_threads(void);
int cg_http_pack(uint64_t h, size_t n, const uint32_t* policy, const uint8_t* ingress,
                 const uint16_t* port, const uint32_t* remote, const uint8_t* hdr_blob,
                 const uint64_t* hdr_off, void* batch, size_t batch_cap, uint32_t* order,
                 size_t* nslots, uint8_t* arena, size_t arena_cap, size_t* arena_used);

int cg_http_parse_heads(const uint8_t* raw, const uint64_t* raw_off, size_t n, uint8_t* hdr_blob,
                        size_t blob_cap, uint64_t* hdr_off, size_t* blob_used, uint8_t* ok);

int cg_http_verdicts_raw_dev(uint64_t h, const uint8_t* d_raw, const uint64_t* d_raw_off, size_t n,
                             const uint32_t* d_policy, const uint8_t* d_ingress, const uint16_t* d_port,
                             const uint32_t* d_remote, uint8_t* d_out, void* stream);

int cg_http_verdicts_raw_host(uint64_t h, const uint8_t* raw, const uint64_t* raw_off, size_t n,
                              const uint32_t* policy, const uint8_t* ingress, const uint16_t* port,
                              const uint32_t* remote, uint8_t* out);

int cg_http_verdicts_fields_dev(uint64_t h, const uint8_t* d_hdr_blob, const uint64_t* d_hdr_off, size_t n,
                                const uint32_t* d_policy, const uint8_t* d_ingress, const uint16_t* d_port,
                                const uint32_t* d_remote, uint8_t* d_out, void* stream);

int cg_http_verdicts_fields_host(uint64_t h, const uint8_t* hdr_blob, const uint64_t* hdr_off, size_t n,
                                 const uint32_t* policy, const uint8_t* ingress, const uint16_t* port,
                                 const uint32_t* remote, uint8_t* out);

int cg_http_ring_open(uint64_t h, uint32_t workgroups, uint32_t slots);
int cg_http_ring_verdicts(uint64_t h, const uint8_t* hdr_blob, const uint64_t* hdr_off, size_t n,
                          const uint32_t* policy, const uint8_t* ingress, const uint16_t* port,
                          const uint32_t* remote, uint8_t* out);
int cg_http_ring_stats(uint64_t h, uint64_t* served, uint64_t* launches);
int cg_http_ring_close(uint64_t h);

int cg_http_verdicts_dev(uint64_t h, const void* d_batch, size_t nslots, const uint8_t* d_arena,
                         uint8_t* d_out, void* stream);
int cg_http_verdicts_host(uint64_t h, const void* batch, size_t nslots, const uint32_t* order,
                          size_t n, const uint8_t* arena, size_t arena_len, uint8_t* out);
int cg_http_verdicts_rules_dev(uint64_t h, const void* d_batch, size_t nslots, const uint8_t* d_arena,
                               uint8_t* d_out, uint32_t* d_rule, void* stream);
int cg_http_verdicts_rules_host(uint64_t h, const void* batch, size_t nslots, const uint32_t* order,
                                size_t n, const uint8_t* arena, size_t arena_len, uint8_t* out,
                                uint32_t* rule);


int cg_kafka_policy_update(uint64_t h, const char* json, size_t len);
int cg_kafka_policy_index(uint64_t h, const char* name, uint32_t* index);

#define CG_KAFKA_MAX_TOPICS 12
typedef struct {
  int16_t api_key;
  int16_t api_version;
  uint8_t kind;
  uint8_t n_topics;
  uint16_t policy;
  uint32_t remote;
  uint32_t client_id;
  uint32_t topic_ids[CG_KAFKA_MAX_TOPICS];
} cg_kafka_request;

#define CG_KAFKA_TOPICS_IN_ARENA 255
#define CG_KAFKA_K_NIL 0
#define CG_KAFKA_K_TYPED 1
#define CG_KAFKA_K_CONSUMER_METADATA 2
#define CG_KAFKA_UNKNOWN_STR 0xFFFFFFFFu

int cg_kafka_intern(uint64_t h, uint32_t what, const char* s, size_t len, uint32_t* id);

#define CG_KAFKA_DECODE_OK 0
#define CG_KAFKA_DECODE_ERROR 1
int cg_kafka_decode_host(uint64_t h, const uint8_t* raw, const uint64_t* raw_off, size_t n,
                         const uint16_t* redirect, const uint32_t* remote, cg_kafka_request* reqs,
                         uint32_t* arena, size_t arena_cap, size_t* arena_used, uint8_t* status);

int cg_kafka_decode_stats(uint64_t h, uint64_t* device_inflated, uint64_t* host_deferred);

int cg_kafka_inflate_stats(uint64_t h, uint64_t* unreserved);

int cg_kafka_decode_dev(uint64_t h, const uint8_t* d_raw, const uint64_t* d_raw_off, size_t n,
                        const uint16_t* d_redirect, const uint32_t* d_remote, cg_kafka_request* d_reqs,
                        uint32_t* d_arena, size_t arena_cap, size_t* arena_used, uint8_t* d_status,
                        void* stream);

#define CG_KAFKA_V_DENY 0
#define CG_KAFKA_V_ALLOW 1
#define CG_KAFKA_V_CLOSE 2
int cg_kafka_verdicts_raw_host(uint64_t h, const uint8_t* raw, const uint64_t* raw_off, size_t n,
                               const uint16_t* redirect, const uint32_t* remote, uint8_t* out);

int cg_kafka_verdicts_dev(uint64_t h, const cg_kafka_request* d_reqs, size_t n,
                          const uint32_t* d_arena, uint8_t* d_out, void* stream);
int cg_kafka_verdicts_host(uint64_t h, const cg_kafka_request* reqs, size_t n,
                           const uint32_t* arena, size_t arena_len, uint8_t* out);
typedef struct {
  int16_t api_key;
  int16_t api_version;
  uint8_t kind;
  uint8_t n_topics;
  uint16_t policy;
  uint32_t remote;
  uint32_t client_id;
} cg_kafka_request_head;
int cg_kafka_verdicts_split_dev(uint64_t h, const cg_kafka_request_head* d_heads, const uint32_t* d_topics,
                                size_t n, const uint32_t* d_arena, uint8_t* d_out, void* stream);

#define CG_CTR_HTTP_PROGRAMS 0u
#define CG_CTR_KAFKA 1u
#define CG_CTR_PREFILTER 2u
#define CG_CTR_HTTP_RULES 3u
#define CG_CTR_HTTP_ALLREDUCE 4u
int cg_read_counters(uint64_t h, uint32_t what, uint32_t pf_or_map, uint64_t* out, size_t cap,
                     size_t* n);
int cg_counters_device_ptr(uint64_t h, uint32_t what, uint32_t pf_or_map, void** d_ptr,
                           size_t* n);
int cg_counters_copy_dev(uint64_t h, uint32_t what, uint32_t pf_or_map, void* d_dst, size_t n,
                         void* stream);
int cg_reset_counters(uint64_t h);

int cg_sync(uint64_t h);

enum { CG_REGEX_ECMA = 0, CG_REGEX_GO = 1 };
int cg_regex_validate(const char* re, size_t re_len, uint32_t flavour);


enum {
  CG_SEL_MATCH_LABEL = 0,
  CG_SEL_IN = 1,
  CG_SEL_NOT_IN = 2,
  CG_SEL_EXISTS = 3,
  CG_SEL_DOES_NOT_EXIST = 4
};

typedef struct {
  size_t n_selectors;
  const uint32_t* req_off;
  const uint8_t* ops;
  const uint8_t* key_blob;
  const uint64_t* key_off;
  const uint32_t* val_off;
  const uint8_t* val_blob;
  const uint64_t* val_str_off;
} cg_selector_table;

typedef struct {
  size_t n_rules;
  const uint32_t* subject;
  const uint8_t* dir_flags;
  const uint32_t* req_off[2];
  const uint32_t* req_idx[2];
  const uint32_t* allow_off[2];
  const uint32_t* allow_idx[2];
} cg_selcache_rules;

int cg_selcache_create(uint64_t h, uint32_t* sc_id);
int cg_selcache_destroy(uint64_t h, uint32_t sc_id);
int cg_selcache_set_identities(uint64_t h, uint32_t sc_id, const uint32_t* ids, size_t n,
                               const uint32_t* label_off, const uint8_t* key_blob, const uint64_t* key_off,
                               const uint8_t* val_blob, const uint64_t* val_off);
int cg_selcache_set_cidr_identities(uint64_t h, uint32_t sc_id, const uint32_t* ids, const cg_cidr* prefixes,
                                    size_t n);
int cg_selcache_set_rules(uint64_t h, uint32_t sc_id, const cg_selector_table* sels,
                          const cg_selcache_rules* rules);
int cg_selcache_info(uint64_t h, uint32_t sc_id, size_t* n_identities, size_t* words, size_t* n_selectors,
                     size_t* n_rules);
int cg_selcache_match_dev(uint64_t h, uint32_t sc_id, const cg_selector_table* sels, uint64_t* d_bits,
                          size_t cap_words, void* stream);
int cg_selcache_match_host(uint64_t h, uint32_t sc_id, const cg_selector_table* sels, uint64_t* bits,
                           size_t cap_words);
int cg_selcache_reach_dev(uint64_t h, uint32_t sc_id, const uint32_t* d_endpoints, size_t n, uint64_t* d_ing,
                          uint64_t* d_eg, uint8_t* d_flags, void* stream);
int cg_selcache_reach_host(uint64_t h, uint32_t sc_id, const uint32_t* endpoints, size_t n, uint64_t* ing,
                           uint64_t* eg, uint8_t* flags);

#define CG_EXP_ALL 0x1u
typedef struct {
  uint16_t dport;
  uint8_t protocol;
  uint8_t egress;
  uint16_t proxy_port;
  uint16_t flags;
} cg_expand_row;
typedef struct {
  size_t n_rows;
  const cg_expand_row* rows;
  const uint32_t* src_off;
  const uint32_t* src_idx;
} cg_expand_table;
int cg_selcache_expand_dev(uint64_t h, uint32_t sc_id, const cg_expand_table* table, const uint64_t* d_src,
                           size_t src_rows, uint64_t* d_row_off, cg_policy_key* d_keys, uint16_t* d_proxy,
                           size_t cap_entries, uint64_t* d_total, void* stream);
int cg_selcache_expand_host(uint64_t h, uint32_t sc_id, const cg_expand_table* table, const uint64_t* src,
                            size_t src_rows, uint64_t* row_off, cg_policy_key* keys, uint16_t* proxy,
                            size_t cap_entries, uint64_t* total);
int cg_selcache_entries_host(uint64_t h, uint32_t sc_id, const cg_selector_table* sels, const uint32_t* endpoints,
                             size_t n_endpoints, const cg_expand_table* table, uint64_t* row_off,
                             cg_policy_key* keys, uint16_t* proxy, size_t cap_entries, uint64_t* total,
                             uint8_t* flags);

int cg_policymap_sync(uint64_t h, uint32_t map_id, const cg_policy_key* keys, const uint16_t* proxy_ports_be,
                      size_t n, size_t* added, size_t* deleted);

int cg_diag_regex_match(const char* re, size_t re_len, const uint8_t* s, size_t len,
                        uint32_t search, uint8_t* result);
int cg_diag_http_eval_host(uint64_t h, const void* batch, size_t nslots, const uint32_t* order,
                           size_t n, const uint8_t* arena, size_t arena_len, uint8_t* out);
int cg_diag_http_rules_host(uint64_t h, const void* batch, size_t nslots, const uint32_t* order,
                            size_t n, const uint8_t* arena, size_t arena_len, uint32_t* rule);
int cg_diag_kafka_eval_host(uint64_t h, const cg_kafka_request* reqs, size_t n,
                            const uint32_t* arena, size_t arena_len, uint8_t* out);
int cg_diag_kafka_decode_host(uint64_t h, const uint8_t* raw, const uint64_t* raw_off, size_t n,
                              const uint16_t* redirect, const uint32_t* remote, cg_kafka_request* reqs,
                              uint32_t* arena, size_t arena_cap, size_t* arena_used, uint8_t* status);
int cg_diag_l4_eval_host(uint64_t h, uint32_t map_id, const cg_l4_tuple* tuples, size_t n,
                         int32_t* verdicts);
int cg_diag_l4_array_eval_host(uint64_t h, uint32_t arr_id, uint32_t mode, const uint16_t* lxc_ids,
                               const cg_l4_tuple* tuples, size_t n, int32_t* verdicts);
int cg_diag_l4_frames_eval_host(uint64_t h, uint32_t arr_id, uint32_t mode, const uint8_t* raw,
                                const uint64_t* raw_off, size_t n, const uint16_t* lxc_ids, uint32_t ep_id,
                                const uint32_t* src_labels, uint32_t ipc_id, const uint32_t* pkt_len,
                                int32_t* verdicts, cg_l4_frame_info* info, uint32_t* l4_off);
int cg_diag_ipcache_eval_host(uint64_t h, uint32_t ipc_id, const uint32_t* v4, size_t n4,
                              cg_remote_endpoint_info* out4, const uint8_t* v6, size_t n6,
                              cg_remote_endpoint_info* out6);
int cg_diag_prefilter_eval_host(uint64_t h, uint32_t pf_id, const uint32_t* v4, size_t n4,
                                uint8_t* out4, const uint8_t* v6, size_t n6, uint8_t* out6);
int cg_diag_selcache_match_host(uint64_t h, uint32_t sc_id, const cg_selector_table* sels, uint64_t* bits,
                                size_t cap_words, uint32_t threads);
int cg_diag_selcache_reach_host(uint64_t h, uint32_t sc_id, const uint32_t* endpoints, size_t n, uint64_t* ing,
                                uint64_t* eg, uint8_t* flags, uint32_t threads);
int cg_diag_selcache_expand_host(uint64_t h, uint32_t sc_id, const cg_expand_table* table, const uint64_t* src,
                                 size_t src_rows, uint64_t* row_off, cg_policy_key* keys, uint16_t* proxy,
                                 size_t cap_entries, uint64_t* total, uint32_t threads);
int cg_diag_selcache_entries_host(uint64_t h, uint32_t sc_id, const cg_selector_table* sels,
                                  const uint32_t* endpoints, size_t n_endpoints, const cg_expand_table* table,
                                  uint64_t* row_off, cg_policy_key* keys, uint16_t* proxy, size_t cap_entries,
                                  uint64_t* total, uint8_t* flags, uint32_t threads);

#ifdef __cplusplus
}
#endif
#endif
```

Before: 87.36 billion.

## Add multi-symbol token columns to class DFAs and compress packed HTTP strings

Extends each class-coded HTTP DFA with extra columns for frequent forced-transition chains, so one transition consumes a whole token of up to 16 symbols. The host packer greedily rewrites class-coded strings into token codes, which shortens the per-request walk the GPU kernel does. The cost is larger transition tables and more host packing work; an environment variable can switch it off. The policy image format gains a version 2 with token tables.

```diff
diff --git a/cilium_amd/_native.py b/cilium_amd/_native.py
--- a/cilium_amd/_native.py
+++ b/cilium_amd/_native.py
@@ -153,6 +153,7 @@
     "cg_http_policy_index": (C.c_int, [_u64, C.c_char_p, C.POINTER(_u32)]),
     "cg_http_policy_stats": (C.c_int, [_u64, C.POINTER(_u64), _sz]),
     "cg_http_rule_info_get": (C.c_int, [_u64, _p, _sz, C.POINTER(_sz)]),
+    "cg_diag_http_tokens": (C.c_int, [_u64, _u32, _p, _p, _sz, C.POINTER(_sz)]),
     "cg_http_batch_bytes": (_sz, [_u64, _sz]),
     "cg_http_batch_slots": (_sz, [_u64, _sz]),
     "cg_http_pack": (C.c_int, [_u64, _sz, _p, _p, _p, _p, _p, _p, _p, _sz, _p, C.POINTER(_sz), _p, _sz,
diff --git a/cilium_amd/classifier.py b/cilium_amd/classifier.py
--- a/cilium_amd/classifier.py
+++ b/cilium_amd/classifier.py
@@ -114,10 +114,10 @@
         return v.value
 
     def http_policy_stats(self) -> dict:
-        out = (C.c_uint64 * 12)()
-        N.check(N.lib.cg_http_policy_stats(self.h, out, 12))
+        out = (C.c_uint64 * 14)()
+        N.check(N.lib.cg_http_policy_stats(self.h, out, 14))
         keys = ["programs", "parts", "states", "table_bytes", "fields", "rules", "policies", "remote_slots",
-                "exceptions", "cells", "max_program_cells", "lds_programs"]
+                "exceptions", "cells", "max_program_cells", "lds_programs", "tokens", "token_cells"]
         return dict(zip(keys, list(out)))
 
     def pack_http(self, policy: np.ndarray, ingress: np.ndarray, port: np.ndarray, remote: np.ndarray,
@@ -259,6 +259,19 @@
         N.check(N.lib.cg_diag_http_rules_host(self.h, _p(b.batch), b.nslots, _p(b.order), b.n, _p(b.arena),
                                               b.arena.nbytes, _p(out)))
         return out[:b.n]
+
+    def http_tokens_diag(self, prog: int) -> tuple[np.ndarray, list[tuple[int, bytes]]]:
+        code_map = np.zeros(256, np.uint8)
+        used = C.c_size_t()
+        N.check(N.lib.cg_diag_http_tokens(self.h, prog, _p(code_map), None, 0, C.byref(used)))
+        buf = np.zeros(max(used.value, 1), np.uint8)
+        N.check(N.lib.cg_diag_http_tokens(self.h, prog, None, _p(buf), buf.nbytes, C.byref(used)))
+        toks, at = [], 0
+        while at < used.value:
+            n = int(buf[at + 1])
+            toks.append((int(buf[at]), buf[at + 2:at + 2 + n].tobytes()))
+            at += 2 + n
+        return code_map, toks
 
     def http_eval_host_diag_slots(self, b: "HttpBatch") -> np.ndarray:
         v = self.http_eval_host_diag(b)
diff --git a/cilium_amd/csrc/capi.cc b/cilium_amd/csrc/capi.cc
--- a/cilium_amd/csrc/capi.cc
+++ b/cilium_amd/csrc/capi.cc
@@ -1722,7 +1722,7 @@
       max_prog_cells = std::max<uint64_t>(max_prog_cells, pg.cell_count);
       lds_progs += (pg.flags & kProgRebased) && pg.cell_count <= kMaxLdsCells;
     }
-    uint64_t v[12] = {s->progs.size(),
+    uint64_t v[14] = {s->progs.size(),
                      s->parts.size(),
                      s->total_states,
                      s->cells.size() * 4,
@@ -1733,8 +1733,31 @@
                      s->total_exceptions,
                      s->cells.size(),
                      max_prog_cells,
-                     lds_progs};
-    for (size_t i = 0; i < n && i < 12; ++i) out[i] = v[i];
+                     lds_progs,
+                     s->total_tokens,
+                     s->total_token_cells};
+    for (size_t i = 0; i < n && i < 14; ++i) out[i] = v[i];
+  });
+}
+
+int cg_diag_http_tokens(uint64_t h, uint32_t prog, uint8_t* code_map, uint8_t* out, size_t cap, size_t* used) {
+  return guarded([&] {
+    auto e = get(h);
+    auto s = http_snap(*e);
+    if (prog >= s->progs.size()) fail(CG_INVALID_ARGUMENT, "no such HTTP program");
+    const bool cls = s->progs[prog].flags & kProgClass;
+    if (code_map)
+      for (int b = 0; b < 256; ++b) code_map[b] = cls ? s->prog_code[prog][b] : (uint8_t)b;
+    size_t at = 0;
+    for (const auto& t : s->prog_tokens[prog]) {
+      if (out && at + 2 + t.seq.size() <= cap) {
+        out[at] = t.code;
+        out[at + 1] = (uint8_t)t.seq.size();
+        memcpy(out + at + 2, t.seq.data(), t.seq.size());
+      }
+      at += 2 + t.seq.size();
+    }
+    if (used) *used = at;
   });
 }
 
diff --git a/cilium_amd/csrc/clsdfa.cc b/cilium_amd/csrc/clsdfa.cc
--- a/cilium_amd/csrc/clsdfa.cc
+++ b/cilium_amd/csrc/clsdfa.cc
@@ -4,6 +4,8 @@
 #include <deque>
 #include <map>
 #include <numeric>
+#include <set>
+#include <string>
 #include <unordered_map>
 
 #include "common.h"
@@ -163,4 +165,149 @@
   return out;
 }
 
-}
+int run_classes(const ClsDfa& d, int s, const uint8_t* seq, size_t n) {
+  for (size_t i = 0; i < n && s != 0 && !d.label[s]; ++i) s = d.trans[(size_t)s * d.ncls + seq[i]];
+  return s;
+}
+
+ClsDfa with_token_columns(const ClsDfa& d, const std::vector<ClsSeq>& toks) {
+  ClsDfa o = d;
+  const int k = d.ncls, k2 = k + (int)toks.size();
+  o.ncls = k2;
+  o.trans.assign((size_t)d.size() * k2, 0);
+  for (int s = 0; s < d.size(); ++s) {
+    std::copy(d.trans.begin() + (size_t)s * k, d.trans.begin() + (size_t)(s + 1) * k, o.trans.begin() + (size_t)s * k2);
+    if (s == 0 || d.label[s]) continue;
+    for (size_t t = 0; t < toks.size(); ++t)
+      o.trans[(size_t)s * k2 + k + t] = run_classes(d, s, toks[t].data(), toks[t].size());
+  }
+  return o;
+}
+
+std::vector<ClsSeq> pick_tokens(const ClsDfa& d, const std::vector<std::vector<uint64_t>>& label_masks,
+                                int max_tokens, size_t cell_budget) {
+  std::vector<ClsSeq> picked;
+  const int n = d.size(), k = d.ncls;
+  if (max_tokens <= 0 || n < 3 || label_masks.empty()) return picked;
+  const size_t W = label_masks[0].size();
+  auto tr = [&](int s, int c) { return d.trans[(size_t)s * k + c]; };
+  std::vector<int> fcls(n, -1);
+  for (int s = 1; s < n; ++s) {
+    if (d.label[s]) continue;
+    int live = 0, c1 = -1;
+    for (int c = 0; c < k; ++c)
+      if (tr(s, c) != 0) {
+        ++live;
+        c1 = c;
+      }
+    if (live == 1 && tr(s, c1) != s) fcls[s] = c1;
+  }
+  std::vector<uint64_t> reach((size_t)n * W, 0);
+  for (int s = 1; s < n; ++s)
+    if (d.label[s] && d.label[s] - 1 < label_masks.size())
+      std::copy(label_masks[d.label[s] - 1].begin(), label_masks[d.label[s] - 1].end(), reach.begin() + (size_t)s * W);
+  for (bool changed = true; changed;) {
+    changed = false;
+    for (int s = n - 1; s >= 1; --s)
+      for (int c = 0; c < k; ++c) {
+        const int t = tr(s, c);
+        if (t == 0 || t == s) continue;
+        for (size_t w = 0; w < W; ++w) {
+          const uint64_t v = reach[(size_t)s * W + w] | reach[(size_t)t * W + w];
+          if (v != reach[(size_t)s * W + w]) {
+            reach[(size_t)s * W + w] = v;
+            changed = true;
+          }
+        }
+      }
+  }
+  std::vector<uint32_t> tags(n, 0);
+  for (int s = 0; s < n; ++s)
+    for (size_t w = 0; w < W; ++w) tags[s] += (uint32_t)__builtin_popcountll(reach[(size_t)s * W + w]);
+  constexpr size_t kChainMax = 64;
+  std::map<std::string, std::vector<uint64_t>> chains;
+  for (int s = 1; s < n; ++s) {
+    if (d.label[s] || (fcls[s] >= 0 && s != 1)) continue;
+    for (int c = 0; c < k; ++c) {
+      const int t = tr(s, c);
+      if (t == 0 || t == s || fcls[t] < 0) continue;
+      std::string sp(1, (char)c);
+      std::vector<uint64_t> w{tags[t]};
+      for (int cur = t; fcls[cur] >= 0 && sp.size() < kChainMax;) {
+        sp.push_back((char)fcls[cur]);
+        cur = tr(cur, fcls[cur]);
+        w.push_back(tags[cur]);
+      }
+      auto& acc = chains[sp];
+      acc.resize(w.size(), 0);
+      for (size_t i = 0; i < w.size(); ++i) acc[i] += w[i];
+    }
+  }
+  std::vector<uint8_t> self_row(n, 0);
+  for (int s = 1; s < n; ++s) {
+    int self_n = 0, dead_n = 0;
+    for (int c = 0; c < k; ++c) {
+      self_n += tr(s, c) == s;
+      dead_n += tr(s, c) == 0;
+    }
+    self_row[s] = !d.label[s] && self_n > dead_n;
+  }
+  auto cells_of = [&](const std::string& t) {
+    size_t cells = 0;
+    for (int s = 1; s < n; ++s)
+      if (!d.label[s]) cells += run_classes(d, s, (const uint8_t*)t.data(), t.size()) != (self_row[s] ? s : 0);
+    return cells;
+  };
+  size_t column_cap = std::max<size_t>((size_t)n / 8, 16);
+  std::vector<std::string> toks;
+  std::set<std::string> too_dear;
+  std::vector<uint8_t> covered;
+  for (int round = 0; round < max_tokens && cell_budget; ++round) {
+    std::unordered_map<std::string, uint64_t> score;
+    for (const auto& [sp, w] : chains) {
+      covered.assign(sp.size(), 0);
+      for (size_t i = 0; i < sp.size();) {
+        size_t best = 0;
+        for (const std::string& t : toks)
+          if (t.size() > best && sp.compare(i, t.size(), t) == 0) best = t.size();
+        if (best) std::fill(covered.begin() + i, covered.begin() + i + best, 1);
+        i += best ? best : 1;
+      }
+      for (size_t i = 0; i < sp.size(); ++i) {
+        if (covered[i]) continue;
+        for (size_t len = 2; len <= (size_t)kTokenMaxLen && i + len <= sp.size() && !covered[i + len - 1]; ++len)
+          score[sp.substr(i, len)] += (uint64_t)(len - 1) * w[i + len - 1];
+      }
+    }
+    std::vector<std::pair<uint64_t, const std::string*>> cand;
+    for (const auto& [sp, sc] : score)
+      if (sc && !too_dear.count(sp)) cand.push_back({sc, &sp});
+    std::sort(cand.begin(), cand.end(), [](const auto& a, const auto& b) {
+      if (a.first != b.first) return a.first > b.first;
+      if (a.second->size() != b.second->size()) return a.second->size() > b.second->size();
+      return *a.second < *b.second;
+    });
+    const std::string* best = nullptr;
+    for (const auto& c : cand) {
+      const size_t cells = cells_of(*c.second);
+      if (cells <= cell_budget && cells <= column_cap) {
+        best = c.second;
+        cell_budget -= cells;
+        break;
+      }
+      too_dear.insert(*c.second);
+    }
+    if (!best) {
+      if (column_cap == SIZE_MAX) break;
+      column_cap = SIZE_MAX;
+      too_dear.clear();
+      --round;
+      continue;
+    }
+    toks.push_back(*best);
+  }
+  for (const std::string& t : toks) picked.emplace_back(t.begin(), t.end());
+  return picked;
+}
+
+}
diff --git a/cilium_amd/csrc/clsdfa.h b/cilium_amd/csrc/clsdfa.h
--- a/cilium_amd/csrc/clsdfa.h
+++ b/cilium_amd/csrc/clsdfa.h
@@ -17,4 +17,14 @@
 
 ClsDfa minimize_cls(const ClsDfa& d);
 
+constexpr int kTokenMaxLen = 16;
+using ClsSeq = std::vector<uint8_t>;
+
+int run_classes(const ClsDfa& d, int s, const uint8_t* seq, size_t n);
+
+std::vector<ClsSeq> pick_tokens(const ClsDfa& d, const std::vector<std::vector<uint64_t>>& label_masks,
+                                int max_tokens, size_t cell_budget);
+
+ClsDfa with_token_columns(const ClsDfa& d, const std::vector<ClsSeq>& toks);
+
 }
diff --git a/cilium_amd/csrc/dev_types.h b/cilium_amd/csrc/dev_types.h
--- a/cilium_amd/csrc/dev_types.h
+++ b/cilium_amd/csrc/dev_types.h
@@ -142,6 +142,7 @@
 constexpr uint32_t kRdirMaxSpan = 8192;
 constexpr uint32_t kLdsRuleHits = 512;
 constexpr uint32_t kMaxLdsCells = (160 * 1024 - 64 - 4 * kLdsRuleHits - 4 * 64) / 4;
+constexpr uint32_t kTwoWgLdsCells = (80 * 1024 / 4 - 64 - kLdsRuleHits - 3) & ~255u;
 constexpr uint32_t kNoRow = 0xFFFFFFFFu;
 constexpr uint32_t kProgRebased = 4;
 constexpr uint32_t kProgClass = 8;
diff --git a/cilium_amd/csrc/http.cc b/cilium_amd/csrc/http.cc
--- a/cilium_amd/csrc/http.cc
+++ b/cilium_amd/csrc/http.cc
@@ -612,133 +612,186 @@
       S.prog_code.resize(pid + 1);
       S.prog_code[pid] = code;
     }
-    pg.part_begin = (uint32_t)S.parts.size();
-    pg.part_count = (uint32_t)parts.size();
-    while (S.cells.size() & 3) S.cells.push_back(kCombEmpty);
-    pg.cell_begin = (uint32_t)S.cells.size();
-    size_t block = 0;
-    for (const auto& po : parts) block += po.comb.cells.size();
-    const bool rebase = block <= kCombMaxBase;
-    if (rebase) pg.flags |= kProgRebased;
-    for (auto& po : parts) {
-      HttpPart hp{};
-      const ClsDfa& d = po.dfa;
-      CombTable& cb = po.comb;
-      hp.cell_off = (uint32_t)S.cells.size();
-      if (rebase) rebase_comb(&cb, hp.cell_off - pg.cell_begin);
-      hp.walk_off = rebase ? pg.cell_begin : hp.cell_off;
-      hp.nstates = (uint32_t)d.size();
-      hp.start = cb.start;
-      hp.dead = cb.dead;
-      hp.ncells = (uint32_t)cb.cells.size();
-      hp.mode = cb.scaled ? kPartClass : 0;
-      S.cells.insert(S.cells.end(), cb.cells.begin(), cb.cells.end());
-      S.total_states += d.size();
-      S.total_exceptions += cb.exceptions;
-      S.parts.push_back(hp);
-    }
-    auto put_mask = [&](const std::vector<uint64_t>& m) -> uint32_t {
-      if (S.cells.size() & 1) S.cells.push_back(0);
-      const uint32_t off = (uint32_t)S.cells.size() - pg.cell_begin;
-      for (uint64_t w : m) {
-        S.cells.push_back((uint32_t)w);
-        S.cells.push_back((uint32_t)(w >> 32));
-      }
-      return off;
+    const size_t parts0 = S.parts.size(), cells0 = S.cells.size();
+    const uint64_t totals0[3] = {S.total_states, S.total_exceptions, S.total_remote_slots};
+    const HttpProg pg0 = pg;
+    auto retract = [&] {
+      S.parts.resize(parts0);
+      S.cells.resize(cells0);
+      S.total_states = totals0[0];
+      S.total_exceptions = totals0[1];
+      S.total_remote_slots = totals0[2];
+      pg = pg0;
     };
-    for (size_t i = 0; i < parts.size(); ++i) {
-      HttpPart& hp = S.parts[pg.part_begin + i];
-      if (S.cells.size() & 1) S.cells.push_back(0);
-      hp.acc_off = (uint32_t)S.cells.size() - pg.cell_begin;
-      for (size_t l = 0; l < parts[i].label_masks.size(); ++l) put_mask(parts[i].label_masks[l]);
-    }
-    pg.always_off = put_mask(always);
-    {
-      std::map<std::vector<uint64_t>, uint32_t> rows;
-      auto row_of = [&](const std::vector<uint64_t>& m) {
-        auto it = rows.find(m);
-        if (it == rows.end()) it = rows.emplace(m, put_mask(m)).first;
-        return it->second;
+    auto emit = [&] {
+      pg.part_begin = (uint32_t)S.parts.size();
+      pg.part_count = (uint32_t)parts.size();
+      while (S.cells.size() & 3) S.cells.push_back(kCombEmpty);
+      pg.cell_begin = (uint32_t)S.cells.size();
+      size_t block = 0;
+      for (const auto& po : parts) block += po.comb.cells.size();
+      const bool rebase = block <= kCombMaxBase;
+      if (rebase) pg.flags |= kProgRebased;
+      for (auto& po : parts) {
+        HttpPart hp{};
+        const ClsDfa& d = po.dfa;
+        CombTable& cb = po.comb;
+        hp.cell_off = (uint32_t)S.cells.size();
+        if (rebase) rebase_comb(&cb, hp.cell_off - pg.cell_begin);
+        hp.walk_off = rebase ? pg.cell_begin : hp.cell_off;
+        hp.nstates = (uint32_t)d.size();
+        hp.start = cb.start;
+        hp.dead = cb.dead;
+        hp.ncells = (uint32_t)cb.cells.size();
+        hp.mode = cb.scaled ? kPartClass : 0;
+        S.cells.insert(S.cells.end(), cb.cells.begin(), cb.cells.end());
+        S.total_states += d.size();
+        S.total_exceptions += cb.exceptions;
+        S.parts.push_back(hp);
+      }
+      auto put_mask = [&](const std::vector<uint64_t>& m) -> uint32_t {
+        if (S.cells.size() & 1) S.cells.push_back(0);
+        const uint32_t off = (uint32_t)S.cells.size() - pg.cell_begin;
+        for (uint64_t w : m) {
+          S.cells.push_back((uint32_t)w);
+          S.cells.push_back((uint32_t)(w >> 32));
+        }
+        return off;
       };
-      pg.default_remote = row_of(open);
-      std::vector<std::pair<uint32_t, uint32_t>> ent;
-      for (auto& [rid, m] : by_remote) ent.push_back({rid, row_of(m)});
-      uint32_t nb = (uint32_t)std::max<size_t>((ent.size() * 10 / 9 + 3) / 4, 1);
-      std::vector<std::pair<uint32_t, uint32_t>> slots;
-      for (;; nb += nb / 8 + 1) {
-        if (nb >= 65536) fail(CG_POLICY_REJECTED, "too many remote identities in one HTTP policy scope");
-        slots.assign((size_t)nb * 4, {0u, kNoRow});
-        std::mt19937 rng(0xC111A);
-        auto put = [&](uint32_t bk, const std::pair<uint32_t, uint32_t>& e) {
-          for (int sl = 0; sl < 4; ++sl)
-            if (slots[(size_t)bk * 4 + sl].second == kNoRow) {
-              slots[(size_t)bk * 4 + sl] = e;
-              return true;
+      for (size_t i = 0; i < parts.size(); ++i) {
+        HttpPart& hp = S.parts[pg.part_begin + i];
+        if (S.cells.size() & 1) S.cells.push_back(0);
+        hp.acc_off = (uint32_t)S.cells.size() - pg.cell_begin;
+        for (size_t l = 0; l < parts[i].label_masks.size(); ++l) put_mask(parts[i].label_masks[l]);
+      }
+      pg.always_off = put_mask(always);
+      {
+        std::map<std::vector<uint64_t>, uint32_t> rows;
+        auto row_of = [&](const std::vector<uint64_t>& m) {
+          auto it = rows.find(m);
+          if (it == rows.end()) it = rows.emplace(m, put_mask(m)).first;
+          return it->second;
+        };
+        pg.default_remote = row_of(open);
+        std::vector<std::pair<uint32_t, uint32_t>> ent;
+        for (auto& [rid, m] : by_remote) ent.push_back({rid, row_of(m)});
+        uint32_t nb = (uint32_t)std::max<size_t>((ent.size() * 10 / 9 + 3) / 4, 1);
+        std::vector<std::pair<uint32_t, uint32_t>> slots;
+        for (;; nb += nb / 8 + 1) {
+          if (nb >= 65536) fail(CG_POLICY_REJECTED, "too many remote identities in one HTTP policy scope");
+          slots.assign((size_t)nb * 4, {0u, kNoRow});
+          std::mt19937 rng(0xC111A);
+          auto put = [&](uint32_t bk, const std::pair<uint32_t, uint32_t>& e) {
+            for (int sl = 0; sl < 4; ++sl)
+              if (slots[(size_t)bk * 4 + sl].second == kNoRow) {
+                slots[(size_t)bk * 4 + sl] = e;
+                return true;
+              }
+            return false;
+          };
+          bool ok = true;
+          for (const auto& e : ent) {
+            auto cur = e;
+            uint32_t from = 0xFFFFFFFFu;
+            bool placed = false;
+            for (int kick = 0; kick < 500 && !placed; ++kick) {
+              const uint32_t c1 = rtab_b1(cur.first, nb), c2 = rtab_b2(cur.first, nb);
+              if (put(c1, cur) || put(c2, cur)) {
+                placed = true;
+                break;
+              }
+              const uint32_t vb = c1 == from ? c2 : c2 == from ? c1 : (rng() & 1) ? c1 : c2;
+              std::swap(cur, slots[(size_t)vb * 4 + (rng() & 3)]);
+              from = vb;
             }
-          return false;
-        };
-        bool ok = true;
-        for (const auto& e : ent) {
-          auto cur = e;
-          uint32_t from = 0xFFFFFFFFu;
-          bool placed = false;
-          for (int kick = 0; kick < 500 && !placed; ++kick) {
-            const uint32_t c1 = rtab_b1(cur.first, nb), c2 = rtab_b2(cur.first, nb);
-            if (put(c1, cur) || put(c2, cur)) {
-              placed = true;
+            if (!placed) {
+              ok = false;
               break;
             }
-            const uint32_t vb = c1 == from ? c2 : c2 == from ? c1 : (rng() & 1) ? c1 : c2;
-            std::swap(cur, slots[(size_t)vb * 4 + (rng() & 3)]);
-            from = vb;
           }
-          if (!placed) {
-            ok = false;
-            break;
+          if (ok) break;
+        }
+        while ((S.cells.size() - pg.cell_begin) & 3) S.cells.push_back(0);
+
+        pg.rtab_off = (uint32_t)S.cells.size() - pg.cell_begin;
+        pg.rtab_nb = nb;
+        uint32_t empty_id = 0;
+        while (by_remote.count(empty_id)) ++empty_id;
+        const size_t at = S.cells.size();
+        S.cells.resize(at + kRtabBucketCells * (size_t)nb, 0);
+        for (uint32_t k = 0; k < nb; ++k)
+          for (int sl = 0; sl < 4; ++sl) {
+            const auto& e = slots[(size_t)k * 4 + sl];
+            const bool empty = e.second == kNoRow;
+            S.cells[at + kRtabBucketCells * k + sl] = empty ? empty_id : e.first;
+            S.cells[at + kRtabBucketCells * k + 4 + sl] = empty ? pg.default_remote : e.second;
           }
-        }
-        if (ok) break;
-      }
-      while ((S.cells.size() - pg.cell_begin) & 3) S.cells.push_back(0);
-
-      pg.rtab_off = (uint32_t)S.cells.size() - pg.cell_begin;
-      pg.rtab_nb = nb;
-      uint32_t empty_id = 0;
-      while (by_remote.count(empty_id)) ++empty_id;
-      const size_t at = S.cells.size();
-      S.cells.resize(at + kRtabBucketCells * (size_t)nb, 0);
-      for (uint32_t k = 0; k < nb; ++k)
-        for (int sl = 0; sl < 4; ++sl) {
-          const auto& e = slots[(size_t)k * 4 + sl];
-          const bool empty = e.second == kNoRow;
-          S.cells[at + kRtabBucketCells * k + sl] = empty ? empty_id : e.first;
-          S.cells[at + kRtabBucketCells * k + 4 + sl] = empty ? pg.default_remote : e.second;
-        }
-      const uint32_t cap = 4 * nb;
-      S.total_remote_slots += cap;
-      if (!ent.empty()) {
-        uint32_t lo = ent[0].first, hi = ent[0].first;
-        bool rows16 = pg.default_remote < 0x10000;
-        for (const auto& e : ent) {
-          lo = std::min(lo, e.first);
-          hi = std::max(hi, e.first);
-          rows16 &= e.second < 0x10000;
-        }
-        if (rows16 && hi - lo < kRdirMaxSpan) {
-          const uint32_t len = hi - lo + 1;
-          std::vector<uint16_t> t(len + 1, (uint16_t)pg.default_remote);
-          for (const auto& e : ent) t[e.first - lo] = (uint16_t)e.second;
-          pg.rdir_base = lo;
-          pg.rdir_len = len;
-          pg.rdir_off = (uint32_t)S.cells.size() - pg.cell_begin;
-          for (uint32_t k = 0; k < len; k += 2) S.cells.push_back((uint32_t)t[k] | (uint32_t)t[k + 1] << 16);
-          pg.flags |= kProgRemoteDirect;
-        }
-      }
-    }
-    S.cells.push_back(0);
-    S.cells.push_back(0);
-    pg.cell_count = (uint32_t)S.cells.size() - pg.cell_begin;
+        const uint32_t cap = 4 * nb;
+        S.total_remote_slots += cap;
+        if (!ent.empty()) {
+          uint32_t lo = ent[0].first, hi = ent[0].first;
+          bool rows16 = pg.default_remote < 0x10000;
+          for (const auto& e : ent) {
+            lo = std::min(lo, e.first);
+            hi = std::max(hi, e.first);
+            rows16 &= e.second < 0x10000;
+          }
+          if (rows16 && hi - lo < kRdirMaxSpan) {
+            const uint32_t len = hi - lo + 1;
+            std::vector<uint16_t> t(len + 1, (uint16_t)pg.default_remote);
+            for (const auto& e : ent) t[e.first - lo] = (uint16_t)e.second;
+            pg.rdir_base = lo;
+            pg.rdir_len = len;
+            pg.rdir_off = (uint32_t)S.cells.size() - pg.cell_begin;
+            for (uint32_t k = 0; k < len; k += 2) S.cells.push_back((uint32_t)t[k] | (uint32_t)t[k + 1] << 16);
+            pg.flags |= kProgRemoteDirect;
+          }
+        }
+      }
+      S.cells.push_back(0);
+      S.cells.push_back(0);
+      pg.cell_count = (uint32_t)S.cells.size() - pg.cell_begin;
+    };
+    emit();
+    if ((pg.flags & kProgClass) && (pg.flags & kProgRebased) && pg.cell_count <= kMaxLdsCells &&
+        parts[0].dfa.ncls < 64) {
+      const uint32_t base_count = pg.cell_count;
+      const uint32_t limit = base_count <= kTwoWgLdsCells ? kTwoWgLdsCells : kMaxLdsCells;
+      const PartOut base = parts[0];
+      const int ncls = base.dfa.ncls;
+      std::vector<uint32_t> labels(base.dfa.size(), kCombNoLabel);
+      for (int st = 0; st < base.dfa.size(); ++st)
+        if (base.dfa.label[st]) labels[st] = base.dfa.label[st] - 1;
+      std::vector<ClsSeq> toks = pick_tokens(base.dfa, base.label_masks, 64 - ncls, limit - base_count);
+      bool relaid = false;
+      while (!toks.empty()) {
+        ClsDfa wide = with_token_columns(base.dfa, toks);
+        CombTable ct;
+        if (build_comb(wide, labels, &ct, kCombMaxBase, true) && scale_comb(&ct)) {
+          retract();
+          parts[0].dfa = std::move(wide);
+          parts[0].comb = std::move(ct);
+          emit();
+          relaid = true;
+          if ((pg.flags & kProgRebased) && pg.cell_count <= limit) break;
+        }
+        toks.pop_back();
+      }
+      if (toks.empty() && relaid) {
+        retract();
+        parts[0] = base;
+        emit();
+      }
+      S.prog_tokens.resize(pid + 1);
+      for (size_t t = 0; t < toks.size(); ++t) {
+        HttpSnapshot::Token tk;
+        tk.code = (uint8_t)(4 * (ncls + t));
+        for (uint8_t c : toks[t]) tk.seq.push_back((uint8_t)(4 * c));
+        S.prog_tokens[pid].push_back(std::move(tk));
+      }
+      S.total_tokens += toks.size();
+      S.total_token_cells += pg.cell_count > base_count ? pg.cell_count - base_count : 0;
+    }
     if (getenv("CILIUM_GPU_DEBUG")) {
       size_t comb = 0, labels = 0;
       for (uint32_t i = 0; i < pg.part_count; ++i) {
@@ -789,6 +842,7 @@
   if (S.cells.empty()) S.cells.push_back(kCombEmpty);
   if (S.progs.empty()) S.progs.push_back(HttpProg{});
   S.prog_code.resize(S.progs.size());
+  S.prog_tokens.resize(S.progs.size());
   if (S.parts.empty()) S.parts.push_back(HttpPart{});
   if (S.dflt.empty()) S.dflt.push_back(kProgDeny);
   return snap;
diff --git a/cilium_amd/csrc/http.h b/cilium_amd/csrc/http.h
--- a/cilium_amd/csrc/http.h
+++ b/cilium_amd/csrc/http.h
@@ -25,6 +25,13 @@
   std::vector<uint32_t> dflt;
   std::vector<uint32_t> prog_key;
   std::vector<std::array<uint8_t, 256>> prog_code;
+  struct Token {
+    uint8_t code;
+    std::vector<uint8_t> seq;
+  };
+  std::vector<std::vector<Token>> prog_tokens;
+  uint64_t total_tokens = 0;
+  uint64_t total_token_cells = 0;
   std::vector<cg_http_rule_info> rule_info;
 
   uint32_t epoch = 0;
diff --git a/cilium_amd/csrc/http_image.cc b/cilium_amd/csrc/http_image.cc
--- a/cilium_amd/csrc/http_image.cc
+++ b/cilium_amd/csrc/http_image.cc
@@ -10,8 +10,10 @@
 namespace {
 
 constexpr uint32_t kImageMagic = 0x49484743u;
-constexpr uint32_t kImageVersion = 1u | (uint32_t)sizeof(HttpProg) << 8 | (uint32_t)sizeof(HttpPart) << 16 |
+constexpr uint32_t kImageLayouts = (uint32_t)sizeof(HttpProg) << 8 | (uint32_t)sizeof(HttpPart) << 16 |
                                    (uint32_t)sizeof(cg_http_rule_info) << 24;
+constexpr uint32_t kImageVersion1 = 1u | kImageLayouts;
+constexpr uint32_t kImageVersion = 2u | kImageLayouts;
 
 uint64_t fnv64(const uint8_t* p, size_t n) {
   uint64_t h = 1469598103934665603ull;
@@ -101,6 +103,17 @@
   w.u64(s.total_exceptions);
   w.u64(s.total_rules);
   w.u64(s.total_remote_slots);
+  w.u64(s.total_tokens);
+  w.u64(s.total_token_cells);
+  w.u64(s.prog_tokens.size());
+  for (const auto& toks : s.prog_tokens) {
+    w.u32((uint32_t)toks.size());
+    for (const auto& t : toks) {
+      w.u32(t.code);
+      w.u32((uint32_t)t.seq.size());
+      w.raw(t.seq.data(), t.seq.size());
+    }
+  }
   w.u64(fnv64(w.b.data(), w.b.size()));
   return std::move(w.b);
 }
@@ -117,7 +130,8 @@
     if (s.phash_keys[i] != 0xFFFFFFFFu && !prog_ref_ok(s.phash_vals[i])) bad("program hash value out of range");
   }
   if (!empty_slot) bad("program hash has no empty slot");
-  if (s.dflt.size() < (size_t)s.npolicies * 2 || s.prog_code.size() != np || s.prog_key.size() > np)
+  if (s.dflt.size() < (size_t)s.npolicies * 2 || s.prog_code.size() != np || s.prog_key.size() > np ||
+      s.prog_tokens.size() != np)
     bad("inconsistent tables");
   for (uint32_t v : s.dflt)
     if (!prog_ref_ok(v)) bad("default program out of range");
@@ -165,6 +179,16 @@
         if (c & 3) bad("class code not a cell offset");
         max_code = std::max<uint32_t>(max_code, c);
       }
+      const uint32_t max_class = max_code;
+      for (const auto& t : s.prog_tokens[pi]) {
+        if ((t.code & 3) || t.code <= max_class) bad("token code not a free cell offset");
+        if (t.seq.size() < 2 || t.seq.size() > (size_t)kTokenMaxLen) bad("bad token length");
+        for (uint8_t c : t.seq)
+          if ((c & 3) || c > max_class) bad("token symbol not a class code");
+        max_code = std::max<uint32_t>(max_code, t.code);
+      }
+    } else if (!s.prog_tokens[pi].empty()) {
+      bad("tokens of a program without class codes");
     }
     const bool rebased = pg.flags & kProgRebased;
     const uint64_t limit = rebased ? (uint64_t)pg.cell_begin + pg.cell_count : nc;
@@ -204,7 +228,9 @@
   if (sum != fnv64(p, n - 8)) fail(CG_POLICY_REJECTED, "policy image: checksum mismatch");
   Reader r{p, p + n - 8};
   if (r.u32() != kImageMagic) fail(CG_POLICY_REJECTED, "policy image: bad magic");
-  if (r.u32() != kImageVersion) fail(CG_POLICY_REJECTED, "policy image: built by another library version");
+  const uint32_t version = r.u32();
+  if (version != kImageVersion && version != kImageVersion1)
+    fail(CG_POLICY_REJECTED, "policy image: built by another library version");
   auto snap = std::make_shared<HttpSnapshot>();
   HttpSnapshot& s = *snap;
   s.raw_values = r.u32() != 0;
@@ -231,6 +257,26 @@
   s.total_exceptions = r.u64();
   s.total_rules = r.u64();
   s.total_remote_slots = r.u64();
+  if (version != kImageVersion1) {
+    s.total_tokens = r.u64();
+    s.total_token_cells = r.u64();
+    const uint64_t nprog = r.u64();
+    if (nprog > s.progs.size()) fail(CG_POLICY_REJECTED, "policy image: bad token table");
+    s.prog_tokens.resize((size_t)nprog);
+    for (auto& toks : s.prog_tokens) {
+      const uint32_t nt = r.u32();
+      if (nt > 64) fail(CG_POLICY_REJECTED, "policy image: bad token count");
+      toks.resize(nt);
+      for (auto& t : toks) {
+        t.code = (uint8_t)r.u32();
+        const uint32_t len = r.u32();
+        if (len > (uint32_t)kTokenMaxLen) fail(CG_POLICY_REJECTED, "policy image: bad token length");
+        t.seq.resize(len);
+        r.raw(t.seq.data(), len);
+      }
+    }
+  }
+  s.prog_tokens.resize(s.progs.size());
   if (r.p != r.e) fail(CG_POLICY_REJECTED, "policy image: trailing bytes");
   validate_image(s);
   s.epoch = http_next_epoch();
diff --git a/cilium_amd/csrc/http_pack.cc b/cilium_amd/csrc/http_pack.cc
--- a/cilium_amd/csrc/http_pack.cc
+++ b/cilium_amd/csrc/http_pack.cc
@@ -142,6 +142,24 @@
     const size_t L = s.fields[f].size();
     if (by_len.size() <= L) by_len.resize(L + 1);
     by_len[L].push_back((uint32_t)f);
+  }
+  const char* tok_env = getenv("CILIUM_GPU_PACK_TOKENS");
+  const bool tokens = !(tok_env && tok_env[0] == '0' && !tok_env[1]);
+  std::vector<std::vector<int16_t>> tok_first(np), tok_next(np);
+  for (size_t p = 0; p < np && p < s.prog_tokens.size() && tokens && build; ++p) {
+    const auto& toks = s.prog_tokens[p];
+    if (toks.empty()) continue;
+    std::vector<int16_t> asc(toks.size());
+    for (size_t t = 0; t < toks.size(); ++t) asc[t] = (int16_t)t;
+    std::stable_sort(asc.begin(), asc.end(),
+                     [&](int16_t a, int16_t b) { return toks[a].seq.size() < toks[b].seq.size(); });
+    tok_first[p].assign(64, -1);
+    tok_next[p].assign(toks.size(), -1);
+    for (int16_t t : asc) {
+      int16_t& head = tok_first[p][toks[t].seq[0] >> 2];
+      tok_next[p][t] = head;
+      head = t;
+    }
   }
   auto worker_of = [&](size_t i) -> unsigned {
     unsigned t = (unsigned)((i * nt) / n);
@@ -206,6 +224,29 @@
       if (prog[i] < np && (s.progs[prog[i]].flags & kProgClass)) {
         const auto& code = s.prog_code[prog[i]];
         for (size_t k = o; k < strs.size(); ++k) strs[k] = code[strs[k]];
+        if (tokens && slen[i] <= CG_HTTP_SLOT_BYTES && !tok_first[prog[i]].empty()) {
+          const auto& first = tok_first[prog[i]];
+          const auto& toks = s.prog_tokens[prog[i]];
+          uint8_t* q = strs.data() + o;
+          const size_t L = slen[i];
+          size_t w = 0;
+          for (size_t r = 0; r < L;) {
+            size_t hit = 0;
+            uint8_t sym = q[r];
+            for (int16_t t = first[q[r] >> 2]; t >= 0; t = tok_next[prog[i]][t]) {
+              const auto& sq = toks[t].seq;
+              if (sq.size() <= L - r && memcmp(q + r, sq.data(), sq.size()) == 0) {
+                hit = sq.size();
+                sym = toks[t].code;
+                break;
+              }
+            }
+            q[w++] = sym;
+            r += hit ? hit : 1;
+          }
+          strs.resize(o + w);
+          slen[i] = (uint32_t)w;
+        }
       }
     }
   });
diff --git a/include/cilium_gpu.h b/include/cilium_gpu.h
--- a/include/cilium_gpu.h
+++ b/include/cilium_gpu.h
@@ -464,6 +464,7 @@
                         uint32_t search, uint8_t* result);
 int cg_diag_http_eval_host(uint64_t h, const void* batch, size_t nslots, const uint32_t* order,
                            size_t n, const uint8_t* arena, size_t arena_len, uint8_t* out);
+int cg_diag_http_tokens(uint64_t h, uint32_t prog, uint8_t* code_map, uint8_t* out, size_t cap, size_t* used);
 int cg_diag_http_rules_host(uint64_t h, const void* batch, size_t nslots, const uint32_t* order,
                             size_t n, const uint8_t* arena, size_t arena_len, uint32_t* rule);
 int cg_diag_kafka_eval_host(uint64_t h, const cg_kafka_request* reqs, size_t n,
```

Result: faster. 100.7 billion (median of 6 runs) (+15.3%).
